# jopohl/urh

Hardware: NVIDIA H100
Metric: MSamples/s IQ demod+digitize (complex64) (higher is better)
Workload: dtype f32

## Files before the change

urh_b200/csrc/center.cu:

```cuda
#include "dense.cuh"
#include "tilescan.cuh"

#include <math.h>
#include <stdlib.h>

int urh_window_var_bitwise(urh_ctx* ctx, const float* d_x, int64_t n, const int64_t* d_prefix, int64_t t0, int64_t t1, int64_t r0,
                           int64_t r1, float* h_out2);

struct CenStats {
    double sum, sumsq;
    float mn, mx;
    long long cnt;
};

__global__ void __launch_bounds__(URH_WARPS_PER_BLOCK * 32)
k_tile_stats_f32(const float* __restrict__ x, int64_t n, int64_t ntiles, UrhTileStats* __restrict__ ts) {
    const int lane = threadIdx.x & 31;
    const int64_t tile = (int64_t)blockIdx.x * URH_WARPS_PER_BLOCK + (threadIdx.x >> 5);
    if (tile >= ntiles) return;
    const int64_t base = tile * URH_TILE;
    UrhStatAcc acc;
    acc.init();
    acc.all_noise = false;
    if (base + URH_TILE <= n && (((uintptr_t)x) & 15) == 0) {
        const float4* p = (const float4*)(x + base) + lane;
        constexpr int ITERS = URH_TILE / 128;
        float4 cur[4], nxt[4];
#pragma unroll
        for (int j = 0; j < 4; j++) cur[j] = __ldg(p + j * 32);
        for (int it = 0; it < ITERS; it += 4) {
            if (it + 4 < ITERS) {
#pragma unroll
                for (int j = 0; j < 4; j++) nxt[j] = __ldg(p + (it + 4 + j) * 32);
            }
#pragma unroll
            for (int j = 0; j < 4; j++) {
                acc.add(cur[j].x); acc.add(cur[j].y); acc.add(cur[j].z); acc.add(cur[j].w);
            }
#pragma unroll
            for (int j = 0; j < 4; j++) cur[j] = nxt[j];
        }
    } else {
        for (int j = lane; j < URH_TILE; j += 32)
            if (base + j < n) acc.add(x[base + j]);
    }
    acc.store(ts + tile, lane);
}

struct ScanKept {
    const UrhTileStats* ts;
    int64_t* prefix;
    __device__ __forceinline__ int64_t load(int64_t t) const { return ts[t].cnt; }
    __device__ __forceinline__ void post(int64_t t, const int64_t& excl, const int64_t&) const { prefix[t] = excl; }
};
struct CenAddI64 {
    __device__ __forceinline__ int64_t operator()(int64_t a, int64_t b) const { return a + b; }
};

static int kept_prefix(urh_ctx* ctx, const UrhTileStats* ts, int64_t ntiles, int64_t* prefix) {
    ScanKept fk;
    fk.ts = ts; fk.prefix = prefix;
    return urhts::scan<int64_t, CenAddI64, ScanKept>(ctx, ntiles, (int64_t)0, CenAddI64(), fk, prefix + ntiles);
}

#define CEN_PER (URH_TILE / 256)
__device__ __forceinline__ int64_t cen_tile_ranks(const float* __restrict__ x, int64_t n, int64_t t, int64_t tile_rank0, float (&v)[CEN_PER],
                                                  int* s_pre) {
    const int64_t base = t * URH_TILE + (int64_t)threadIdx.x * CEN_PER;
    int mine = 0;
#pragma unroll
    for (int j = 0; j < CEN_PER; j++) {
        v[j] = (base + j < n) ? x[base + j] : -5.0f;
        mine += (v[j] > -4.0f) ? 1 : 0;
    }
    s_pre[threadIdx.x] = mine;
    __syncthreads();
    for (int off = 1; off < 256; off <<= 1) {
        int add = 0;
        if (threadIdx.x >= off) add = s_pre[threadIdx.x - off];
        __syncthreads();
        s_pre[threadIdx.x] += add;
        __syncthreads();
    }
    return tile_rank0 + s_pre[threadIdx.x] - mine;
}

__device__ __forceinline__ void cen_block_fold(double sum, double sq, float mn, float mx, long long cnt, CenStats* out) {
    __shared__ double s_sum[256], s_sq[256];
    __shared__ float s_mn[256], s_mx[256];
    __shared__ long long s_cnt[256];
    __syncthreads();
    s_sum[threadIdx.x] = sum; s_sq[threadIdx.x] = sq; s_mn[threadIdx.x] = mn; s_mx[threadIdx.x] = mx; s_cnt[threadIdx.x] = cnt;
    __syncthreads();
    for (int off = 128; off > 0; off >>= 1) {
        if (threadIdx.x < off) {
            s_sum[threadIdx.x] += s_sum[threadIdx.x + off];
            s_sq[threadIdx.x] += s_sq[threadIdx.x + off];
            s_mn[threadIdx.x] = fminf(s_mn[threadIdx.x], s_mn[threadIdx.x + off]);
            s_mx[threadIdx.x] = fmaxf(s_mx[threadIdx.x], s_mx[threadIdx.x + off]);
            s_cnt[threadIdx.x] += s_cnt[threadIdx.x + off];
        }
        __syncthreads();
    }
    if (threadIdx.x == 0) {
        CenStats r;
        r.sum = s_sum[0]; r.sumsq = s_sq[0]; r.mn = s_mn[0]; r.mx = s_mx[0]; r.cnt = s_cnt[0];
        *out = r;
    }
}

int urh_center_tiles_begin(urh_ctx* ctx, const float* d_x, const UrhTileStats* ts, int64_t n, int64_t* h_total) {
    const int64_t ntiles = urh_div_up(n, URH_TILE);
    int64_t* prefix;
    URH_CHECK(urh_arena(ctx, (size_t)ntiles + 1, &prefix));
    URH_CHECK(kept_prefix(ctx, ts, ntiles, prefix));
    URH_CHECK(urh_read_i64(ctx, prefix + ntiles, 1, h_total));
    ctx->center_prefix = prefix;
    ctx->center_ts = ts;
    ctx->center_n = n;
    ctx->center_x = d_x;
    return URH_OK;
}

static int tiles_from_array(urh_ctx* ctx, const float* d_x, int64_t n, int64_t* h_total) {
    urh_arena_reset(ctx);
    ctx->center_prefix = nullptr;
    const int64_t ntiles = urh_div_up(n, URH_TILE);
    UrhTileStats* ts;
    URH_CHECK(urh_arena(ctx, (size_t)ntiles, &ts));
    URH_LAUNCH(ctx, k_tile_stats_f32, (unsigned)urh_div_up(ntiles, URH_WARPS_PER_BLOCK), URH_WARPS_PER_BLOCK * 32, 0, d_x, n, ntiles, ts);
    return urh_center_tiles_begin(ctx, d_x, ts, n, h_total);
}

static bool tiles_match(const urh_ctx* ctx, const float* d_x, int64_t n) {
    return ctx->center_prefix && ctx->center_n == n && ctx->center_x == (const void*)d_x;
}

extern "C" int urh_center_window_var(urh_ctx* ctx, const float* d_qad, int64_t n, int64_t r0, int64_t r1, double* h_out2) {
    h_out2[0] = h_out2[1] = 0.0;
    if (!tiles_match(ctx, d_qad, n)) URH_FAIL(ctx, URH_ERR_INVALID, "the tile table of this array must precede urh_center_window_var");
    if (r1 <= r0) return URH_OK;
    float mv[2];
    URH_CHECK(urh_window_var_bitwise(ctx, d_qad, n, (const int64_t*)ctx->center_prefix, 0, urh_div_up(n, URH_TILE) - 1, r0, r1, mv));
    h_out2[0] = (double)mv[0];
    h_out2[1] = (double)mv[1];
    return URH_OK;
}

extern "C" int urh_center_stats(urh_ctx* ctx, const float* d_x, int64_t n, int64_t max_size, double* h_out) {
    for (int i = 0; i < 7; i++) h_out[i] = 0.0;
    if (n <= 0) return URH_OK;
    int64_t total = 0;
    URH_CHECK(tiles_from_array(ctx, d_x, n, &total));
    int64_t r0 = (int64_t)(0.05 * (double)total), r1 = (int64_t)(0.95 * (double)total);
    if (max_size >= 0 && r1 - r0 > max_size) r1 = r0 + max_size;
    h_out[0] = (double)total; h_out[1] = (double)r0; h_out[2] = (double)r1;
    if (r1 <= r0) return URH_OK;
    double w[5];
    URH_CHECK(urh_center_window_stats(ctx, d_x, n, r0, r1, w));
    if (w[0] <= 0.0) return URH_OK;
    h_out[3] = w[1]; h_out[4] = w[2];
    float mv[2];
    URH_CHECK(urh_window_var_bitwise(ctx, d_x, n, (const int64_t*)ctx->center_prefix, 0, urh_div_up(n, URH_TILE) - 1, r0, r1, mv));
    h_out[5] = (double)mv[0];
    h_out[6] = (double)mv[1];
    return URH_OK;
}


template <typename K>
__device__ __forceinline__ double cen_edge(K k, const double& hmin, const double& edge1, const double& delta) {
    return (k == 0) ? hmin : (k == 1 ? edge1 : __dadd_rn(hmin, __dmul_rn((double)k, delta)));
}

__device__ __forceinline__ void cen_edge_table(long long k0, long long stride, long long nbins, const double& hmin, const double& edge1,
                                               const double& delta, float* __restrict__ fe, unsigned long long* __restrict__ hist,
                                               unsigned long long* __restrict__ xhist) {
    for (long long k = k0; k <= nbins; k += stride) {
        const double e = cen_edge(k, hmin, edge1, delta);
        fe[k] = __double2float_ru(e);
        if (k == nbins) {
            fe[nbins + 1] = __double2float_rd(e);
            fe[nbins + 2] = fmaxf(__double2float_ru(hmin), nextafterf(-4.0f, 0.0f));
        }
        if (k < nbins) {
            hist[k] = 0ull;
            if (xhist) xhist[k] = 0ull;
        }
    }
}

struct HistBins {
    const float* fe;
    float f_min, f_hi, scale, off;
    int nbins;
    __device__ __forceinline__ void load(const float* fe_, float scale_, int nbins_) {
        fe = fe_; nbins = nbins_; scale = scale_;
        f_hi = fe[nbins + 1];
        f_min = fe[nbins + 2];
        off = -fe[0] * scale;
    }
    template <bool FAST>
    __device__ __forceinline__ int bin_of(float f) const {
        const bool valid = f >= f_min && f <= f_hi;
        if (FAST) {
            const float t = fmaf(f, scale, off);
            int r = __float_as_int(t + 12582912.0f) - 0x4B400000;
            r = max(0, min(r, nbins));
            int k = r - ((f < fe[r]) ? 1 : 0);
            k = min(k, nbins - 1);
            return valid ? k : -1;
        }
        if (!valid) return -1;
        int k = (int)((f - fe[0]) * scale);
        k = max(0, min(k, nbins - 1));
        while (k > 0 && f < fe[k]) k--;
        while (k < nbins - 1 && f >= fe[k + 1]) k++;
        return k;
    }
};

struct HistCache {
    float lo0, hi0, lo1, hi1, lo2, hi2, lo3, hi3;
    int h0, h1, h2, h3;
    unsigned c0, c1, c2, c3;
    __device__ __forceinline__ void init() {
        lo0 = lo1 = lo2 = lo3 = INFINITY;
        hi0 = hi1 = hi2 = hi3 = -INFINITY;
        h0 = h1 = h2 = h3 = 0;
        c0 = c1 = c2 = c3 = 0u;
    }
};

template <bool SMEM>
__device__ __forceinline__ void hist_bump(unsigned int* s_hist, unsigned long long* hist, int k, unsigned c) {
    if (SMEM) atomicAdd(&s_hist[k], c);
    else atomicAdd(&hist[k], (unsigned long long)c);
}

template <bool SMEM, bool FAST>
__device__ __forceinline__ void hist_miss(HistCache& hc, const HistBins& hb, unsigned int* s_hist, unsigned long long* hist, float f) {
    const int k = hb.bin_of<FAST>(f);
    if (k < 0) return;
    const float lo = fmaxf(hb.fe[k], hb.f_min);
    const float hi = (k == hb.nbins - 1) ? nextafterf(hb.f_hi, INFINITY) : hb.fe[k + 1];
    unsigned cm = hc.c0; int which = 0;
    if (hc.c1 < cm) { cm = hc.c1; which = 1; }
    if (hc.c2 < cm) { cm = hc.c2; which = 2; }
    if (hc.c3 < cm) { cm = hc.c3; which = 3; }
    const int old = which == 0 ? hc.h0 : which == 1 ? hc.h1 : which == 2 ? hc.h2 : hc.h3;
    if (cm) hist_bump<SMEM>(s_hist, hist, old, cm);
    if (which == 0) { hc.h0 = k; hc.c0 = 1u; hc.lo0 = lo; hc.hi0 = hi; }
    else if (which == 1) { hc.h1 = k; hc.c1 = 1u; hc.lo1 = lo; hc.hi1 = hi; }
    else if (which == 2) { hc.h2 = k; hc.c2 = 1u; hc.lo2 = lo; hc.hi2 = hi; }
    else { hc.h3 = k; hc.c3 = 1u; hc.lo3 = lo; hc.hi3 = hi; }
}

template <bool SMEM, bool FAST>
__device__ __forceinline__ void hist_put(HistCache& hc, const HistBins& hb, unsigned int* s_hist, unsigned long long* hist, float f,
                                         unsigned one) {
    unsigned miss;
    asm("{\n\t.reg .pred p0, p1, p2, p3, pv;\n\t"
        "setp.ge.f32 p0, %5, %6;\n\tsetp.lt.and.f32 p0, %5, %7, p0;\n\t@p0 mad.lo.u32 %0, %0, %15, %15;\n\t"
        "setp.ge.f32 p1, %5, %8;\n\tsetp.lt.and.f32 p1, %5, %9, p1;\n\t@p1 mad.lo.u32 %1, %1, %15, %15;\n\t"
        "setp.ge.f32 p2, %5, %10;\n\tsetp.lt.and.f32 p2, %5, %11, p2;\n\t@p2 mad.lo.u32 %2, %2, %15, %15;\n\t"
        "setp.ge.f32 p3, %5, %12;\n\tsetp.lt.and.f32 p3, %5, %13, p3;\n\t@p3 mad.lo.u32 %3, %3, %15, %15;\n\t"
        "or.pred p0, p0, p1;\n\tor.pred p2, p2, p3;\n\tor.pred p0, p0, p2;\n\t"
        "setp.ge.f32 pv, %5, %14;\n\t"
        "and.pred pv, pv, !p0;\n\t"
        "selp.u32 %4, 1, 0, pv;\n\t}"
        : "+r"(hc.c0), "+r"(hc.c1), "+r"(hc.c2), "+r"(hc.c3), "=r"(miss)
        : "f"(f), "f"(hc.lo0), "f"(hc.hi0), "f"(hc.lo1), "f"(hc.hi1), "f"(hc.lo2), "f"(hc.hi2), "f"(hc.lo3), "f"(hc.hi3),
          "f"(hb.f_min), "r"(one));
    if (miss) hist_miss<SMEM, FAST>(hc, hb, s_hist, hist, f);
}

template <bool SMEM>
__device__ __forceinline__ void hist_flush(HistCache& hc, unsigned int* s_hist, unsigned long long* hist) {
    if (hc.c0) hist_bump<SMEM>(s_hist, hist, hc.h0, hc.c0);
    if (hc.c1) hist_bump<SMEM>(s_hist, hist, hc.h1, hc.c1);
    if (hc.c2) hist_bump<SMEM>(s_hist, hist, hc.h2, hc.c2);
    if (hc.c3) hist_bump<SMEM>(s_hist, hist, hc.h3, hc.c3);
}

template <bool SMEM, bool FAST>
__device__ __forceinline__ void hist_interior_body(const float* __restrict__ x, int64_t n, int64_t t_first, int64_t t_end, int blk, int nblk,
                                                   const float* __restrict__ g_fe, float scale, int nbins,
                                                   unsigned long long* __restrict__ hist, int edges_in_smem,
                                                   const int64_t* __restrict__ prefix) {
    extern __shared__ unsigned int s_dyn[];
    unsigned int* s_hist = s_dyn;
    float* s_fe = (float*)(s_dyn + (SMEM ? nbins : 0));
    const int lane = threadIdx.x & 31;
    if (SMEM)
        for (int b = threadIdx.x; b < nbins; b += 256) s_hist[b] = 0u;
    if (edges_in_smem)
        for (int b = threadIdx.x; b < nbins + 3; b += 256) s_fe[b] = g_fe[b];
    __syncthreads();
    HistBins hb;
    if (FAST) hb.load(s_fe, scale, nbins);
    else hb.load(edges_in_smem ? s_fe : g_fe, scale, nbins);
    HistCache hc;
    hc.init();
    const int64_t gw = (int64_t)blk * 8 + (threadIdx.x >> 5), nw = (int64_t)nblk * 8;
    const bool vec = (((uintptr_t)x) & 15) == 0;
    const unsigned one = blockDim.x >> 8;
    {
        for (int64_t t = t_first + gw; t < t_end; t += nw) {
            if (prefix[t + 1] == prefix[t]) continue;
            const int64_t base = t * URH_TILE;
            if (vec) {
                const float4* p = (const float4*)(x + base) + lane;
                constexpr int ITERS = URH_TILE / 128, DEPTH = 4;
                float4 buf[DEPTH];
#pragma unroll
                for (int j = 0; j < DEPTH; j++) buf[j] = __ldg(p + j * 32);
#pragma unroll 1
                for (int it = 0; it < ITERS; it += DEPTH) {
                    const bool more = it + DEPTH < ITERS;
#pragma unroll
                    for (int j = 0; j < DEPTH; j++) {
                        const float4 v = buf[j];
                        if (more) buf[j] = __ldg(p + (it + DEPTH + j) * 32);
                        hist_put<SMEM, FAST>(hc, hb, s_hist, hist, v.x, one);
                        hist_put<SMEM, FAST>(hc, hb, s_hist, hist, v.y, one);
                        hist_put<SMEM, FAST>(hc, hb, s_hist, hist, v.z, one);
                        hist_put<SMEM, FAST>(hc, hb, s_hist, hist, v.w, one);
                    }
                }
            } else {
                for (int j = lane; j < URH_TILE; j += 32) hist_put<SMEM, FAST>(hc, hb, s_hist, hist, x[base + j], one);
            }
        }
    }
    hist_flush<SMEM>(hc, s_hist, hist);
    if (SMEM) {
        __syncthreads();
        for (int b = threadIdx.x; b < nbins; b += 256)
            if (s_hist[b]) atomicAdd(&hist[b], (unsigned long long)s_hist[b]);
    }
}

__device__ __forceinline__ void hist_window_ends_body(const float* __restrict__ x, int64_t n, const int64_t* __restrict__ prefix,
                                                      const int64_t* __restrict__ win, int64_t r0, int64_t r1,
                                                      const float* __restrict__ g_fe, float scale, int nbins,
                                                      unsigned long long* __restrict__ hist, unsigned long long* __restrict__ hist2 = nullptr) {
    __shared__ int s_pre[256];
    const int64_t t = win[blockIdx.x];
    if (t < 0 || (blockIdx.x == 1 && t == win[0])) return;
    HistBins hb;
    hb.load(g_fe, scale, nbins);
    float v[CEN_PER];
    int64_t rank = cen_tile_ranks(x, n, t, prefix[t], v, s_pre);
#pragma unroll
    for (int j = 0; j < CEN_PER; j++) {
        const bool kept = v[j] > -4.0f;
        const int k = hb.bin_of<false>(v[j]);
        if (k >= 0 && rank >= r0 && rank < r1) {
            atomicAdd(&hist[k], 1ull);
            if (hist2) atomicAdd(&hist2[k], 1ull);
        }
        rank += kept ? 1 : 0;
    }
}

extern "C" int urh_center_histogram(urh_ctx* ctx, const float* d_x, int64_t n, int64_t r0, int64_t r1, double hmin,
                                    double hstep, int64_t nbins, int64_t* h_hist) {
    if (nbins <= 0 || n <= 0) return URH_OK;
    if (!tiles_match(ctx, d_x, n)) {
        int64_t total = 0;
        URH_CHECK(tiles_from_array(ctx, d_x, n, &total));
    }
    return urh_center_histogram_tiles(ctx, d_x, n, r0, r1, hmin, hstep, nbins, h_hist);
}

#define CEN_MAX_BINS 6000
#define CEN_VAR_MIN_RATIO 0x1p-14

struct __align__(16) CenterPlan {
    long long total, offset;
    long long r0, r1;
    long long lr0, lr1;
    long long win[4];
    CenStats local;
    double hmin, edge1, delta;
    long long nbins;
    double center;
    float centerf;
    float scale;
    int fast;
    int state;
    unsigned int ticket;
    int certified;
    long long straddle;
    long long pad;
};

__global__ void k_center_ranks(const int64_t* __restrict__ counts, int rank, int world, int64_t max_size, CenterPlan* __restrict__ plan) {
    long long total = 0, offset = 0;
    for (int q = 0; q < world; q++) {
        if (q < rank) offset += counts[q];
        total += counts[q];
    }
    const long long kept = counts[rank];
    long long r0 = (long long)(0.05 * (double)total), r1 = (long long)(0.95 * (double)total);
    if (max_size >= 0 && r1 - r0 > max_size) r1 = r0 + max_size;
    plan->total = total; plan->offset = offset; plan->r0 = r0; plan->r1 = r1;
    long long a = r0 - offset, b = r1 - offset;
    a = a < 0 ? 0 : (a > kept ? kept : a);
    b = b < 0 ? 0 : (b > kept ? kept : b);
    plan->lr0 = a; plan->lr1 = b;
    plan->ticket = 0u;
    plan->state = 1;
    plan->certified = 0;
    plan->straddle = 0;
}

__device__ __forceinline__ int64_t cen_tile_of_rank(const int64_t* __restrict__ prefix, int64_t ntiles, int64_t r) {
    int64_t lo = 0, hi = ntiles;
    while (hi - lo > 1) {
        const int64_t mid = (lo + hi) >> 1;
        if (prefix[mid] <= r) lo = mid; else hi = mid;
    }
    return lo;
}

__device__ __forceinline__ void cen_window_tiles(const int64_t* __restrict__ prefix, int64_t ntiles, long long r0, long long r1,
                                                 long long (&w)[4]) {
    long long w0 = -1, w1 = -1, w2 = -1, w3 = -1;
    if (r1 > r0) {
        w0 = cen_tile_of_rank(prefix, ntiles, r0);
        w1 = cen_tile_of_rank(prefix, ntiles, r1 - 1);
        const bool cov0 = prefix[w0] >= r0 && prefix[w0 + 1] <= r1;
        const bool cov1 = prefix[w1] >= r0 && prefix[w1 + 1] <= r1;
        w2 = cov0 ? -1 : w0;
        w3 = (cov1 || w1 == w0) ? -1 : w1;
    }
    w[0] = w0; w[1] = w1; w[2] = w2; w[3] = w3;
}

__global__ void __launch_bounds__(256) k_center_window(const float* __restrict__ x, int64_t n, const UrhTileStats* __restrict__ ts,
                                                      const int64_t* __restrict__ prefix, int64_t ntiles, CenterPlan* __restrict__ plan,
                                                      CenStats* __restrict__ partial) {
    __shared__ long long s_win[4];
    __shared__ int s_pre[256];
    __shared__ bool s_last;
    const long long r0 = plan->lr0, r1 = plan->lr1;
    if (threadIdx.x == 0) {
        long long w[4];
        cen_window_tiles(prefix, ntiles, r0, r1, w);
        s_win[0] = w[0]; s_win[1] = w[1]; s_win[2] = w[2]; s_win[3] = w[3];
        if (blockIdx.x == 0) { plan->win[0] = w[0]; plan->win[1] = w[1]; plan->win[2] = w[2]; plan->win[3] = w[3]; }
    }
    __syncthreads();
    double sum = 0.0, sq = 0.0;
    float mn = INFINITY, mx = -INFINITY;
    long long cnt = 0;
    if (s_win[0] >= 0) {
        for (int64_t t = s_win[0] + (int64_t)blockIdx.x * 256 + threadIdx.x; t <= s_win[1]; t += (int64_t)gridDim.x * 256) {
            const int64_t a = prefix[t], b = prefix[t + 1];
            if (b > a && a >= r0 && b <= r1) {
                const UrhTileStats v = ts[t];
                sum += v.sum; sq += v.sumsq; mn = fminf(mn, v.mn); mx = fmaxf(mx, v.mx); cnt += v.cnt;
            }
        }
    }
    cen_block_fold(sum, sq, mn, mx, cnt, partial + blockIdx.x);
    if (blockIdx.x < 2) {
        const int64_t t = s_win[2 + blockIdx.x];
        sum = 0.0; sq = 0.0; mn = INFINITY; mx = -INFINITY; cnt = 0;
        if (t >= 0) {
            float v[CEN_PER];
            int64_t rank = cen_tile_ranks(x, n, t, prefix[t], v, s_pre);
#pragma unroll
            for (int j = 0; j < CEN_PER; j++) {
                if (v[j] > -4.0f) {
                    if (rank >= r0 && rank < r1) {
                        sum += (double)v[j];
                        sq += (double)v[j] * (double)v[j];
                        mn = fminf(mn, v[j]);
                        mx = fmaxf(mx, v[j]);
                        cnt++;
                    }
                    rank++;
                }
            }
        }
        cen_block_fold(sum, sq, mn, mx, cnt, partial + gridDim.x + blockIdx.x);
    }
    __threadfence();
    __syncthreads();
    if (threadIdx.x == 0) s_last = atomicAdd(&plan->ticket, 1u) == gridDim.x - 1;
    __syncthreads();
    if (!s_last) return;
    __threadfence();
    sum = 0.0; sq = 0.0; mn = INFINITY; mx = -INFINITY; cnt = 0;
    for (int64_t t = threadIdx.x; t < (int64_t)gridDim.x + 2; t += 256) {
        CenStats p;
        {
            const int4* src = (const int4*)(partial + t);
            int4 w0 = __ldcg(src), w1 = __ldcg(src + 1);
            memcpy(&p, &w0, 16);
            memcpy((char*)&p + 16, &w1, 16);
        }
        sum += p.sum; sq += p.sumsq; mn = fminf(mn, p.mn); mx = fmaxf(mx, p.mx); cnt += p.cnt;
    }
    cen_block_fold(sum, sq, mn, mx, cnt, &plan->local);
}

__global__ void __launch_bounds__(256) k_center_plan(const CenStats* __restrict__ parts, int world, CenterPlan* __restrict__ plan,
                                                    float* __restrict__ fe, unsigned long long* __restrict__ hist,
                                                    unsigned long long* __restrict__ xhist) {
    __shared__ int s_state;
    __shared__ long long s_nbins;
    __shared__ double s_hmin, s_edge1, s_delta;
    if (threadIdx.x == 0) {
        double cnt = 0.0, sum = 0.0, sq = 0.0;
        float mn = INFINITY, mx = -INFINITY;
        for (int q = 0; q < world; q++) {
            cnt += (double)parts[q].cnt;
            mn = fminf(mn, parts[q].mn);
            mx = fmaxf(mx, parts[q].mx);
            sum = __dadd_rn(sum, parts[q].sum);
            sq = __dadd_rn(sq, parts[q].sumsq);
        }
        int state = 0;
        long long nbins = 0;
        double hmin = 0.0, edge1 = 0.0, delta = 0.0;
        if (plan->r1 > plan->r0 && cnt > 0.0) {
            const double mean = __ddiv_rn(sum, cnt);
            double ss = __dsub_rn(sq, __dmul_rn(__dmul_rn(cnt, mean), mean));
            if (ss < 0.0) ss = 0.0;
            const double var = __ddiv_rn(ss, cnt);
            const double hstep = (double)__double2float_rn(var);
            hmin = (double)mn;
            const double stop = __dadd_rn((double)mx, hstep);
            if (!(var >= __dmul_rn(__dmul_rn(mean, mean), CEN_VAR_MIN_RATIO))) state = 2;
            else if (hstep != 0.0) {
                const double val = __ddiv_rn(__dsub_rn(stop, hmin), hstep);
                if (val == val && fabs(val) < 9.0e18) {
                    const long long len = (long long)ceil(val);
                    if (len >= 2) {
                        nbins = len - 1;
                        edge1 = __dadd_rn(hmin, hstep);
                        delta = __dsub_rn(edge1, hmin);
                        state = (nbins <= CEN_MAX_BINS && delta > 0.0) ? 1 : 2;
                    }
                }
            }
        }
        plan->hmin = hmin; plan->edge1 = edge1; plan->delta = delta; plan->nbins = nbins;
        plan->state = state;
        plan->center = 0.0; plan->centerf = 0.0f;
        if (state == 1) {
            plan->scale = (float)(1.0 / delta);
            const double edge_abs = fmax(fabs(hmin), fabs(hmin + (double)nbins * delta));
            plan->fast = (edge_abs / delta < 1048576.0) ? 1 : 0;
        }
        s_state = state; s_nbins = nbins; s_hmin = hmin; s_edge1 = edge1; s_delta = delta;
    }
    __syncthreads();
    if (s_state != 1) return;
    cen_edge_table(threadIdx.x, 256, s_nbins, s_hmin, s_edge1, s_delta, fe, hist, xhist);
}

template <bool SMEM, bool FAST, int MIN_BLOCKS>
__global__ void __launch_bounds__(256, MIN_BLOCKS) k_hist_interior(const float* __restrict__ x, int64_t n, const CenterPlan* __restrict__ plan,
                                                                  const float* __restrict__ g_fe, unsigned long long* __restrict__ hist,
                                                                  const int64_t* __restrict__ prefix, int edges_in_smem) {
    if (plan->state != 1 || plan->certified || (plan->fast != 0) != FAST) return;
    hist_interior_body<SMEM, FAST>(x, n, plan->win[0] + 1, plan->win[1], blockIdx.x, gridDim.x, g_fe, plan->scale, (int)plan->nbins, hist,
                                   edges_in_smem, prefix);
}

__device__ __forceinline__ void cen_full_slabs(int64_t win0, int64_t win1, int64_t slab_tiles, int64_t* sf, int64_t* se) {
    *sf = (win0 + slab_tiles) / slab_tiles;
    *se = win1 / slab_tiles;
}

__global__ void __launch_bounds__(256) k_hist_window_ends(const float* __restrict__ x, int64_t n, const int64_t* __restrict__ prefix,
                                                         const CenterPlan* __restrict__ plan, const float* __restrict__ g_fe,
                                                         unsigned long long* __restrict__ hist, unsigned long long* __restrict__ xhist,
                                                         int64_t slab_tiles) {
    if (plan->state != 1) return;
    if (blockIdx.x < 2) {
        hist_window_ends_body(x, n, prefix, (const int64_t*)plan->win, plan->lr0, plan->lr1, g_fe, plan->scale, (int)plan->nbins, hist, xhist);
        return;
    }
    const int64_t w0 = plan->win[0], w1 = plan->win[1];
    int64_t sf, se;
    cen_full_slabs(w0, w1, slab_tiles, &sf, &se);
    int64_t a_end = w1, b_begin = w1;
    if (sf < se) { a_end = sf * slab_tiles; b_begin = se * slab_tiles; }
    const int blk = blockIdx.x - 2, nblk = gridDim.x - 2, nbins = (int)plan->nbins;
    const float scale = plan->scale;
    if (plan->fast) {
        hist_interior_body<true, true>(x, n, w0 + 1, a_end, blk, nblk, g_fe, scale, nbins, xhist, 1, prefix);
        hist_interior_body<true, true>(x, n, b_begin, w1, blk, nblk, g_fe, scale, nbins, xhist, 1, prefix);
    } else {
        hist_interior_body<true, false>(x, n, w0 + 1, a_end, blk, nblk, g_fe, scale, nbins, xhist, 1, prefix);
        hist_interior_body<true, false>(x, n, b_begin, w1, blk, nblk, g_fe, scale, nbins, xhist, 1, prefix);
    }
}

__device__ __forceinline__ double cen_left_edge(const CenterPlan* plan, int k) {
    return cen_edge(k, plan->hmin, plan->edge1, plan->delta);
}

#define CERT_THREADS 512
__global__ void __launch_bounds__(CERT_THREADS) k_center_certify(const UrhFine fine, CenterPlan* __restrict__ plan, const float* __restrict__ fe,
                                                                 const unsigned long long* __restrict__ xhist, unsigned long long* __restrict__ lo,
                                                                 unsigned long long* __restrict__ hi) {
    __shared__ unsigned long long s_ge[URH_FINE_NB + 1];
    __shared__ unsigned long long s_part[CERT_THREADS];
    __shared__ unsigned char s_flag[CEN_MAX_BINS];
    __shared__ unsigned long long s_key[3];
    __shared__ unsigned int s_certain;
    if (plan->state != 1) return;
    const int tid = threadIdx.x;
    constexpr int PER = URH_FINE_NB / CERT_THREADS;
    int64_t sf, se;
    cen_full_slabs(plan->win[0], plan->win[1], fine.slab_tiles, &sf, &se);
    unsigned long long b[PER], tot = 0;
#pragma unroll
    for (int j = 0; j < PER; j++) {
        unsigned long long v = 0;
        for (int64_t sl = sf; sl < se; sl++) v += fine.gh[sl * URH_FINE_NB + tid * PER + j];
        b[j] = v;
        tot += v;
    }
    s_part[tid] = tot;
    if (tid < 3) s_key[tid] = 0ull;
    if (tid == 0) s_certain = 0u;
    __syncthreads();
    for (int off = 1; off < CERT_THREADS; off <<= 1) {
        const unsigned long long add = (tid + off < CERT_THREADS) ? s_part[tid + off] : 0ull;
        __syncthreads();
        s_part[tid] += add;
        __syncthreads();
    }
    unsigned long long run = (tid + 1 < CERT_THREADS) ? s_part[tid + 1] : 0ull;
#pragma unroll
    for (int j = PER - 1; j >= 0; j--) {
        run += b[j];
        s_ge[tid * PER + j] = run;
    }
    if (tid == 0) s_ge[URH_FINE_NB] = 0ull;
    __syncthreads();
    const int nbins = (int)plan->nbins;
    const float f_hi = fe[nbins + 1], f_min = fe[nbins + 2], top = nextafterf(f_hi, INFINITY);
    auto ge = [&](float t, unsigned long long& glo, unsigned long long& ghi) {
        const int bt = urh_fine_bucket(t, fine.scale, fine.off);
        const bool straddles = urh_fine_bucket(nextafterf(t, -INFINITY), fine.scale, fine.off) == bt;
        ghi = s_ge[bt];
        glo = straddles ? s_ge[bt + 1] : s_ge[bt];
    };
    for (int k = tid; k < nbins; k += CERT_THREADS) {
        const float a = fmaxf(fe[k], f_min), e = (k == nbins - 1) ? top : fminf(fe[k + 1], top);
        unsigned long long l = 0, u = 0;
        if (a < e) {
            unsigned long long alo, ahi, elo, ehi;
            ge(a, alo, ahi);
            ge(e, elo, ehi);
            l = alo > ehi ? alo - ehi : 0ull;
            u = ahi - elo;
        }
        lo[k] = xhist[k] + l;
        hi[k] = xhist[k] + u;
    }
    __syncthreads();
    int window = (int)(0.05 * (double)nbins) + 1;
    if (window < 2) window = 2;
    for (int k = tid; k < nbins; k += CERT_THREADS) {
        const unsigned long long l = lo[k], u = hi[k];
        bool certain = l > 0ull, possible = u > 0ull;
        for (int d = -(window - 1); d < window && (certain || possible); d++) {
            const int j = k + d;
            if (d == 0 || j < 0 || j >= nbins) continue;
            certain = certain && l > hi[j];
            possible = possible && u > lo[j];
        }
        s_flag[k] = certain ? 1 : (possible ? 2 : 0);
        if (certain) atomicAdd(&s_certain, 1u);
    }
    __syncthreads();
    for (int pass = 0; pass < 3; pass++) {
        const long long p0 = pass > 0 ? (long long)(8191 - (s_key[0] & 8191)) : -1, p1 = pass > 1 ? (long long)(8191 - (s_key[1] & 8191)) : -1;
        for (int k = tid; k < nbins; k += CERT_THREADS) {
            if (k == p0 || k == p1) continue;
            if (pass < 2 && s_flag[k] == 1) atomicMax(&s_key[pass], (lo[k] << 13) | (unsigned long long)(8191 - k));
            if (pass == 2 && s_flag[k] != 0) atomicMax(&s_key[2], hi[k]);
        }
        __syncthreads();
    }
    if (tid != 0 || s_certain < 2u) return;
    const int k1 = 8191 - (int)(s_key[0] & 8191), k2 = 8191 - (int)(s_key[1] & 8191);
    plan->straddle = (long long)((hi[k1] - lo[k1]) + (hi[k2] - lo[k2]));
    if (!(lo[k2] > s_key[2])) return;
    const double c = __ddiv_rn(__dadd_rn(cen_left_edge(plan, k1), cen_left_edge(plan, k2)), 2.0);
    plan->center = c;
    plan->centerf = __double2float_rn(c);
    plan->certified = 1;
}

__global__ void __launch_bounds__(256) k_center_pick(const unsigned long long* __restrict__ y, CenterPlan* __restrict__ plan) {
    __shared__ unsigned long long s_best[256];
    __shared__ int s_idx[256];
    __shared__ int s_cnt[256];
    if (plan->state != 1 || plan->certified) return;
    const int nbins = (int)plan->nbins;
    int window = (int)(0.05 * (double)nbins) + 1;
    if (window < 2) window = 2;
    unsigned long long top_val[2] = {0ull, 0ull};
    int top_idx[2] = {-1, -1};
    int found = 0;
    bool undecided = false;
    for (int pass = 0; pass < 2 && !undecided; pass++) {
        unsigned long long best = 0ull;
        int bi = -1, ties = 0;
        for (int i = threadIdx.x; i < nbins; i += 256) {
            if (pass == 1 && i == top_idx[0]) continue;
            const unsigned long long v = y[i];
            if (v == 0ull || v < best) continue;
            bool peak = true;
            for (int d = 1; d < window && peak; d++) {
                const unsigned long long a = (i + d < nbins) ? y[i + d] : 0ull;
                const unsigned long long b = (i - d >= 0) ? y[i - d] : 0ull;
                peak = v > a && v > b;
            }
            if (!peak) continue;
            if (v > best) { best = v; bi = i; ties = 1; }
            else ties++;
        }
        s_best[threadIdx.x] = best; s_idx[threadIdx.x] = bi; s_cnt[threadIdx.x] = ties;
        __syncthreads();
        if (threadIdx.x == 0) {
            unsigned long long b = 0ull;
            int idx = -1, t = 0;
            for (int j = 0; j < 256; j++) {
                if (s_idx[j] < 0) continue;
                if (s_best[j] > b) { b = s_best[j]; idx = s_idx[j]; t = s_cnt[j]; }
                else if (s_best[j] == b) t += s_cnt[j];
            }
            s_best[0] = b; s_idx[0] = idx; s_cnt[0] = t;
        }
        __syncthreads();
        const unsigned long long b = s_best[0];
        const int idx = s_idx[0], t = s_cnt[0];
        __syncthreads();
        if (idx < 0) break;
        if (pass == 0) {
            top_val[0] = b; top_idx[0] = idx; found = 1;
            if (t == 2) {
                int other = -1;
                for (int i = threadIdx.x; i < nbins; i += 256) {
                    if (i == idx || y[i] != b) continue;
                    bool peak = true;
                    for (int d = 1; d < window && peak; d++) {
                        const unsigned long long a = (i + d < nbins) ? y[i + d] : 0ull;
                        const unsigned long long c = (i - d >= 0) ? y[i - d] : 0ull;
                        peak = b > a && b > c;
                    }
                    if (peak) other = i;
                }
                s_idx[threadIdx.x] = other;
                __syncthreads();
                if (threadIdx.x == 0) {
                    int o = -1;
                    for (int j = 0; j < 256; j++) if (s_idx[j] >= 0) o = s_idx[j];
                    s_idx[0] = o;
                }
                __syncthreads();
                top_idx[1] = s_idx[0]; top_val[1] = b; found = 2;
                __syncthreads();
                break;
            }
            if (t > 2) undecided = true;
        } else {
            if (t > 1) undecided = true;
            else { top_val[1] = b; top_idx[1] = idx; found = 2; }
        }
    }
    if (threadIdx.x != 0) return;
    if (undecided) { plan->state = 2; return; }
    if (found == 0) { plan->state = 0; return; }
    double c;
    if (found == 1) c = cen_left_edge(plan, top_idx[0]);
    else c = __ddiv_rn(__dadd_rn(cen_left_edge(plan, top_idx[0]), cen_left_edge(plan, top_idx[1])), 2.0);
    plan->center = c;
    plan->centerf = __double2float_rn(c);
    plan->state = 1;
    (void)top_val;
}

__global__ void __launch_bounds__(256) k_center_set(const int64_t* __restrict__ prefix, int64_t ntiles, long long r0, long long r1, double hmin,
                                                   double hstep, long long nbins, float scale, int fast, CenterPlan* __restrict__ plan,
                                                   float* __restrict__ fe, unsigned long long* __restrict__ hist) {
    const double edge1 = __dadd_rn(hmin, hstep);
    if (blockIdx.x == 0 && threadIdx.x == 0) {
        plan->lr0 = r0; plan->lr1 = r1;
        plan->ticket = 0u;
        plan->state = 1;
        plan->certified = 0;
        if (nbins > 0) {
            long long w[4];
            cen_window_tiles(prefix, ntiles, r0, r1, w);
            for (int i = 0; i < 4; i++) plan->win[i] = w[i];
            plan->hmin = hmin; plan->edge1 = edge1; plan->delta = hstep; plan->nbins = nbins;
            plan->scale = scale;
            plan->fast = fast;
        }
    }
    if (nbins > 0)
        cen_edge_table((long long)blockIdx.x * blockDim.x + threadIdx.x, (long long)gridDim.x * blockDim.x, nbins, hmin, edge1, hstep, fe, hist,
                       nullptr);
}

extern "C" int urh_center_window_stats(urh_ctx* ctx, const float* d_qad, int64_t n, int64_t r0, int64_t r1, double* h_out5) {
    h_out5[0] = 0.0; h_out5[1] = INFINITY; h_out5[2] = -INFINITY; h_out5[3] = 0.0; h_out5[4] = 0.0;
    if (!tiles_match(ctx, d_qad, n)) URH_FAIL(ctx, URH_ERR_INVALID, "urh_afp_demod_tiles (same qad, same n) must precede urh_center_window_stats");
    if (r1 <= r0) return URH_OK;
    const int64_t ntiles = urh_div_up(n, URH_TILE);
    const int64_t* prefix = (const int64_t*)ctx->center_prefix;
    CenterPlan* plan;
    CenStats* partial;
    const int nb = ctx->sm_count * 2;
    URH_CHECK(urh_arena(ctx, 1, &plan));
    URH_CHECK(urh_arena(ctx, (size_t)nb + 2, &partial));
    URH_LAUNCH(ctx, k_center_set, 1, 1, 0, prefix, ntiles, (long long)r0, (long long)r1, 0.0, 0.0, 0LL, 0.0f, 0, plan, nullptr, nullptr);
    URH_LAUNCH(ctx, k_center_window, nb, 256, 0, d_qad, n, (const UrhTileStats*)ctx->center_ts, prefix, ntiles, plan, partial);
    CenStats st;
    URH_CUDA(ctx, cudaMemcpyAsync(ctx->h_mail, &plan->local, sizeof(CenStats), cudaMemcpyDeviceToHost, ctx->stream));
    URH_CUDA(ctx, cudaStreamSynchronize(ctx->stream));
    memcpy(&st, ctx->h_mail, sizeof(st));
    h_out5[0] = (double)st.cnt; h_out5[1] = (double)st.mn; h_out5[2] = (double)st.mx; h_out5[3] = st.sum; h_out5[4] = st.sumsq;
    return URH_OK;
}

extern "C" int urh_center_histogram_tiles(urh_ctx* ctx, const float* d_qad, int64_t n, int64_t r0, int64_t r1, double hmin,
                                          double hstep, int64_t nbins, int64_t* h_hist) {
    if (nbins <= 0) return URH_OK;
    if (!tiles_match(ctx, d_qad, n)) URH_FAIL(ctx, URH_ERR_INVALID, "urh_afp_demod_tiles (same qad, same n) must precede urh_center_histogram_tiles");
    if (nbins > (int64_t)1 << 30) URH_FAIL(ctx, URH_ERR_INVALID, "too many histogram bins");
    if (r1 <= r0) {
        memset(h_hist, 0, (size_t)nbins * sizeof(int64_t));
        return URH_OK;
    }
    const int64_t ntiles = urh_div_up(n, URH_TILE);
    const int64_t* prefix = (const int64_t*)ctx->center_prefix;
    CenterPlan* plan;
    float* fe;
    unsigned long long* hist;
    URH_CHECK(urh_arena(ctx, 1, &plan));
    URH_CHECK(urh_arena(ctx, (size_t)nbins + 3, &fe));
    URH_CHECK(urh_arena(ctx, (size_t)nbins, &hist));
    const bool in_smem = nbins <= 12000;
    const int edges_smem = (in_smem && nbins <= 6000) ? 1 : 0;
    const size_t dyn = (in_smem ? (size_t)nbins * 4 : 0) + (edges_smem ? (size_t)(nbins + 3) * 4 : 0);
    const float scale = (float)(1.0 / hstep);
    const double edge_abs = fmax(fabs(hmin), fabs(hmin + (double)nbins * hstep));
    const int fast = (edges_smem && hstep > 0.0 && edge_abs / hstep < 1048576.0) ? 1 : 0;
    const unsigned gs = (unsigned)min(urh_div_up(ntiles, 8), (int64_t)ctx->sm_count * 8);
    URH_LAUNCH(ctx, k_center_set, (unsigned)urh_div_up(nbins + 1, 256), 256, 0, prefix, ntiles, (long long)r0, (long long)r1, hmin, hstep,
               (long long)nbins, scale, fast, plan, fe, hist);
    const CenterPlan* cplan = plan;
    const float* cfe = fe;
    if (fast) URH_LAUNCH(ctx, (k_hist_interior<true, true, 3>), gs, 256, dyn, d_qad, n, cplan, cfe, hist, prefix, edges_smem);
    else if (edges_smem) URH_LAUNCH(ctx, (k_hist_interior<true, false, 3>), gs, 256, dyn, d_qad, n, cplan, cfe, hist, prefix, edges_smem);
    else if (in_smem) URH_LAUNCH(ctx, (k_hist_interior<true, false, 4>), gs, 256, dyn, d_qad, n, cplan, cfe, hist, prefix, edges_smem);
    else URH_LAUNCH(ctx, (k_hist_interior<false, false, 4>), gs, 256, dyn, d_qad, n, cplan, cfe, hist, prefix, edges_smem);
    URH_LAUNCH(ctx, k_hist_window_ends, 2, 256, 0, d_qad, n, prefix, cplan, cfe, hist, (unsigned long long*)nullptr, (int64_t)1);
    URH_CUDA(ctx, cudaMemcpyAsync(h_hist, hist, (size_t)nbins * sizeof(int64_t), cudaMemcpyDeviceToHost, ctx->stream));
    URH_CUDA(ctx, cudaStreamSynchronize(ctx->stream));
    return URH_OK;
}

int urh_center_chain(urh_ctx* ctx, const float* d_qad, int64_t n, const UrhTileStats* ts, int64_t max_size, int rank, int world,
                     const UrhFine* fine, CenterPlan** d_plan_out) {
    const int64_t ntiles = urh_div_up(n, URH_TILE);
    int64_t* prefix;
    CenterPlan* plan;
    CenStats* partial;
    float* fe;
    unsigned long long* hist;
    int64_t* d_counts;
    CenStats* d_parts;
    unsigned long long *xhist = nullptr, *cert_lo = nullptr, *cert_hi = nullptr;
    const int nb = ctx->sm_count * 2;
    URH_CHECK(urh_arena(ctx, (size_t)ntiles + 1, &prefix));
    URH_CHECK(urh_arena(ctx, 1, &plan));
    URH_CHECK(urh_arena(ctx, (size_t)nb + 2, &partial));
    URH_CHECK(urh_arena(ctx, (size_t)CEN_MAX_BINS + 3, &fe));
    URH_CHECK(urh_arena(ctx, (size_t)CEN_MAX_BINS, &hist));
    URH_CHECK(urh_arena(ctx, (size_t)world, &d_counts));
    URH_CHECK(urh_arena(ctx, (size_t)world, &d_parts));
    if (fine) {
        URH_CHECK(urh_arena(ctx, (size_t)CEN_MAX_BINS, &xhist));
        URH_CHECK(urh_arena(ctx, (size_t)CEN_MAX_BINS, &cert_lo));
        URH_CHECK(urh_arena(ctx, (size_t)CEN_MAX_BINS, &cert_hi));
    }
    URH_CHECK(kept_prefix(ctx, ts, ntiles, prefix));
    const int64_t* counts = prefix + ntiles;
    if (world > 1) {
        URH_TL_MARK(ctx, "x1 kept counts: enter");
        URH_CHECK(urh_nccl_allgather(ctx, prefix + ntiles, d_counts, sizeof(int64_t)));
        URH_TL_MARK(ctx, "x1 kept counts: done");
        counts = d_counts;
    }
    URH_LAUNCH(ctx, k_center_ranks, 1, 1, 0, counts, rank, world, max_size, plan);
    URH_LAUNCH(ctx, k_center_window, nb, 256, 0, d_qad, n, ts, (const int64_t*)prefix, ntiles, plan, partial);
    const CenStats* parts = &plan->local;
    if (world > 1) {
        URH_TL_MARK(ctx, "x2 window partials: enter");
        URH_CHECK(urh_nccl_allgather(ctx, &plan->local, d_parts, sizeof(CenStats)));
        URH_TL_MARK(ctx, "x2 window partials: done");
        parts = d_parts;
    }
    URH_LAUNCH(ctx, k_center_plan, 1, 256, 0, parts, world, plan, fe, hist, xhist);
    const size_t dyn = (size_t)CEN_MAX_BINS * 4 + (size_t)(CEN_MAX_BINS + 3) * 4;
    const unsigned gs = (unsigned)min(urh_div_up(ntiles, 8), (int64_t)ctx->sm_count * 8);
    URH_LAUNCH(ctx, k_hist_window_ends, fine ? 2 + ctx->sm_count * 4 : 2, 256, fine ? dyn : 0, d_qad, n, (const int64_t*)prefix,
               (const CenterPlan*)plan, (const float*)fe, hist, xhist, fine ? fine->slab_tiles : (int64_t)1);
    if (fine) URH_LAUNCH(ctx, k_center_certify, 1, CERT_THREADS, 0, *fine, plan, (const float*)fe, (const unsigned long long*)xhist, cert_lo, cert_hi);
    URH_LAUNCH(ctx, (k_hist_interior<true, true, 3>), gs, 256, dyn, d_qad, n, (const CenterPlan*)plan, (const float*)fe, hist, (const int64_t*)prefix, 1);
    URH_LAUNCH(ctx, (k_hist_interior<true, false, 3>), gs, 256, dyn, d_qad, n, (const CenterPlan*)plan, (const float*)fe, hist, (const int64_t*)prefix, 1);
    if (world > 1) {
        URH_TL_MARK(ctx, "x3 histogram sum: enter");
        URH_CHECK(urh_nccl_allreduce_i64(ctx, (int64_t*)hist, CEN_MAX_BINS, 0));
        URH_TL_MARK(ctx, "x3 histogram sum: done");
    }
    URH_LAUNCH(ctx, k_center_pick, 1, 256, 0, (const unsigned long long*)hist, plan);
    ctx->center_prefix = prefix;
    ctx->center_ts = ts;
    ctx->center_n = n;
    ctx->center_x = d_qad;
    *d_plan_out = plan;
    return URH_OK;
}

int urh_center_plan_certify_stats(urh_ctx* ctx, const CenterPlan* plan, int64_t* h_dst3) {
    h_dst3[0] = h_dst3[1] = h_dst3[2] = 0;
    URH_CUDA(ctx, cudaMemcpyAsync(h_dst3, &plan->certified, sizeof(int), cudaMemcpyDeviceToHost, ctx->stream));
    URH_CUDA(ctx, cudaMemcpyAsync(h_dst3 + 2, &plan->straddle, sizeof(long long), cudaMemcpyDeviceToHost, ctx->stream));
    return URH_OK;
}

extern "C" int urh_center_certify_stats(urh_ctx* ctx, int64_t* h_out3) {
    for (int i = 0; i < 3; i++) h_out3[i] = ctx->center_cert[i];
    return URH_OK;
}

int urh_center_plan_result(urh_ctx* ctx, const CenterPlan* plan, const float** d_centerf, const double** d_center, const int** d_state) {
    if (d_centerf) *d_centerf = &plan->centerf;
    if (d_center) *d_center = &plan->center;
    if (d_state) *d_state = &plan->state;
    return URH_OK;
}
```

urh_b200/csrc/digitize.cu:

```cuda
#include "dense.cuh"
#include "tilescan.cuh"
#include "sparse.cuh"
#include "fsk_fast.cuh"
#include "dense_f32.cuh"
#include "stream_ring.cuh"

#include <math.h>
#include <stdlib.h>


template <int DT, int MOD, bool DIGITIZE>
__device__ __forceinline__ void dense_iq_tile(const void* __restrict__ iq, int64_t n, const UrhDemodParams& dp, float* __restrict__ qad_out,
                                              int vec_in, int vec_out, const UrhClassify& cls, int tol, UrhTileSummary* __restrict__ tiles,
                                              uint32_t* __restrict__ staging, int stage_cap, int16_t* __restrict__ init_cls, int cls_of_zero,
                                              int64_t tile, int has_halo, UrhTileStats* __restrict__ tile_stats, const UrhFine& fine,
                                              unsigned int* s_fine, unsigned int* g_fine) {
    const int lane = threadIdx.x & 31;
    const int64_t tile_start = tile * URH_TILE;
    const int tile_len = (int)((n - tile_start) < URH_TILE ? (n - tile_start) : URH_TILE);
    const int iters = (tile_len + 63) >> 6;

    UrhRunTracker rt;
    if (DIGITIZE) rt.init(tol, staging + tile * (int64_t)stage_cap);
    UrhStatAcc acc;
    acc.init();

    float cA = 0.0f, cB = 0.0f;
    if (MOD == URH_MOD_FSK && (tile_start > 0 || has_halo) && lane == 0) {
        typedef typename UrhElem<DT>::type E;
        const E* pp = (const E*)iq + 2 * (tile_start - 1);
        const UrhFskTerms t = urh_fsk_terms((float)pp[0], (float)pp[1]);
        cA = t.A; cB = t.B;
    }

    UrhPair cur = urh_load_pair<DT>(iq, tile_start + 2 * lane, n, vec_in != 0);
    for (int it = 0; it < iters; it++) {
        const int64_t pos0 = tile_start + (int64_t)it * 64 + 2 * lane;
        UrhPair nxt;
        if (it + 1 < iters) nxt = urh_load_pair<DT>(iq, pos0 + 64, n, vec_in != 0);

        const float m0 = __fadd_rn(__fmul_rn(cur.r0, cur.r0), __fmul_rn(cur.i0, cur.i0));
        const float m1 = __fadd_rn(__fmul_rn(cur.r1, cur.r1), __fmul_rn(cur.i1, cur.i1));
        float s0 = dp.noise_value, s1 = dp.noise_value;
        if (MOD == URH_MOD_FSK) {
            const UrhFskTerms t0 = urh_fsk_terms(cur.r0, cur.i0);
            const UrhFskTerms t1 = urh_fsk_terms(cur.r1, cur.i1);
            float pA = __shfl_up_sync(URH_FULL_MASK, t1.A, 1);
            float pB = __shfl_up_sync(URH_FULL_MASK, t1.B, 1);
            if (lane == 0) { pA = cA; pB = cB; }
            cA = __shfl_sync(URH_FULL_MASK, t1.A, 31);
            cB = __shfl_sync(URH_FULL_MASK, t1.B, 31);
            if (!(m0 <= dp.noise_sqrd)) s0 = urh_fsk_angle(pA, pB, t0.C, t0.D);
            if (!(m1 <= dp.noise_sqrd)) s1 = urh_fsk_angle(t0.A, t0.B, t1.C, t1.D);
        } else if (MOD == URH_MOD_ASK) {
            if (!(m0 <= dp.noise_sqrd)) s0 = __fdiv_rn(__fsqrt_rn(m0), dp.max_mag);
            if (!(m1 <= dp.noise_sqrd)) s1 = __fdiv_rn(__fsqrt_rn(m1), dp.max_mag);
        }
        if (pos0 == 0 && !has_halo) s0 = dp.noise_value;

        const bool v0 = pos0 < n, v1 = pos0 + 1 < n;
        if (tile_stats) {
            if (v0) { acc.add(s0); acc.all_noise = acc.all_noise && (s0 == dp.noise_value); }
            if (v1) { acc.add(s1); acc.all_noise = acc.all_noise && (s1 == dp.noise_value); }
            if (s_fine) {
                if (v0) urh_fine_add(s0, fine, s_fine, g_fine);
                if (v1) urh_fine_add(s1, fine, s_fine, g_fine);
            }
        }
        if (qad_out) {
            if (v1 && vec_out) urh_stg_f2(qad_out + pos0, s0, s1);
            else {
                if (v0) qad_out[pos0] = s0;
                if (v1) qad_out[pos0 + 1] = s1;
            }
        }
        if (DIGITIZE) {
            const int c0 = urh_classify(s0, cls), c1 = urh_classify(s1, cls);
            if (pos0 == 0) *init_cls = (int16_t)((s0 == cls.noise_value) ? -1 : cls_of_zero);
            rt.feed(it, c0, c1, v0, v1, lane);
        }
        cur = nxt;
    }
    if (tile_stats) acc.store(tile_stats + tile, lane);
    if (DIGITIZE) rt.finish(tile_len, tiles + tile, lane);
}

template <int DT, int MOD, bool DIGITIZE>
__global__ void __launch_bounds__(URH_WARPS_PER_BLOCK * 32)
k_dense_iq(const void* __restrict__ iq, int64_t n, UrhDemodParams dp, float* __restrict__ qad_out, int vec_in,
           int vec_out, const __grid_constant__ UrhClassify cls, int tol, UrhTileSummary* __restrict__ tiles,
           uint32_t* __restrict__ staging, int stage_cap, int16_t* __restrict__ init_cls, int cls_of_zero,
           int64_t tile_begin, int64_t tile_count, int has_halo, UrhTileStats* __restrict__ tile_stats, const UrhFine fine) {
    extern __shared__ unsigned int s_fine[];
    const int64_t tile_rel = (int64_t)blockIdx.x * URH_WARPS_PER_BLOCK + (threadIdx.x >> 5);
    const int64_t block_tile0 = tile_begin + (int64_t)blockIdx.x * URH_WARPS_PER_BLOCK;
    if (fine.gh) urh_fine_zero(s_fine);
    if (tile_rel < tile_count && (tile_begin + tile_rel) * URH_TILE < n)
        dense_iq_tile<DT, MOD, DIGITIZE>(iq, n, dp, qad_out, vec_in, vec_out, cls, tol, tiles, staging, stage_cap, init_cls, cls_of_zero,
                                    tile_begin + tile_rel, has_halo, tile_stats, fine,
                                    fine.gh ? s_fine : nullptr, fine.gh ? urh_fine_row(fine, tile_begin + tile_rel, block_tile0) : nullptr);
    if (fine.gh) urh_fine_flush(fine, s_fine, block_tile0);
}

template <int DT, bool DIGITIZE, bool WRITE, bool STATS>
__global__ void __launch_bounds__(URH_WARPS_PER_BLOCK * 32, (DT == URH_DT_F32) ? 5 : 4)
k_fsk_fifo(const void* __restrict__ iq, int64_t n, UrhDemodParams dp, float* __restrict__ qad_out, float thr0,
           float cls_noise, int tol, UrhTileSummary* __restrict__ tiles, uint32_t* __restrict__ staging, int stage_cap,
           int64_t tile_begin, int64_t tile_count, UrhTileStats* __restrict__ tile_stats, const UrhFine fine,
           const float* __restrict__ d_thr0 = nullptr, float* __restrict__ margin = nullptr) {
    __shared__ __align__(16) unsigned char s_fifo[URH_WARPS_PER_BLOCK][URH_FSK_FIFO + 1][64 * 2 * sizeof(typename UrhElem<DT>::type)];
    extern __shared__ unsigned int s_fine[];
    const bool fine_on = STATS && fine.gh;
    if (DIGITIZE && STATS) thr0 = *d_thr0;
    const int lane = threadIdx.x & 31;
    const int64_t tile_rel = (int64_t)blockIdx.x * URH_WARPS_PER_BLOCK + (threadIdx.x >> 5);
    const int64_t block_tile0 = tile_begin + (int64_t)blockIdx.x * URH_WARPS_PER_BLOCK;
    if (fine_on) urh_fine_zero(s_fine);
    if (tile_rel < tile_count) {
        const int64_t tile = tile_begin + tile_rel;
        UrhRunTracker rt;
        if (DIGITIZE) rt.init(tol, staging + tile * (int64_t)stage_cap);
        UrhOne one;
        one.p = dp.one;
        one.m = dp.mone;
        const uint32_t fifo = (uint32_t)__cvta_generic_to_shared(&s_fifo[threadIdx.x >> 5][0][0]);
        urh_fsk_full_tile<DT, DIGITIZE, WRITE, STATS>(iq, n, tile * URH_TILE, dp, qad_out, thr0, cls_noise, rt, lane, one,
                                                      STATS ? tile_stats + tile : nullptr, fifo, DIGITIZE ? tiles + tile : nullptr, fine,
                                                      fine_on ? s_fine : nullptr, fine_on ? urh_fine_row(fine, tile, block_tile0) : nullptr,
                                                      (DIGITIZE && STATS) ? margin + tile : nullptr);
    }
    if (fine_on) urh_fine_flush(fine, s_fine, block_tile0);
}

#define URH_GUESS_SAMPLES 16384
#define URH_GUESS_BINS 128
#define URH_GUESS_THREADS 1024
__global__ void __launch_bounds__(URH_GUESS_THREADS) k_speculate_guess(const float2* __restrict__ iq, int64_t n, float noise_sqrd, int forced,
                                                                      float forced_tg, float* __restrict__ d_tg, unsigned int* __restrict__ redone) {
    constexpr int PER = URH_GUESS_SAMPLES / URH_GUESS_THREADS;
    __shared__ unsigned int s_hist[URH_GUESS_BINS];
    __shared__ float s_mn[32], s_mx[32];
    if (forced) {
        if (threadIdx.x == 0) { *d_tg = forced_tg; *redone = 0u; }
        return;
    }
    for (int b = threadIdx.x; b < URH_GUESS_BINS; b += blockDim.x) s_hist[b] = 0u;
    float v[PER];
    float mn = INFINITY, mx = -INFINITY;
#pragma unroll
    for (int k = 0; k < PER; k++) {
        const int64_t i = 1 + (int64_t)(k * URH_GUESS_THREADS + threadIdx.x) * (n - 1) / URH_GUESS_SAMPLES;
        const float2 p = iq[i - 1], c = iq[i];
        v[k] = NAN;
        if (!(c.x * c.x + c.y * c.y <= noise_sqrd)) {
            v[k] = atan2f(p.x * c.y - p.y * c.x, p.x * c.x + p.y * c.y);
            mn = fminf(mn, v[k]);
            mx = fmaxf(mx, v[k]);
        }
    }
    for (int off = 16; off > 0; off >>= 1) {
        mn = fminf(mn, __shfl_xor_sync(URH_FULL_MASK, mn, off));
        mx = fmaxf(mx, __shfl_xor_sync(URH_FULL_MASK, mx, off));
    }
    if ((threadIdx.x & 31) == 0) { s_mn[threadIdx.x >> 5] = mn; s_mx[threadIdx.x >> 5] = mx; }
    __syncthreads();
    mn = INFINITY; mx = -INFINITY;
    for (int w = 0; w < URH_GUESS_THREADS / 32; w++) { mn = fminf(mn, s_mn[w]); mx = fmaxf(mx, s_mx[w]); }
    const float width = (mx - mn) / URH_GUESS_BINS;
    if (width > 0.0f) {
#pragma unroll
        for (int k = 0; k < PER; k++)
            if (!isnan(v[k])) atomicAdd(&s_hist[min((int)((v[k] - mn) / width), URH_GUESS_BINS - 1)], 1u);
    }
    __syncthreads();
    if (threadIdx.x != 0) return;
    *redone = 0u;
    if (!(mn <= mx)) { *d_tg = 0.0f; return; }
    if (!(width > 0.0f)) { *d_tg = mn; return; }
    constexpr int WINDOW = (int)(0.05 * URH_GUESS_BINS) + 1;
    int top[2] = {-1, -1};
    for (int b = 0; b < URH_GUESS_BINS; b++) {
        const unsigned int y = s_hist[b];
        bool peak = y > 0u;
        for (int d = 1; d < WINDOW && peak; d++)
            peak = y > (b + d < URH_GUESS_BINS ? s_hist[b + d] : 0u) && y > (b - d >= 0 ? s_hist[b - d] : 0u);
        if (!peak) continue;
        if (top[0] < 0 || y > s_hist[top[0]]) { top[1] = top[0]; top[0] = b; }
        else if (top[1] < 0 || y > s_hist[top[1]]) top[1] = b;
    }
    if (top[0] < 0) *d_tg = 0.5f * (mn + mx);
    else if (top[1] < 0) *d_tg = mn + ((float)top[0] + 0.5f) * width;
    else *d_tg = mn + (0.5f * (float)(top[0] + top[1]) + 0.5f) * width;
}


extern "C" int urh_get_center_thresholds(float center, float spacing, int modulation_order, float* h_out) {
    const int n = modulation_order / 2;
    for (int i = 0; i < n; i++) {
        volatile float t = (float)(n - (i + 1)) * spacing;
        h_out[i] = center - t;
    }
    for (int i = n; i < modulation_order - 1; i++) {
        volatile float t = (float)(i + 1 - n) * spacing;
        h_out[i] = center + t;
    }
    return URH_OK;
}

static int fill_classify(urh_ctx* ctx, UrhClassify* C, int mod_type, float center, uint8_t bits_per_symbol,
                         float spacing) {
    if (bits_per_symbol > 8) URH_FAIL(ctx, URH_ERR_INVALID, "bits_per_symbol %d > 8 not supported", (int)bits_per_symbol);
    memset(C, 0, sizeof(*C));
    C->noise_value = urh_noise_value(mod_type);
    C->order = 1 << bits_per_symbol;
    if (C->order > 1) urh_get_center_thresholds(center, spacing, C->order, C->thr);
    return URH_OK;
}

static int host_classify(float s, const UrhClassify& C) {
    int c = C.order - 1;
    for (int k = 0; k < C.order - 1; k++)
        if (s <= C.thr[k]) { c = k; break; }
    return c;
}

static float max_magnitude_for(int dtype) {
    switch (dtype) {
        case URH_DT_I8: return (float)sqrt(127.0 * 127.0 + 128.0 * 128.0);
        case URH_DT_U8: return (float)sqrt(255.0 * 255.0);
        case URH_DT_I16: return (float)sqrt(32768.0 * 32768.0 + 32767.0 * 32767.0);
        case URH_DT_U16: return (float)sqrt(65535.0 * 65535.0);
        default: return (float)sqrt(2.0);
    }
}

static bool iq_vec_aligned(const void* p, int dtype) { return ((uintptr_t)p % (2 * (size_t)urh_iq_bytes(dtype))) == 0; }

struct DensePass {
    float* qad = nullptr;
    const UrhDigitizer* dz = nullptr;
    int has_halo = 0;
    UrhTileStats* tile_stats = nullptr;
    int64_t tile_lo = 0, tile_hi = -1;
    UrhFine fine = {};
    UrhSpec* spec = nullptr;
};

template <int DT, int MOD, bool DIG>
static int launch_dense_iq_t(urh_ctx* ctx, const void* d_iq, int64_t n, const UrhDemodParams& dp, const UrhClassify& cls,
                             const DensePass& o) {
    static const UrhDigitizer none = {};
    const UrhDigitizer& dz = o.dz ? *o.dz : none;
    int16_t* init_cls = DIG ? dz.d_init : nullptr;
    const int cls_of_zero = DIG ? host_classify(0.0f, cls) : 0;
    const int64_t ntiles = urh_div_up(n, URH_TILE);
    const size_t fine_smem = o.fine.gh ? (size_t)URH_FINE_NB * sizeof(unsigned int) : 0;
    const int64_t tile_lo = o.tile_lo, tile_hi = (o.tile_hi < 0 || o.tile_hi > ntiles) ? ntiles : o.tile_hi;
    const int vec_in = iq_vec_aligned(d_iq, DT) ? 1 : 0;
    const int vec_out = (o.qad && ((uintptr_t)o.qad % 8) == 0) ? 1 : 0;
    const int threads = URH_WARPS_PER_BLOCK * 32;
    auto generic = [&](int64_t begin, int64_t end) -> int {
        begin = begin < tile_lo ? tile_lo : begin;
        end = end > tile_hi ? tile_hi : end;
        const int64_t count = end - begin;
        if (count <= 0) return URH_OK;
        URH_LAUNCH(ctx, (k_dense_iq<DT, MOD, DIG>), (unsigned)urh_div_up(count, URH_WARPS_PER_BLOCK), threads, fine_smem, d_iq, n, dp,
                   o.qad, vec_in, vec_out, cls, dz.tol, dz.tiles, dz.staging, dz.cap, init_cls, cls_of_zero, begin, count, o.has_halo,
                   o.tile_stats, o.fine);
        return URH_OK;
    };
    const int64_t nfull = n / URH_TILE;
    const bool fast = MOD == URH_MOD_FSK && vec_in && (!o.qad || vec_out) && (!DIG || cls.order == 2) && nfull > 1;
    URH_PROF_BEGIN(ctx);
    if (fast) {
        const int64_t fb = tile_lo > 1 ? tile_lo : 1, fe = tile_hi < nfull ? tile_hi : nfull;
        if (fe > fb) {
            const unsigned grid = (unsigned)urh_div_up(fe - fb, URH_WARPS_PER_BLOCK);
            bool speculated = false;
            if constexpr (DT == URH_DT_F32 && MOD == URH_MOD_FSK && !DIG) {
                if (o.spec && o.tile_stats && o.qad) {
                    URH_LAUNCH(ctx, (k_fsk_fifo<DT, true, true, true>), grid, threads, fine_smem, d_iq, n, dp, o.qad, 0.0f, dp.noise_value,
                               dz.tol, dz.tiles, dz.staging, dz.cap, fb, fe - fb, o.tile_stats, o.fine, (const float*)o.spec->tg, o.spec->margin);
                    o.spec->lo = fb;
                    o.spec->hi = fe;
                    speculated = true;
                }
            }
            if (speculated) {
            } else if (o.tile_stats && o.qad && !DIG) {
                URH_LAUNCH(ctx, (k_fsk_fifo<DT, false, true, true>), grid, threads, fine_smem, d_iq, n, dp, o.qad, cls.thr[0], cls.noise_value,
                           dz.tol, dz.tiles, dz.staging, dz.cap, fb, fe - fb, o.tile_stats, o.fine);
            } else if (o.qad) {
                URH_LAUNCH(ctx, (k_fsk_fifo<DT, DIG, true, false>), grid, threads, 0, d_iq, n, dp, o.qad, cls.thr[0], cls.noise_value, dz.tol,
                           dz.tiles, dz.staging, dz.cap, fb, fe - fb, nullptr, UrhFine{});
            } else {
                URH_LAUNCH(ctx, (k_fsk_fifo<DT, DIG, false, false>), grid, threads, 0, d_iq, n, dp, o.qad, cls.thr[0], cls.noise_value, dz.tol,
                           dz.tiles, dz.staging, dz.cap, fb, fe - fb, nullptr, UrhFine{});
            }
        }
        URH_CHECK(generic(0, 1));
        URH_CHECK(generic(nfull, ntiles));
    } else {
        URH_CHECK(generic(0, ntiles));
    }
    URH_PROF_END(ctx);
    return URH_OK;
}

template <int DT>
static int launch_dense_iq_dt(urh_ctx* ctx, int mod_type, const void* d_iq, int64_t n, const UrhDemodParams& dp, const UrhClassify& cls,
                              const DensePass& o) {
    const bool dig = o.dz && !o.spec;
    if (mod_type == URH_MOD_ASK)
        return dig ? launch_dense_iq_t<DT, URH_MOD_ASK, true>(ctx, d_iq, n, dp, cls, o) : launch_dense_iq_t<DT, URH_MOD_ASK, false>(ctx, d_iq, n, dp, cls, o);
    return dig ? launch_dense_iq_t<DT, URH_MOD_FSK, true>(ctx, d_iq, n, dp, cls, o) : launch_dense_iq_t<DT, URH_MOD_FSK, false>(ctx, d_iq, n, dp, cls, o);
}

static int launch_dense_iq(urh_ctx* ctx, int dtype, int mod_type, const void* d_iq, int64_t n, const UrhDemodParams& dp,
                           const UrhClassify& cls, const DensePass& o) {
    switch (dtype) {
        case URH_DT_I8: return launch_dense_iq_dt<URH_DT_I8>(ctx, mod_type, d_iq, n, dp, cls, o);
        case URH_DT_U8: return launch_dense_iq_dt<URH_DT_U8>(ctx, mod_type, d_iq, n, dp, cls, o);
        case URH_DT_I16: return launch_dense_iq_dt<URH_DT_I16>(ctx, mod_type, d_iq, n, dp, cls, o);
        case URH_DT_U16: return launch_dense_iq_dt<URH_DT_U16>(ctx, mod_type, d_iq, n, dp, cls, o);
        case URH_DT_F32: return launch_dense_iq_dt<URH_DT_F32>(ctx, mod_type, d_iq, n, dp, cls, o);
        default: URH_FAIL(ctx, URH_ERR_DTYPE, "Unsupported dtype");
    }
}

int urh_costas_demod(urh_ctx* ctx, const void* d_iq, int dtype, int64_t n, float noise_sqrd, int loop_order,
                     float bandwidth, float* d_out);

static UrhDemodParams make_demod_params(float noise_mag, int mod_type, int dtype) {
    UrhDemodParams dp;
    volatile float nm = noise_mag;
    volatile float sq = nm * nm;
    dp.noise_sqrd = sq;
    dp.noise_value = urh_noise_value(mod_type);
    dp.max_mag = max_magnitude_for(dtype);
    dp.one = 1.0f;
    dp.mone = -1.0f;
    return dp;
}

extern "C" int urh_afp_demod(urh_ctx* ctx, const void* d_iq, int dtype, int64_t n, float noise_mag, int mod_type,
                             int mod_order, float costas_loop_bandwidth, float* d_out) {
    if (n < 0) URH_FAIL(ctx, URH_ERR_INVALID, "negative length");
    if (urh_iq_bytes(dtype) == 0) URH_FAIL(ctx, URH_ERR_DTYPE, "Unsupported dtype");
    if (n == 0) return URH_OK;
    if (n <= 2 || (mod_type != URH_MOD_ASK && mod_type != URH_MOD_FSK && mod_type != URH_MOD_PSK)) {
        URH_CUDA(ctx, cudaMemsetAsync(d_out, 0, (size_t)n * sizeof(float), ctx->stream));
        if (n > 2) {
            const float nv = urh_noise_value(mod_type);
            URH_CUDA(ctx, cudaMemcpyAsync(d_out, &nv, sizeof(float), cudaMemcpyHostToDevice, ctx->stream));
            URH_CUDA(ctx, cudaStreamSynchronize(ctx->stream));
        }
        return URH_OK;
    }
    const UrhDemodParams dp = make_demod_params(noise_mag, mod_type, dtype);
    if (mod_type == URH_MOD_PSK) return urh_costas_demod(ctx, d_iq, dtype, n, dp.noise_sqrd, mod_order, costas_loop_bandwidth, d_out);
    UrhClassify cls;
    memset(&cls, 0, sizeof(cls));
    return launch_dense_iq(ctx, dtype, mod_type, d_iq, n, dp, cls, DensePass{d_out});
}

int urh_center_tiles_begin(urh_ctx* ctx, const float* d_x, const UrhTileStats* ts, int64_t n, int64_t* h_total);

extern "C" int urh_afp_demod_tiles(urh_ctx* ctx, const void* d_iq, int dtype, int64_t n, float noise_mag, int mod_type,
                                   float* d_qad_out, int halo, int64_t* h_kept) {
    if (n <= 2 || (mod_type != URH_MOD_ASK && mod_type != URH_MOD_FSK) || !d_qad_out)
        URH_FAIL(ctx, URH_ERR_INVALID, "urh_afp_demod_tiles: ASK/FSK, n > 2 and a qad buffer are required");
    if (urh_iq_bytes(dtype) == 0) URH_FAIL(ctx, URH_ERR_DTYPE, "Unsupported dtype");
    urh_arena_reset(ctx);
    const UrhDemodParams dp = make_demod_params(noise_mag, mod_type, dtype);
    UrhClassify cls;
    memset(&cls, 0, sizeof(cls));
    const int64_t ntiles = urh_div_up(n, URH_TILE);
    UrhTileStats* ts;
    URH_CHECK(urh_arena(ctx, (size_t)ntiles, &ts));
    URH_CHECK(launch_dense_iq(ctx, dtype, mod_type, d_iq, n, dp, cls, DensePass{d_qad_out, nullptr, halo, ts}));
    return urh_center_tiles_begin(ctx, d_qad_out, ts, n, h_kept);
}

static int pulses_begin(urh_ctx* ctx, int64_t* k, bool args_ok = true) {
    if (!k || !args_ok) return URH_ERR_INVALID;
    *k = 0;
    ctx->pulses_k = 0;
    return URH_OK;
}

static int launch_dense_qad(urh_ctx* ctx, const UrhDigitizer& dz, const float* x, int64_t s0, int64_t s1, const UrhClassify& cls,
                            const float* d_thr0 = nullptr, const UrhTileStats* ts = nullptr) {
    const int64_t n = s1 - s0;
    const unsigned grid = (unsigned)urh_div_up(urh_div_up(n, URH_TILE), URH_WARPS_PER_BLOCK);
    const int vec_in = (((uintptr_t)x % 8) == 0) ? 1 : 0;
    int16_t* init = s0 == 0 ? dz.d_init : nullptr;
    const int c0 = d_thr0 ? 0 : host_classify(0.0f, cls);
    if (ts) ts += s0 / URH_TILE;
    if (cls.order == 2)
        URH_LAUNCH(ctx, (k_dense_f32<SrcQad2, float>), grid, URH_WARPS_PER_BLOCK * 32, 0, x, n, vec_in, cls, dz.tol, dz.tiles, dz.staging,
                   dz.cap, init, c0, d_thr0, ts);
    else
        URH_LAUNCH(ctx, (k_dense_f32<SrcQad, float>), grid, URH_WARPS_PER_BLOCK * 32, 0, x, n, vec_in, cls, dz.tol, dz.tiles, dz.staging,
                   dz.cap, init, c0, d_thr0, ts);
    return URH_OK;
}

extern "C" int urh_grab_pulse_lens(urh_ctx* ctx, const float* d_qad, int64_t n, float center, uint16_t tolerance,
                                   int mod_type, uint32_t samples_per_symbol, uint8_t bits_per_symbol,
                                   float center_spacing, int64_t* k) {
    URH_CHECK(pulses_begin(ctx, k));
    if (n < 0) URH_FAIL(ctx, URH_ERR_INVALID, "negative length");
    if (n == 0) return URH_OK;
    urh_arena_reset(ctx);
    UrhClassify cls;
    URH_CHECK(fill_classify(ctx, &cls, mod_type, center, bits_per_symbol, center_spacing));
    UrhDigitizer dz;
    URH_CHECK(dz.init(ctx, n, tolerance, mod_type == URH_MOD_ASK, samples_per_symbol, urh_div_up(n, URH_TILE), false));
    URH_PROF_BEGIN(ctx);
    URH_CHECK(launch_dense_qad(ctx, dz, d_qad, 0, n, cls));
    URH_PROF_END(ctx);
    return finish_tiles(ctx, dz, FinishShard::local(dz), k);
}

extern "C" int urh_demod_digitize(urh_ctx* ctx, const void* d_iq, int dtype, int64_t n, float noise_mag,
                                  int mod_type, float center, uint16_t tolerance, uint32_t samples_per_symbol,
                                  uint8_t bits_per_symbol, float center_spacing, float* d_qad_out, int64_t* k) {
    URH_CHECK(pulses_begin(ctx, k));
    if (n < 0) URH_FAIL(ctx, URH_ERR_INVALID, "negative length");
    if (urh_iq_bytes(dtype) == 0) URH_FAIL(ctx, URH_ERR_DTYPE, "Unsupported dtype");
    if (n == 0) return URH_OK;
    if (n <= 2 || (mod_type != URH_MOD_ASK && mod_type != URH_MOD_FSK)) {
        float* q = d_qad_out;
        if (!q) URH_CUDA(ctx, cudaMalloc((void**)&q, (size_t)n * sizeof(float)));
        int rc = urh_afp_demod(ctx, d_iq, dtype, n, noise_mag, mod_type, 1 << bits_per_symbol, 0.1f, q);
        if (rc == URH_OK)
            rc = urh_grab_pulse_lens(ctx, q, n, center, tolerance, mod_type, samples_per_symbol, bits_per_symbol,
                                     center_spacing, k);
        if (!d_qad_out) {
            cudaStreamSynchronize(ctx->stream);
            cudaFree(q);
        }
        return rc;
    }
    urh_arena_reset(ctx);
    UrhClassify cls;
    URH_CHECK(fill_classify(ctx, &cls, mod_type, center, bits_per_symbol, center_spacing));
    const UrhDemodParams dp = make_demod_params(noise_mag, mod_type, dtype);
    UrhDigitizer dz;
    URH_CHECK(dz.init(ctx, n, tolerance, mod_type == URH_MOD_ASK, samples_per_symbol, urh_div_up(n, URH_TILE), false));
    URH_CHECK(launch_dense_iq(ctx, dtype, mod_type, d_iq, n, dp, cls, DensePass{d_qad_out, &dz}));
    return finish_tiles(ctx, dz, FinishShard::local(dz), k);
}

static int64_t rows_bound(int64_t n, int tol) { return n / (tol + 1) + 3; }

struct StreamSizes {
    int64_t cs;
    int64_t src_slot;
    int64_t qad_slot;
    int64_t ring_bytes;
    int64_t arena;
    int64_t scan_items;
    int64_t rows_chunk;
};
static int64_t scan_workspace_bytes(int64_t items) {
    const int64_t nb = 2 * (items / 256 + 1);
    return 256 + (nb > 8192 ? nb : 8192) * (4 + 2 * (int64_t)urhts::SLOT);
}
static int64_t finish_arena_bytes(int64_t tiles, int64_t rows_cap, bool ask) {
    return r256(tiles * (int64_t)sizeof(RunCarry)) + 2 * r256(tiles * 4) + 2 * r256(tiles * 8) + r256((32 + 8) * 8) +
           (ask ? r256(rows_cap * 16) : 0);
}
static int psk_order_of(int entry) { return (entry & URH_STREAM_PSK) ? ((entry & URH_STREAM_PSK4) ? 4 : 2) : 0; }
static int psk_entry_flags(int mod_order) { return URH_STREAM_PSK | (mod_order >= 4 ? URH_STREAM_PSK4 : 0); }

static StreamSizes stream_sizes(int64_t n, int dtype, int tol, int64_t chunk_samples, int ring, int entry) {
    StreamSizes z;
    const int kind = entry & 0xf;
    const int psk = psk_order_of(entry);
    const bool resident = entry & URH_STREAM_RESIDENT;
    const int64_t ntiles = urh_div_up(n, URH_TILE);
    z.cs = resident ? ntiles * URH_TILE : stream_chunk_samples(n, chunk_samples);
    const int64_t ct = z.cs / URH_TILE;
    const int64_t cap = stage_cap_for(tol);
    const bool iq = kind != URH_STREAM_ENTRY_GRAB_PULSE_LENS;
    const bool digitize = kind != URH_STREAM_ENTRY_AFP_DEMOD;
    z.rows_chunk = rows_bound(z.cs, tol);
    if (resident) {
        z.src_slot = iq ? n * urh_iq_bytes(dtype) : n * 4;
        z.qad_slot = (kind == URH_STREAM_ENTRY_GRAB_PULSE_LENS) ? 0 : n * 4;
        z.ring_bytes = r256(z.src_slot) + r256(z.qad_slot);
    } else {
        z.src_slot = (kind == URH_STREAM_ENTRY_GRAB_PULSE_LENS && (entry & URH_STREAM_QAD_ON_DEVICE)) ? 0
                     : URH_STREAM_PAD + z.cs * (iq ? urh_iq_bytes(dtype) : 4);
        const bool qad_ring = kind == URH_STREAM_ENTRY_AFP_DEMOD ||
                              (kind == URH_STREAM_ENTRY_DEMOD_DIGITIZE && ((entry & URH_STREAM_QAD_OUT) || psk));
        z.qad_slot = qad_ring ? z.cs * 4 : 0;
        z.ring_bytes = ring * (r256(z.src_slot) + r256(z.qad_slot));
        if (kind == URH_STREAM_ENTRY_DEMOD_CENTER_DIGITIZE) z.ring_bytes += r256(n * 4);
    }
    z.arena = 0;
    z.scan_items = ct > z.rows_chunk ? ct : z.rows_chunk;
    if (digitize) z.arena += r256(ct * (int64_t)sizeof(UrhTileSummary)) + r256(ct * cap * 4) + r256(16) + r256(sizeof(UrhChain)) +
                             finish_arena_bytes(ct, z.rows_chunk, true);
    if (psk && !resident) z.arena += urh_costas_arena_bytes(z.cs, psk) + r256(16) + r256(6 * 8);
    if (kind == URH_STREAM_ENTRY_DEMOD_CENTER_DIGITIZE) {
        z.arena += r256(ntiles * (int64_t)sizeof(UrhTileStats)) + r256((int64_t)URH_FINE_SLABS * URH_FINE_NB * 4) + r256((ntiles + 1) * 8) +
                   ((int64_t)2 << 20);
        if (ntiles > z.scan_items) z.scan_items = ntiles;
    }
    return z;
}

static int64_t segment_arena_bytes(int64_t tiles) {
    const int64_t cap = URH_TILE / 10 + 2, cand = tiles * URH_TILE / 10 + 3;
    return r256(tiles * (int64_t)sizeof(UrhTileSummary)) + r256(tiles * cap * 4) + 2 * r256(2 * (int64_t)sizeof(RunCarry)) +
           r256(tiles * 4) + r256(tiles * 8) + r256(32) + r256(cand * 8) + r256(cand * 2);
}
SegmentStreamSizes urh_segment_stream_sizes(int64_t n, int dtype, int64_t chunk_samples) {
    SegmentStreamSizes z;
    z.cs = stream_chunk_samples(n, chunk_samples);
    z.src_slot = r256(URH_STREAM_PAD + z.cs * urh_iq_bytes(dtype));
    z.mag_bytes = r256(z.cs * 8);
    z.arena = segment_arena_bytes(z.cs / URH_TILE);
    return z;
}

extern "C" int urh_stream_footprint(int64_t n, int dtype, int tolerance, int64_t chunk_samples, int ring, int entry, int64_t rows,
                                    int64_t* bytes) {
    if (!bytes || n < 0 || tolerance < 0 || tolerance > 0xffff || (entry & 0xf) > URH_STREAM_ENTRY_ESTIMATE) return URH_ERR_INVALID;
    if ((entry & 0xf) == URH_STREAM_ENTRY_SEGMENT_MESSAGES) {
        if (urh_iq_bytes(dtype) == 0) return URH_ERR_DTYPE;
        if (entry & URH_STREAM_RESIDENT) {
            const int64_t ntiles = urh_div_up(n, URH_TILE);
            *bytes = r256(n * urh_iq_bytes(dtype)) + r256(n * 8) + segment_arena_bytes(ntiles) + URH_ARENA_BLOCK + scan_workspace_bytes(ntiles);
            return URH_OK;
        }
        if (ring < 2 || ring > URH_STREAM_MAX_RING) return URH_ERR_INVALID;
        const SegmentStreamSizes z = urh_segment_stream_sizes(n, dtype, chunk_samples);
        *bytes = ring * z.src_slot + z.mag_bytes + stream_arena_bytes(z.arena) + scan_workspace_bytes(z.cs / URH_TILE);
        return URH_OK;
    }
    if ((entry & 0xf) == URH_STREAM_ENTRY_ESTIMATE) {
        if (!(entry & URH_STREAM_RESIDENT)) return URH_ERR_INVALID;
        if (urh_iq_bytes(dtype) == 0) return URH_ERR_DTYPE;
        int64_t demod = 0;
        URH_CHECK(urh_stream_footprint(n, dtype, 0, chunk_samples, ring, URH_STREAM_ENTRY_AFP_DEMOD | URH_STREAM_PSK | URH_STREAM_RESIDENT,
                                       -1, &demod));
        *bytes = r256(n * 8) + demod;
        return URH_OK;
    }
    if (!(entry & URH_STREAM_RESIDENT) && (ring < 2 || ring > URH_STREAM_MAX_RING)) return URH_ERR_INVALID;
    if ((entry & 0xf) != URH_STREAM_ENTRY_GRAB_PULSE_LENS && urh_iq_bytes(dtype) == 0) return URH_ERR_DTYPE;
    if ((entry & URH_STREAM_PSK) && (entry & 0xf) != URH_STREAM_ENTRY_AFP_DEMOD && (entry & 0xf) != URH_STREAM_ENTRY_DEMOD_DIGITIZE)
        return URH_ERR_INVALID;
    const StreamSizes z = stream_sizes(n, dtype, tolerance, chunk_samples, ring, entry);
    const bool digitize = (entry & 0xf) != URH_STREAM_ENTRY_AFP_DEMOD;
    const int64_t r = rows == -2 ? n / 64 + 1024 : (rows < 0 ? rows_bound(n, tolerance) : rows);
    if (entry & URH_STREAM_RESIDENT) {
        const int64_t ntiles = urh_div_up(n, URH_TILE);
        int64_t b = z.ring_bytes + URH_ARENA_BLOCK;
        if (digitize)
            b += r256(ntiles * (int64_t)sizeof(UrhTileSummary)) + r256(ntiles * (int64_t)stage_cap_for(tolerance) * 4) +
                 finish_arena_bytes(ntiles, r + r / 4, true) + 16 * (r + r / 4);
        if ((entry & 0xf) == URH_STREAM_ENTRY_DEMOD_CENTER_DIGITIZE)
            b += r256(ntiles * (int64_t)sizeof(UrhTileStats)) + r256((int64_t)URH_FINE_SLABS * URH_FINE_NB * 4) + r256((ntiles + 1) * 8);
        if (psk_order_of(entry)) b += urh_costas_arena_bytes(n, psk_order_of(entry));
        *bytes = b;
        return URH_OK;
    }
    int64_t b = z.ring_bytes + stream_arena_bytes(z.arena);
    b += scan_workspace_bytes(z.scan_items);
    if (digitize) b += 3 * 16 * (r + z.rows_chunk);
    *bytes = b;
    return URH_OK;
}

extern "C" int urh_stream_stats(urh_ctx* ctx, int64_t* h_out3) {
    h_out3[0] = ctx->stream_free_low;
    h_out3[1] = ctx->stream_chunks;
    h_out3[2] = (int64_t)ctx->arena_peak;
    return URH_OK;
}

struct StreamDigitizer {
    UrhDigitizer dz;
    UrhChain* chain;
    int64_t rows, rows_all;
    UrhArenaMark mark;
    int init(urh_ctx* ctx, int64_t n, int64_t cs, int tol, bool ask, uint32_t sps) {
        rows = 0;
        rows_all = rows_bound(n, tol);
        URH_CHECK(dz.init(ctx, n, tol, ask, sps, cs / URH_TILE, true));
        URH_CHECK(urh_arena(ctx, 1, &chain));
        mark = urh_arena_mark(ctx);
        return URH_OK;
    }
    int finish(urh_ctx* ctx, int64_t s0, int64_t s1) {
        const int64_t rc = rows_bound(s1 - s0, dz.tol);
        const int64_t need = rows + rc;
        if (need > (int64_t)ctx->pulses_cap_rows) {
            int64_t grow = 2 * (int64_t)ctx->pulses_cap_rows;
            if (grow > rows_all + rc) grow = rows_all + rc;
            URH_CHECK(urh_ensure_pulses_keep(ctx, (size_t)(grow > need ? grow : need), (size_t)rows));
        }
        urh_arena_release(ctx, mark);
        int64_t kc = 0;
        URH_CHECK(finish_tiles(ctx, dz, FinishShard::chunk(chain, s0, s1, dz.n, rows, rc), &kc));
        urh_stream_sample_free(ctx);
        rows += kc;
        return URH_OK;
    }
};

static int stream_check(urh_ctx* ctx, int64_t n, int ring, int mod_type, int dtype, bool iq);
static int psk_stream_check(urh_ctx* ctx, int64_t n, int ring, int dtype) {
    URH_CHECK(stream_check(ctx, n, ring, URH_MOD_PSK, dtype, false));
    if (n <= 2) URH_FAIL(ctx, URH_ERR_INVALID, "streamed PSK demodulation: n > 2");
    if (urh_iq_bytes(dtype) == 0) URH_FAIL(ctx, URH_ERR_DTYPE, "Unsupported dtype");
    return URH_OK;
}

static int stream_check(urh_ctx* ctx, int64_t n, int ring, int mod_type, int dtype, bool iq) {
    if (n <= 0) URH_FAIL(ctx, URH_ERR_INVALID, "streamed call: empty capture");
    if (ring < 2 || ring > URH_STREAM_MAX_RING) URH_FAIL(ctx, URH_ERR_INVALID, "streamed call: ring of %d slots (2..%d)", ring, URH_STREAM_MAX_RING);
    if (iq && (n <= 2 || (mod_type != URH_MOD_ASK && mod_type != URH_MOD_FSK)))
        URH_FAIL(ctx, URH_ERR_INVALID, "streamed demodulation: ASK/FSK and n > 2 (PSK is a serial recurrence)");
    if (iq && urh_iq_bytes(dtype) == 0) URH_FAIL(ctx, URH_ERR_DTYPE, "Unsupported dtype");
    return URH_OK;
}

static int stream_dense_iq(urh_ctx* ctx, int dtype, int mod_type, const char* slot, int64_t n, const UrhDemodParams& dp,
                           const UrhClassify& cls, const UrhWindow& w, DensePass o) {
    const void* iq = slot + URH_STREAM_PAD - w.k0 * urh_iq_bytes(dtype);
    o.tile_lo = w.k0 / URH_TILE;
    o.tile_hi = urh_div_up(w.k1, URH_TILE);
    UrhDigitizer view;
    if (o.dz) {
        view = *o.dz;
        view.tiles -= o.tile_lo;
        view.staging -= o.tile_lo * view.cap;
        o.dz = &view;
    }
    return launch_dense_iq(ctx, dtype, mod_type, iq, n, dp, cls, o);
}

struct CenterPlan;
int urh_center_chain(urh_ctx* ctx, const float* d_qad, int64_t n, const UrhTileStats* ts, int64_t max_size, int rank, int world,
                     const UrhFine* fine, CenterPlan** d_plan_out);
int urh_center_plan_result(urh_ctx* ctx, const CenterPlan* plan, const float** d_centerf, const double** d_center, const int** d_state);
int urh_center_plan_certify_stats(urh_ctx* ctx, const CenterPlan* plan, int64_t* h_dst3);

extern "C" int urh_shard_digitize(urh_ctx* ctx, const void* d_iq, int dtype, const float* d_qad_in, int64_t n, int has_halo,
                                  float noise_mag, int mod_type, float center, uint16_t tolerance, uint32_t samples_per_symbol,
                                  uint8_t bits_per_symbol, float center_spacing, float* d_qad_out, int64_t global_offset,
                                  int64_t n_total, int64_t* k) {
    URH_CHECK(pulses_begin(ctx, k));
    if (n <= 0) URH_FAIL(ctx, URH_ERR_INVALID, "empty shard");
    if (mod_type != URH_MOD_ASK && mod_type != URH_MOD_FSK) URH_FAIL(ctx, URH_ERR_INVALID, "sharded path: ASK / FSK only");
    if (!d_qad_in && urh_iq_bytes(dtype) == 0) URH_FAIL(ctx, URH_ERR_DTYPE, "Unsupported dtype");
    if (!ctx->nccl_comm) URH_FAIL(ctx, URH_ERR_INVALID, "NCCL communicator not initialised (urh_nccl_init)");
    urh_arena_reset(ctx);
    UrhClassify cls;
    URH_CHECK(fill_classify(ctx, &cls, mod_type, center, bits_per_symbol, center_spacing));
    UrhDigitizer dz;
    URH_CHECK(dz.init(ctx, n, tolerance, mod_type == URH_MOD_ASK, samples_per_symbol, urh_div_up(n, URH_TILE), true));
    if (d_qad_in) {
        URH_PROF_BEGIN(ctx);
        URH_CHECK(launch_dense_qad(ctx, dz, d_qad_in, 0, n, cls));
        URH_PROF_END(ctx);
    } else {
        const UrhDemodParams dp = make_demod_params(noise_mag, mod_type, dtype);
        URH_CHECK(launch_dense_iq(ctx, dtype, mod_type, d_iq, n, dp, cls, DensePass{d_qad_out, &dz, has_halo}));
    }
    return finish_tiles(ctx, dz, FinishShard::shard(ctx, dz, global_offset, n_total), k);
}

struct CenterMail {
    double center;
    int state, pad;
    int64_t cert[3];
    int64_t kept;
    unsigned int redone;
};
static_assert(40 * sizeof(int64_t) + sizeof(CenterMail) <= 64 * sizeof(int64_t), "CenterMail outgrows the mailbox");

struct StreamCenter {
    int ring;
    int64_t chunk_samples;
    const void* h_iq;
    float* h_qad;
    int64_t* kept;
};

struct CenterStep {
    const void* d_iq;
    int dtype, mod_type, has_halo;
    int64_t n, ntiles;
    float* d_qad;
    UrhDemodParams dp;
    UrhClassify cls;
    UrhTileStats* ts;
    UrhFine fine;
    bool speculate;
    UrhSpec spec;
    UrhDigitizer dz;
};

static int center_setup(urh_ctx* ctx, CenterStep& S, bool certify, bool tables, const char* forced_guess, int tol, uint32_t sps) {
    URH_CHECK(urh_arena(ctx, (size_t)S.ntiles, &S.ts));
    if (certify) {
        S.fine.slab_tiles = urh_div_up(S.ntiles, URH_FINE_SLABS);
        if (S.fine.slab_tiles < URH_WARPS_PER_BLOCK) S.fine.slab_tiles = URH_WARPS_PER_BLOCK;
        const int64_t nslabs = urh_div_up(S.ntiles, S.fine.slab_tiles);
        URH_CHECK(urh_arena(ctx, (size_t)(nslabs * URH_FINE_NB), &S.fine.gh));
        URH_CUDA(ctx, cudaMemsetAsync(S.fine.gh, 0, (size_t)(nslabs * URH_FINE_NB) * sizeof(unsigned int), ctx->stream));
        S.fine.scale = (S.mod_type == URH_MOD_FSK) ? 512.0f : 4096.0f;
        S.fine.off = (S.mod_type == URH_MOD_FSK) ? 2048.0f : 0.0f;
    }
    S.cls.noise_value = urh_noise_value(S.mod_type);
    S.cls.order = 2;
    if (tables) URH_CHECK(S.dz.init(ctx, S.n, tol, S.mod_type == URH_MOD_ASK, sps, S.ntiles, false));
    if (S.speculate) {
        float* tg;
        URH_CHECK(urh_arena(ctx, 1, &tg));
        URH_CHECK(urh_arena(ctx, 1, &S.spec.redone));
        URH_CHECK(urh_arena(ctx, (size_t)S.ntiles, &S.spec.margin));
        S.spec.tg = tg;
        URH_LAUNCH(ctx, k_speculate_guess, 1, URH_GUESS_THREADS, 0, (const float2*)S.d_iq, S.n, S.dp.noise_sqrd, forced_guess ? 1 : 0,
                   forced_guess ? strtof(forced_guess, nullptr) : 0.0f, tg, S.spec.redone);
    }
    return URH_OK;
}

static int center_demod(urh_ctx* ctx, CenterStep& S, int64_t t0, int64_t t1) {
    DensePass o{S.d_qad, nullptr, S.has_halo, S.ts, t0, t1, S.fine};
    if (S.speculate) {
        o.dz = &S.dz;
        o.spec = &S.spec;
    }
    return launch_dense_iq(ctx, S.dtype, S.mod_type, S.d_iq, S.n, S.dp, S.cls, o);
}

static int center_demod_host(urh_ctx* ctx, CenterStep& S, const void* h_iq, int64_t chunk_samples) {
    const int64_t chunk_tiles = chunk_samples >= URH_TILE ? chunk_samples / URH_TILE : 1;
    const size_t sample_bytes = (size_t)urh_iq_bytes(S.dtype);
    int chunk_no = 0;
    for (int64_t t0 = 0; t0 < S.ntiles; t0 += chunk_tiles, chunk_no++) {
        const int64_t t1 = (t0 + chunk_tiles < S.ntiles) ? t0 + chunk_tiles : S.ntiles;
        const int64_t s0 = t0 * URH_TILE, s1 = (t1 * URH_TILE < S.n) ? t1 * URH_TILE : S.n;
        cudaEvent_t ev = ctx->ev_copy[chunk_no & 1];
        URH_CUDA(ctx, cudaMemcpyAsync((char*)S.d_iq + (size_t)s0 * sample_bytes, (const char*)h_iq + (size_t)s0 * sample_bytes,
                                      (size_t)(s1 - s0) * sample_bytes, cudaMemcpyHostToDevice, ctx->copy_stream[0]));
        URH_CUDA(ctx, cudaEventRecord(ev, ctx->copy_stream[0]));
        URH_CUDA(ctx, cudaStreamWaitEvent(ctx->stream, ev, 0));
        URH_CHECK(center_demod(ctx, S, t0, t1));
    }
    return URH_OK;
}

static int center_demod_ring(urh_ctx* ctx, CenterStep& S, const StreamCenter& sc, int tol, StreamRing& R, int64_t* cs) {
    const StreamSizes z = stream_sizes(S.n, S.dtype, tol, sc.chunk_samples, sc.ring, URH_STREAM_ENTRY_DEMOD_CENTER_DIGITIZE);
    *cs = z.cs;
    const int64_t slot = r256(z.src_slot);
    URH_CHECK(R.init(ctx, sc.ring, sc.ring * slot));
    std::vector<UrhWindow> win;
    URH_CHECK(urh_filter_windows(URH_FILTER_TILES, S.n, S.n, 1, 0, sc.chunk_samples, nullptr, nullptr, 0, win));
    return stream_run(ctx, win, R, (const char*)sc.h_iq, urh_iq_bytes(S.dtype), R.mem, slot, sc.h_qad != nullptr,
                      [&](int64_t, const UrhWindow& w, int s) {
                          return stream_dense_iq(ctx, S.dtype, S.mod_type, R.mem + s * slot, S.n, S.dp, S.cls, w,
                                                 DensePass{S.d_qad, nullptr, 0, S.ts, 0, -1, S.fine});
                      },
                      [&](int64_t, const UrhWindow& w, int, cudaStream_t cp) {
                          URH_CUDA(ctx, cudaMemcpyAsync(sc.h_qad + w.k0, S.d_qad + w.k0, (size_t)(w.k1 - w.k0) * sizeof(float),
                                                        cudaMemcpyDeviceToHost, cp));
                          return URH_OK;
                      },
                      place_after_pad, true);
}

static int center_copy_results(urh_ctx* ctx, const CenterPlan* plan, CenterMail* mail) {
    const double* d_center;
    const int* d_state;
    urh_center_plan_result(ctx, plan, nullptr, &d_center, &d_state);
    URH_CUDA(ctx, cudaMemcpyAsync(&mail->center, d_center, sizeof(double), cudaMemcpyDeviceToHost, ctx->stream));
    URH_CUDA(ctx, cudaMemcpyAsync(&mail->state, d_state, sizeof(int), cudaMemcpyDeviceToHost, ctx->stream));
    return urh_center_plan_certify_stats(ctx, plan, mail->cert);
}

static int center_digitize_resident(urh_ctx* ctx, CenterStep& S, const CenterPlan* plan, const FinishShard& sh, CenterMail* mail,
                                    int64_t* rows) {
    const float* d_centerf;
    urh_center_plan_result(ctx, plan, &d_centerf, nullptr, nullptr);
    URH_CUDA(ctx, cudaMemsetAsync(S.dz.d_init, 0, 16, ctx->stream));
    const int vec_in = (((uintptr_t)S.d_qad % 8) == 0) ? 1 : 0;
    int64_t grid = urh_div_up(S.ntiles, URH_WARPS_PER_BLOCK);
    if (S.speculate) {
        int per_sm = 0;
        URH_CUDA(ctx, cudaOccupancyMaxActiveBlocksPerMultiprocessor(&per_sm, k_dense_f32<SrcQad2, float>, URH_WARPS_PER_BLOCK * 32, 0));
        const int64_t resident = (int64_t)ctx->sm_count * (per_sm > 0 ? per_sm : 1);
        if (grid > resident) grid = resident;
    }
    URH_LAUNCH(ctx, (k_dense_f32<SrcQad2, float>), (unsigned)grid, URH_WARPS_PER_BLOCK * 32, 0, (const float*)S.d_qad, S.n, vec_in, S.cls,
               S.dz.tol, S.dz.tiles, S.dz.staging, S.dz.cap, S.dz.d_init, 0, d_centerf, (const UrhTileStats*)S.ts, S.spec);
    URH_CHECK(center_copy_results(ctx, plan, mail));
    mail->redone = 0u;
    if (S.speculate) URH_CUDA(ctx, cudaMemcpyAsync(&mail->redone, S.spec.redone, sizeof(unsigned int), cudaMemcpyDeviceToHost, ctx->stream));
    return finish_tiles(ctx, S.dz, sh, rows);
}

static int center_digitize_chunked(urh_ctx* ctx, CenterStep& S, const CenterPlan* plan, int64_t cs, int tol, uint32_t sps,
                                   CenterMail* mail, int64_t* rows) {
    URH_CHECK(center_copy_results(ctx, plan, mail));
    URH_CUDA(ctx, cudaMemcpyAsync(&mail->kept, (const int64_t*)ctx->center_prefix + S.ntiles, sizeof(int64_t), cudaMemcpyDeviceToHost,
                                  ctx->stream));
    URH_CUDA(ctx, cudaStreamSynchronize(ctx->stream));
    if (mail->state != 1) return URH_OK;
    const float* d_centerf;
    urh_center_plan_result(ctx, plan, &d_centerf, nullptr, nullptr);
    StreamDigitizer sd;
    URH_CHECK(sd.init(ctx, S.n, cs, tol, S.mod_type == URH_MOD_ASK, sps));
    for (int64_t s0 = 0; s0 < S.n; s0 += cs) {
        const int64_t s1 = s0 + cs < S.n ? s0 + cs : S.n;
        URH_CHECK(launch_dense_qad(ctx, sd.dz, S.d_qad + s0, s0, s1, S.cls, d_centerf, S.ts));
        URH_CHECK(sd.finish(ctx, s0, s1));
    }
    *rows = sd.rows;
    return URH_OK;
}

static int demod_center_digitize_impl(urh_ctx* ctx, const void* d_iq, int dtype, int64_t n, int has_halo, float noise_mag, int mod_type,
                                      uint16_t tolerance, uint32_t samples_per_symbol, int64_t max_size, float* d_qad_out, bool sharded,
                                      int64_t global_offset, int64_t n_total, double* center, int* center_state, int64_t* k,
                                      const void* h_iq = nullptr, int64_t chunk_samples = 0, const StreamCenter* sc = nullptr) {
    URH_CHECK(pulses_begin(ctx, k, center && center_state));
    *center = 0.0;
    *center_state = 0;
    if (n <= 2 || (mod_type != URH_MOD_ASK && mod_type != URH_MOD_FSK) || !d_qad_out)
        URH_FAIL(ctx, URH_ERR_INVALID, "demod_center_digitize: ASK/FSK, n > 2 and a qad buffer are required");
    if (urh_iq_bytes(dtype) == 0) URH_FAIL(ctx, URH_ERR_DTYPE, "Unsupported dtype");
    if (sharded && !ctx->nccl_comm) URH_FAIL(ctx, URH_ERR_INVALID, "NCCL communicator not initialised (urh_nccl_init)");
    const bool no_certify = getenv("URH_B200_CENTER_NO_CERTIFY") != nullptr, no_speculate = getenv("URH_B200_NO_SPECULATE") != nullptr;
    const char* forced_guess = getenv("URH_B200_SPECULATE_GUESS");
    urh_arena_reset(ctx);
    URH_TL_RESET(ctx);
    URH_TL_MARK(ctx, "step start");
    CenterStep S = {};
    S.d_iq = d_iq; S.dtype = dtype; S.mod_type = mod_type; S.has_halo = has_halo;
    S.n = n; S.ntiles = urh_div_up(n, URH_TILE);
    S.d_qad = d_qad_out;
    S.dp = make_demod_params(noise_mag, mod_type, dtype);
    S.speculate = !sharded && !h_iq && !sc && mod_type == URH_MOD_FSK && dtype == URH_DT_F32 && !no_speculate;
    URH_CHECK(center_setup(ctx, S, !sharded && !no_certify, !sc, forced_guess, tolerance, samples_per_symbol));

    StreamRing ring;
    int64_t cs = 0;
    if (sc) URH_CHECK(center_demod_ring(ctx, S, *sc, tolerance, ring, &cs));
    else if (h_iq) URH_CHECK(center_demod_host(ctx, S, h_iq, chunk_samples));
    else URH_CHECK(center_demod(ctx, S, 0, S.ntiles));

    CenterPlan* plan = nullptr;
    URH_CHECK(urh_center_chain(ctx, d_qad_out, n, S.ts, max_size, sharded ? ctx->nccl_rank : 0, sharded ? ctx->nccl_world : 1,
                               S.fine.gh ? &S.fine : nullptr, &plan));

    CenterMail* mail = (CenterMail*)(ctx->h_mail + 40);
    int64_t rows = 0;
    if (sc)
        URH_CHECK(center_digitize_chunked(ctx, S, plan, cs, tolerance, samples_per_symbol, mail, &rows));
    else
        URH_CHECK(center_digitize_resident(ctx, S, plan, sharded ? FinishShard::shard(ctx, S.dz, global_offset, n_total) : FinishShard::local(S.dz),
                                           mail, &rows));

    *center = mail->center;
    *center_state = mail->state;
    if (sc) *sc->kept = mail->kept;
    ctx->center_cert[0] = mail->cert[0];
    ctx->center_cert[1] = S.fine.gh ? URH_FINE_NB : 0;
    ctx->center_cert[2] = mail->cert[2];
    const int64_t redone = (S.spec.hi > S.spec.lo) ? mail->redone : 0;
    ctx->spec_stats[0] = S.spec.hi - S.spec.lo;
    ctx->spec_stats[1] = S.spec.hi - S.spec.lo - redone;
    ctx->spec_stats[2] = redone;
    if (mail->state != 1) {
        ctx->pulses_k = 0;
        rows = 0;
    }
    *k = rows;
    return URH_OK;
}

extern "C" int urh_speculate_stats(urh_ctx* ctx, int64_t* h_out3) {
    for (int i = 0; i < 3; i++) h_out3[i] = ctx->spec_stats[i];
    return URH_OK;
}

extern "C" int urh_demod_center_digitize(urh_ctx* ctx, const void* d_iq, int dtype, int64_t n, float noise_mag, int mod_type,
                                         uint16_t tolerance, uint32_t samples_per_symbol, int64_t max_size, float* d_qad_out,
                                         double* center, int* center_state, int64_t* k) {
    return demod_center_digitize_impl(ctx, d_iq, dtype, n, 0, noise_mag, mod_type, tolerance, samples_per_symbol, max_size, d_qad_out, false,
                                      0, n, center, center_state, k);
}

extern "C" int urh_demod_center_digitize_host(urh_ctx* ctx, const void* h_iq, int dtype, int64_t n, float noise_mag, int mod_type,
                                              uint16_t tolerance, uint32_t samples_per_symbol, int64_t max_size, int64_t chunk_samples,
                                              void* d_iq_scratch, float* d_qad_out, double* center, int* center_state, int64_t* k) {
    if (!h_iq || !d_iq_scratch) return URH_ERR_INVALID;
    URH_CUDA(ctx, cudaEventRecord(ctx->ev_comp[0], ctx->stream));
    URH_CUDA(ctx, cudaStreamWaitEvent(ctx->copy_stream[0], ctx->ev_comp[0], 0));
    return demod_center_digitize_impl(ctx, d_iq_scratch, dtype, n, 0, noise_mag, mod_type, tolerance, samples_per_symbol, max_size, d_qad_out,
                                      false, 0, n, center, center_state, k, h_iq, chunk_samples > 0 ? chunk_samples : ((int64_t)1 << 24));
}

extern "C" int urh_shard_demod_center_digitize_host(urh_ctx* ctx, const void* h_iq, int dtype, int64_t n, int has_halo, float noise_mag,
                                                    int mod_type, uint16_t tolerance, uint32_t samples_per_symbol, int64_t max_size,
                                                    int64_t chunk_samples, void* d_iq_scratch, float* d_qad_out, int64_t global_offset,
                                                    int64_t n_total, double* center, int* center_state, int64_t* k) {
    if (!h_iq || !d_iq_scratch) return URH_ERR_INVALID;
    URH_CUDA(ctx, cudaEventRecord(ctx->ev_comp[0], ctx->stream));
    URH_CUDA(ctx, cudaStreamWaitEvent(ctx->copy_stream[0], ctx->ev_comp[0], 0));
    return demod_center_digitize_impl(ctx, d_iq_scratch, dtype, n, has_halo, noise_mag, mod_type, tolerance, samples_per_symbol, max_size,
                                      d_qad_out, true, global_offset, n_total, center, center_state, k, h_iq,
                                      chunk_samples > 0 ? chunk_samples : ((int64_t)1 << 24));
}

extern "C" int urh_shard_demod_center_digitize(urh_ctx* ctx, const void* d_iq, int dtype, int64_t n, int has_halo, float noise_mag,
                                               int mod_type, uint16_t tolerance, uint32_t samples_per_symbol, int64_t max_size,
                                               float* d_qad_out, int64_t global_offset, int64_t n_total, double* center,
                                               int* center_state, int64_t* k) {
    return demod_center_digitize_impl(ctx, d_iq, dtype, n, has_halo, noise_mag, mod_type, tolerance, samples_per_symbol, max_size, d_qad_out,
                                      true, global_offset, n_total, center, center_state, k);
}

extern "C" int urh_afp_demod_stream(urh_ctx* ctx, const void* h_iq, int dtype, int64_t n, float noise_mag, int mod_type, int64_t chunk_samples,
                                    int ring, float* h_qad) {
    if (!h_iq || !h_qad) return URH_ERR_INVALID;
    URH_CHECK(stream_check(ctx, n, ring, mod_type, dtype, true));
    urh_arena_reset(ctx);
    const StreamSizes z = stream_sizes(n, dtype, 0, chunk_samples, ring, URH_STREAM_ENTRY_AFP_DEMOD);
    StreamRing R;
    URH_CHECK(R.init(ctx, ring, z.ring_bytes));
    char* d_src = R.mem;
    float* d_qad = (float*)(R.mem + ring * r256(z.src_slot));
    const UrhDemodParams dp = make_demod_params(noise_mag, mod_type, dtype);
    UrhClassify cls;
    memset(&cls, 0, sizeof(cls));
    std::vector<UrhWindow> win;
    URH_CHECK(urh_filter_windows(URH_FILTER_TILES, n, n, 1, 0, chunk_samples, nullptr, nullptr, 0, win));
    return stream_run(ctx, win, R, (const char*)h_iq, urh_iq_bytes(dtype), d_src, r256(z.src_slot), true,
                      [&](int64_t, const UrhWindow& w, int s) {
                          return stream_dense_iq(ctx, dtype, mod_type, d_src + s * r256(z.src_slot), n, dp, cls, w,
                                                 DensePass{d_qad + s * z.cs - w.k0});
                      },
                      contiguous_download(ctx, (const char*)d_qad, z.cs * 4, (char*)h_qad, 4), place_after_pad);
}

extern "C" int urh_grab_pulse_lens_stream(urh_ctx* ctx, const float* qad, int qad_on_device, int64_t n, float center, uint16_t tolerance,
                                          int mod_type, uint32_t samples_per_symbol, uint8_t bits_per_symbol, float center_spacing,
                                          int64_t chunk_samples, int ring, int64_t* k) {
    URH_CHECK(pulses_begin(ctx, k, qad != nullptr));
    URH_CHECK(stream_check(ctx, n, ring, mod_type, 0, false));
    urh_arena_reset(ctx);
    UrhClassify cls;
    URH_CHECK(fill_classify(ctx, &cls, mod_type, center, bits_per_symbol, center_spacing));
    const StreamSizes z = stream_sizes(n, 0, tolerance, chunk_samples, ring,
                                       URH_STREAM_ENTRY_GRAB_PULSE_LENS | (qad_on_device ? URH_STREAM_QAD_ON_DEVICE : 0));
    StreamRing R;
    URH_CHECK(R.init(ctx, ring, z.ring_bytes));
    StreamDigitizer sd;
    URH_CHECK(sd.init(ctx, n, z.cs, tolerance, mod_type == URH_MOD_ASK, samples_per_symbol));
    char* d_src = R.mem;
    std::vector<UrhWindow> win;
    URH_CHECK(urh_filter_windows(URH_FILTER_TILES, n, n, 0, 0, chunk_samples, nullptr, nullptr, 0, win));
    URH_CHECK(stream_run(ctx, win, R, qad_on_device ? nullptr : (const char*)qad, 4, d_src, r256(z.src_slot), false,
                         [&](int64_t, const UrhWindow& w, int s) {
                             const float* x = qad_on_device ? qad + w.k0 : (const float*)(d_src + s * r256(z.src_slot) + URH_STREAM_PAD);
                             URH_CHECK(launch_dense_qad(ctx, sd.dz, x, w.k0, w.k1, cls));
                             return sd.finish(ctx, w.k0, w.k1);
                         },
                         no_download, place_after_pad));
    *k = sd.rows;
    return URH_OK;
}

extern "C" int urh_demod_digitize_stream(urh_ctx* ctx, const void* h_iq, int dtype, int64_t n, float noise_mag, int mod_type, float center,
                                         uint16_t tolerance, uint32_t samples_per_symbol, uint8_t bits_per_symbol, float center_spacing,
                                         int64_t chunk_samples, int ring, float* h_qad_out, int64_t* k) {
    URH_CHECK(pulses_begin(ctx, k, h_iq != nullptr));
    URH_CHECK(stream_check(ctx, n, ring, mod_type, dtype, true));
    urh_arena_reset(ctx);
    UrhClassify cls;
    URH_CHECK(fill_classify(ctx, &cls, mod_type, center, bits_per_symbol, center_spacing));
    const UrhDemodParams dp = make_demod_params(noise_mag, mod_type, dtype);
    const StreamSizes z = stream_sizes(n, dtype, tolerance, chunk_samples, ring,
                                       URH_STREAM_ENTRY_DEMOD_DIGITIZE | (h_qad_out ? URH_STREAM_QAD_OUT : 0));
    StreamRing R;
    URH_CHECK(R.init(ctx, ring, z.ring_bytes));
    StreamDigitizer sd;
    URH_CHECK(sd.init(ctx, n, z.cs, tolerance, mod_type == URH_MOD_ASK, samples_per_symbol));
    char* d_src = R.mem;
    float* d_qad = h_qad_out ? (float*)(R.mem + ring * r256(z.src_slot)) : nullptr;
    std::vector<UrhWindow> win;
    URH_CHECK(urh_filter_windows(URH_FILTER_TILES, n, n, 1, 0, chunk_samples, nullptr, nullptr, 0, win));
    URH_CHECK(stream_run(ctx, win, R, (const char*)h_iq, urh_iq_bytes(dtype), d_src, r256(z.src_slot), h_qad_out != nullptr,
                         [&](int64_t, const UrhWindow& w, int s) {
                             URH_CHECK(stream_dense_iq(ctx, dtype, mod_type, d_src + s * r256(z.src_slot), n, dp, cls, w,
                                                       DensePass{d_qad ? d_qad + s * z.cs - w.k0 : nullptr, &sd.dz}));
                             return sd.finish(ctx, w.k0, w.k1);
                         },
                         contiguous_download(ctx, (const char*)d_qad, z.cs * 4, (char*)h_qad_out, 4), place_after_pad));
    *k = sd.rows;
    return URH_OK;
}

extern "C" int urh_demod_center_digitize_stream(urh_ctx* ctx, const void* h_iq, int dtype, int64_t n, float noise_mag, int mod_type,
                                                uint16_t tolerance, uint32_t samples_per_symbol, int64_t max_size, int64_t chunk_samples,
                                                int ring, float* d_qad_out, float* h_qad_out, double* center, int* center_state,
                                                int64_t* kept, int64_t* k) {
    if (!h_iq || !d_qad_out || !kept) return URH_ERR_INVALID;
    URH_CHECK(stream_check(ctx, n, ring, mod_type, dtype, true));
    StreamCenter sc;
    sc.ring = ring; sc.chunk_samples = chunk_samples; sc.h_iq = h_iq; sc.h_qad = h_qad_out; sc.kept = kept;
    return demod_center_digitize_impl(ctx, nullptr, dtype, n, 0, noise_mag, mod_type, tolerance, samples_per_symbol, max_size, d_qad_out,
                                      false, 0, n, center, center_state, k, nullptr, 0, &sc);
}

extern "C" int urh_afp_demod_psk_stream(urh_ctx* ctx, const void* h_iq, int dtype, int64_t n, float noise_mag, int mod_order,
                                        float costas_loop_bandwidth, int64_t chunk_samples, int ring, float* h_qad) {
    if (!h_iq || !h_qad) return URH_ERR_INVALID;
    URH_CHECK(psk_stream_check(ctx, n, ring, dtype));
    urh_arena_reset(ctx);
    const StreamSizes z = stream_sizes(n, dtype, 0, chunk_samples, ring, URH_STREAM_ENTRY_AFP_DEMOD | psk_entry_flags(mod_order));
    StreamRing R;
    URH_CHECK(R.init(ctx, ring, z.ring_bytes));
    const int64_t slot = r256(z.src_slot);
    char* d_src = R.mem;
    float* d_qad = (float*)(R.mem + ring * slot);
    const UrhDemodParams dp = make_demod_params(noise_mag, URH_MOD_PSK, dtype);
    UrhCostasStream cs;
    URH_CHECK(urh_costas_stream_begin(ctx, &cs));
    const UrhArenaMark mark = urh_arena_mark(ctx);
    std::vector<UrhWindow> win;
    URH_CHECK(urh_filter_windows(URH_FILTER_TILES, n, n, 0, 0, chunk_samples, nullptr, nullptr, 0, win));
    URH_CHECK(stream_run(ctx, win, R, (const char*)h_iq, urh_iq_bytes(dtype), d_src, slot, true,
                         [&](int64_t c, const UrhWindow& w, int s) {
                             urh_arena_release(ctx, mark);
                             return urh_costas_stream_chunk(ctx, &cs, c, d_src + s * slot + URH_STREAM_PAD, dtype, w.k1 - w.k0, dp.noise_sqrd,
                                                            mod_order, costas_loop_bandwidth, d_qad + s * z.cs);
                         },
                         contiguous_download(ctx, (const char*)d_qad, z.cs * 4, (char*)h_qad, 4), place_after_pad));
    return urh_costas_stream_end(ctx, &cs);
}

extern "C" int urh_demod_digitize_psk_stream(urh_ctx* ctx, const void* h_iq, int dtype, int64_t n, float noise_mag, float center,
                                             uint16_t tolerance, uint32_t samples_per_symbol, uint8_t bits_per_symbol, float center_spacing,
                                             int64_t chunk_samples, int ring, float* h_qad_out, int64_t* k) {
    URH_CHECK(pulses_begin(ctx, k, h_iq != nullptr));
    URH_CHECK(psk_stream_check(ctx, n, ring, dtype));
    urh_arena_reset(ctx);
    UrhClassify cls;
    URH_CHECK(fill_classify(ctx, &cls, URH_MOD_PSK, center, bits_per_symbol, center_spacing));
    const int mod_order = 1 << bits_per_symbol;
    const UrhDemodParams dp = make_demod_params(noise_mag, URH_MOD_PSK, dtype);
    const StreamSizes z = stream_sizes(n, dtype, tolerance, chunk_samples, ring,
                                       URH_STREAM_ENTRY_DEMOD_DIGITIZE | (h_qad_out ? URH_STREAM_QAD_OUT : 0) | psk_entry_flags(mod_order));
    StreamRing R;
    URH_CHECK(R.init(ctx, ring, z.ring_bytes));
    const int64_t slot = r256(z.src_slot);
    char* d_src = R.mem;
    float* d_qad = (float*)(R.mem + ring * slot);
    UrhCostasStream cs;
    URH_CHECK(urh_costas_stream_begin(ctx, &cs));
    StreamDigitizer sd;
    URH_CHECK(sd.init(ctx, n, z.cs, tolerance, false, samples_per_symbol));
    std::vector<UrhWindow> win;
    URH_CHECK(urh_filter_windows(URH_FILTER_TILES, n, n, 0, 0, chunk_samples, nullptr, nullptr, 0, win));
    URH_CHECK(stream_run(ctx, win, R, (const char*)h_iq, urh_iq_bytes(dtype), d_src, slot, h_qad_out != nullptr,
                         [&](int64_t c, const UrhWindow& w, int s) {
                             urh_arena_release(ctx, sd.mark);
                             float* q = d_qad + s * z.cs;
                             URH_CHECK(urh_costas_stream_chunk(ctx, &cs, c, d_src + s * slot + URH_STREAM_PAD, dtype, w.k1 - w.k0, dp.noise_sqrd,
                                                               mod_order, 0.1f, q));
                             URH_CHECK(launch_dense_qad(ctx, sd.dz, q, w.k0, w.k1, cls));
                             return sd.finish(ctx, w.k0, w.k1);
                         },
                         contiguous_download(ctx, (const char*)d_qad, z.cs * 4, (char*)h_qad_out, 4), place_after_pad));
    *k = sd.rows;
    return urh_costas_stream_end(ctx, &cs);
}

struct UrhShardState {
    UrhCandidates cand;
};
static UrhShardState* shard_state(urh_ctx* ctx) {
    if (!ctx->shard_state) ctx->shard_state = calloc(1, sizeof(UrhShardState));
    return (UrhShardState*)ctx->shard_state;
}

extern "C" int urh_shard_candidates(urh_ctx* ctx, int carry_valid, int carry_cls, int64_t carry_len, int64_t global_offset,
                                    int64_t* count, const int64_t** d_pos, const int16_t** d_cls, int* last_cand_cls) {
    if (!ctx->shard_tiles) URH_FAIL(ctx, URH_ERR_INVALID, "urh_segment_shard_pass must precede urh_shard_candidates");
    UrhShardCarry in;
    in.valid = carry_valid; in.cls = carry_cls; in.len = carry_len;
    UrhShardState* S = shard_state(ctx);
    URH_CHECK(urh_collect_candidates_shard(ctx, ctx->shard_n, ctx->shard_tol, (const UrhTileSummary*)ctx->shard_tiles,
                                           (const uint32_t*)ctx->shard_staging, ctx->shard_cap, in, global_offset, &S->cand));
    *count = S->cand.count;
    if (d_pos) *d_pos = S->cand.pos;
    if (d_cls) *d_cls = S->cand.cls;
    if (last_cand_cls) {
        *last_cand_cls = 0;
        if (S->cand.count > 0) {
            int16_t v = 0;
            URH_CUDA(ctx, cudaMemcpyAsync(&v, S->cand.cls + S->cand.count - 1, sizeof(v), cudaMemcpyDeviceToHost, ctx->stream));
            URH_CUDA(ctx, cudaStreamSynchronize(ctx->stream));
            *last_cand_cls = v;
        }
    }
    ctx->shard_tiles = nullptr;
    return URH_OK;
}

extern "C" int urh_fetch_candidates(urh_ctx* ctx, int64_t* h_pos, int16_t* h_cls, int64_t count) {
    UrhShardState* S = shard_state(ctx);
    if (count < 0 || count > S->cand.count) URH_FAIL(ctx, URH_ERR_INVALID, "fetch_candidates: count exceeds the table");
    if (count == 0) return URH_OK;
    URH_CUDA(ctx, cudaMemcpyAsync(h_pos, S->cand.pos, (size_t)count * sizeof(int64_t), cudaMemcpyDeviceToHost, ctx->stream));
    URH_CUDA(ctx, cudaMemcpyAsync(h_cls, S->cand.cls, (size_t)count * sizeof(int16_t), cudaMemcpyDeviceToHost, ctx->stream));
    URH_CUDA(ctx, cudaStreamSynchronize(ctx->stream));
    return URH_OK;
}

extern "C" int urh_fetch_pulses(urh_ctx* ctx, int64_t* h_rows, int64_t k) {
    if (k < 0 || k > ctx->pulses_k) URH_FAIL(ctx, URH_ERR_INVALID, "fetch_pulses: k=%lld exceeds last result %lld", (long long)k, (long long)ctx->pulses_k);
    if (k == 0) return URH_OK;
    URH_CUDA(ctx, cudaMemcpyAsync(h_rows, ctx->pulses, (size_t)k * 2 * sizeof(int64_t), cudaMemcpyDeviceToHost, ctx->stream));
    URH_CUDA(ctx, cudaStreamSynchronize(ctx->stream));
    return URH_OK;
}

extern "C" int urh_pulses_device_ptr(urh_ctx* ctx, const int64_t** d_rows, int64_t* k) {
    if (d_rows) *d_rows = ctx->pulses;
    if (k) *k = ctx->pulses_k;
    return URH_OK;
}


__global__ void k_selftest_div(uint64_t seed, int64_t count, unsigned long long* mismatches, unsigned long long* tested) {
    const int64_t stride = (int64_t)gridDim.x * blockDim.x;
    unsigned long long bad = 0, ok = 0;
    for (int64_t i = (int64_t)blockIdx.x * blockDim.x + threadIdx.x; i < count; i += stride) {
        uint64_t h = seed + (uint64_t)i * 0x9E3779B97F4A7C15ull;
        h = (h ^ (h >> 30)) * 0xBF58476D1CE4E5B9ull;
        h = (h ^ (h >> 27)) * 0x94D049BB133111EBull;
        h ^= h >> 31;
        uint64_t g = h * 0xD6E8FEB86659FD93ull + 0x632BE59BD9B4E019ull;
        g ^= g >> 29;
        const uint32_t span = URH_DIVWIN_HI - URH_DIVWIN_LO;
        uint32_t ea = URH_DIVWIN_LO + (uint32_t)((h >> 40) % span), eb = URH_DIVWIN_LO + (uint32_t)((g >> 40) % span);
        uint32_t ma = (uint32_t)h & 0x7fffff, mb = (uint32_t)g & 0x7fffff;
        if ((i & 15) == 1) ma = 0;
        if ((i & 15) == 2) mb = 0;
        if ((i & 15) == 3) { ma = 0x7fffff; }
        if ((i & 15) == 4) { mb = 0x7fffff; }
        if ((i & 15) == 5) { eb = ea; }
        float a0 = __uint_as_float((ea << 23) | ma), b0 = __uint_as_float((eb << 23) | mb);
        float a1 = __uint_as_float(((URH_DIVWIN_LO + (uint32_t)((g >> 12) % span)) << 23) | ((uint32_t)(h >> 9) & 0x7fffff));
        float b1 = __uint_as_float(((URH_DIVWIN_LO + (uint32_t)((h >> 12) % span)) << 23) | ((uint32_t)(g >> 9) & 0x7fffff));
        if ((i & 15) == 6) { a1 = __uint_as_float((URH_DIVWIN_LO << 23)); b1 = __uint_as_float(((URH_DIVWIN_HI - 1) << 23) | 0x7fffff); }
        if ((i & 15) == 8) { b1 = __uint_as_float((URH_DIVWIN_LO << 23)); a1 = __uint_as_float(((URH_DIVWIN_HI - 1) << 23) | 0x7fffff); }
        if ((i & 63) == 7) a1 = 0.0f;
        const float2 q = urh_div2_window(make_float2(a0, a1), make_float2(b0, b1));
        const float r0 = __fdiv_rn(a0, b0), r1 = __fdiv_rn(a1, b1);
        bad += (__float_as_uint(q.x) != __float_as_uint(r0)) + (__float_as_uint(q.y) != __float_as_uint(r1));
        ok += 2;
    }
    atomicAdd(mismatches, bad);
    atomicAdd(tested, ok);
}

extern "C" int urh_selftest_packed_div(urh_ctx* ctx, uint64_t seed, int64_t count, int64_t* mismatches, int64_t* tested) {
    urh_arena_reset(ctx);
    unsigned long long* d;
    URH_CHECK(urh_arena(ctx, 2, &d));
    URH_CUDA(ctx, cudaMemsetAsync(d, 0, 16, ctx->stream));
    URH_LAUNCH(ctx, k_selftest_div, (unsigned)(ctx->sm_count * 8), 256, 0, seed, count, d, d + 1);
    int64_t h[2];
    URH_CHECK(urh_read_i64(ctx, (const int64_t*)d, 2, h));
    *mismatches = h[0];
    *tested = h[1];
    return URH_OK;
}
```

urh_b200/csrc/finish.cu:

```cuda
#include "sparse.cuh"
#include "tilescan.cuh"

#include <limits.h>

#define CLS_NONE INT_MIN

struct __align__(16) CandAgg {
    int64_t cnt;
    int32_t last_cls;
    int32_t pad;
};
struct CandOp {
    __device__ __forceinline__ CandAgg operator()(const CandAgg& a, const CandAgg& b) const {
        CandAgg r;
        r.cnt = a.cnt + b.cnt;
        r.last_cls = (b.last_cls != CLS_NONE) ? b.last_cls : a.last_cls;
        r.pad = 0;
        return r;
    }
};
struct __align__(16) FireAgg {
    int64_t fired;
    int64_t last_pos;
};
struct FireOp {
    __device__ __forceinline__ FireAgg operator()(const FireAgg& a, const FireAgg& b) const {
        FireAgg r;
        r.fired = a.fired + b.fired;
        r.last_pos = (b.last_pos >= 0) ? b.last_pos : a.last_pos;
        return r;
    }
};

struct ScanRunCarry : TileRuns {
    RunCarry* carry;
    __device__ __forceinline__ void post(int64_t t, const RunCarry& excl, const RunCarry&) const { carry[t] = excl; }
};

struct __align__(16) TileFire {
    int32_t first_cls;
    int32_t first_rel;
    int32_t fired;
    int32_t last_rel;
};
struct ScanCandidates {
    const UrhTileSummary* tiles;
    const uint32_t* staging;
    int stage_cap;
    const RunCarry* carry;
    const RunCarry* xcarry;
    int tol;
    int32_t* head_rel;
    int32_t* prev_cls;
    TileFire* fire;
    __device__ __forceinline__ CandAgg load(int64_t t) const {
        const UrhTileSummary s = tiles[t];
        RunCarry c = carry[t];
        if (xcarry) c = RunCarryOp()(*xcarry, c);
        int64_t start_len = 0;
        if (!(c.flags & 2) && c.cls == s.first_cls) start_len = c.len;
        int32_t rel = -1;
        if (start_len <= tol && (int64_t)tol < start_len + s.head_len) rel = (int32_t)(tol - start_len);
        head_rel[t] = rel;
        TileFire f;
        f.first_cls = CLS_NONE; f.first_rel = -1; f.fired = 0; f.last_rel = -1;
        int prev = CLS_NONE;
        if (rel >= 0) {
            prev = s.first_cls;
            f.first_cls = prev;
            f.first_rel = rel;
        }
        const uint32_t* st = staging + t * (int64_t)stage_cap;
        for (int j = 0; j < s.ncand; j += 4) {
            uint32_t w[4];
#pragma unroll
            for (int u = 0; u < 4; u++) w[u] = (j + u < s.ncand) ? st[j + u] : 0u;
#pragma unroll
            for (int u = 0; u < 4; u++) {
                if (j + u < s.ncand) {
                    const int cl = (int)(w[u] & 0xffffu) - 1;
                    const int p = (int)(w[u] >> 16);
                    if (prev == CLS_NONE) {
                        f.first_cls = cl;
                        f.first_rel = p;
                    } else if (cl != prev) {
                        f.fired++;
                        f.last_rel = p;
                    }
                    prev = cl;
                }
            }
        }
        fire[t] = f;
        CandAgg r;
        r.cnt = (int64_t)s.ncand + (rel >= 0 ? 1 : 0);
        r.last_cls = prev;
        r.pad = 0;
        return r;
    }
    __device__ __forceinline__ void post(int64_t t, const CandAgg& excl, const CandAgg&) const { prev_cls[t] = excl.last_cls; }
};

struct ScanFirings {
    const TileFire* fire;
    const int32_t* prev_cls;
    const int16_t* d_prev0;
    int64_t global_offset;
    int64_t* row_off;
    int64_t* prev_fired;
    __device__ __forceinline__ FireAgg load(int64_t t) const {
        const TileFire f = fire[t];
        int prev = prev_cls[t];
        if (prev == CLS_NONE) prev = *d_prev0;
        FireAgg r;
        r.fired = f.fired;
        int32_t last = f.last_rel;
        if (f.first_cls != CLS_NONE && f.first_cls != prev) {
            r.fired++;
            if (last < 0) last = f.first_rel;
        }
        r.last_pos = (last >= 0) ? t * URH_TILE + global_offset + last : -1;
        return r;
    }
    __device__ __forceinline__ void post(int64_t t, const FireAgg& excl, const FireAgg&) const {
        row_off[t] = excl.fired;
        prev_fired[t] = excl.last_pos;
    }
};

constexpr int FIN_TILES = 32;
constexpr int FIN_BATCH = 8;

struct FinRows {
    int64_t* out;
    int64_t cap_rows;
    int tol;
    int is_ask;
    int64_t sps;
};

struct FinWalk {
    int prev;
    int64_t pp;
    int64_t idx;
};

__device__ __forceinline__ void fin_row(const FinRows& R, int64_t idx, int64_t p, int64_t pp, int prev) {
    const int64_t rec = (pp >= 0) ? (p - pp) : (p + 1 - R.tol);
    int64_t st = prev;
    if (R.is_ask && st == -1 && rec < R.sps) st = 0;
    if (idx < R.cap_rows) *((longlong2*)R.out + idx) = make_longlong2(st, rec);
}

__device__ __forceinline__ void fin_chunk(FinWalk& W, uint32_t w, int cnt, int lane, int64_t base, const FinRows& R) {
    const int c = (int)(w & 0xffffu) - 1;
    const int rel = (int)(w >> 16);
    int pc = __shfl_up_sync(URH_FULL_MASK, c, 1);
    if (lane == 0) pc = W.prev;
    const bool fire = lane < cnt && c != pc;
    const unsigned fm = __ballot_sync(URH_FULL_MASK, fire);
    const unsigned lower = fm & ((1u << lane) - 1u);
    const int before = __shfl_sync(URH_FULL_MASK, rel, lower ? 31 - __clz(lower) : 0);
    if (fire) fin_row(R, W.idx + __popc(lower), base + rel, lower ? base + before : W.pp, pc);
    if (fm) W.pp = base + __shfl_sync(URH_FULL_MASK, rel, 31 - __clz(fm));
    W.idx += __popc(fm);
    if (cnt > 0) W.prev = __shfl_sync(URH_FULL_MASK, c, cnt - 1);
}

__global__ void __launch_bounds__(256) k_finish_rows(const UrhTileSummary* __restrict__ tiles, const uint32_t* __restrict__ staging,
                                                    int stage_cap, const int32_t* __restrict__ head_rel, const int32_t* __restrict__ prev_cls,
                                                    const int16_t* __restrict__ d_prev0, const int64_t* __restrict__ row_off,
                                                    const int64_t* __restrict__ prev_fired, const int64_t* __restrict__ d_xprev_fired,
                                                    int64_t ntiles, int64_t global_offset, int64_t n_total, int tol, int is_ask, int64_t sps,
                                                    int emit_tail, int64_t row_base, int64_t* __restrict__ out, int64_t cap_rows,
                                                    int64_t* __restrict__ d_out) {
    const int64_t t0 = ((int64_t)blockIdx.x * blockDim.x + threadIdx.x) / 32 * FIN_TILES;
    if (t0 >= ntiles) return;
    const int lane = threadIdx.x & 31;
    FinRows R;
    R.out = out; R.cap_rows = cap_rows; R.tol = tol; R.is_ask = is_ask; R.sps = sps;
    const int64_t tl = t0 + lane;
    int l_first = 0, l_ncand = 0, l_rel = -1, l_prev = 0;
    int64_t l_idx = 0, l_pp = -1;
    if (tl < ntiles) {
        const UrhTileSummary s = tiles[tl];
        l_first = s.first_cls;
        l_ncand = s.ncand;
        l_rel = head_rel[tl];
        l_prev = prev_cls[tl];
        if (l_prev == CLS_NONE) l_prev = *d_prev0;
        l_idx = row_off[tl];
        l_pp = prev_fired[tl];
        if (l_pp < 0) l_pp = *d_xprev_fired;
    }
    for (int j0 = 0; j0 < FIN_TILES && t0 + j0 < ntiles; j0 += FIN_BATCH) {
        uint32_t w0[FIN_BATCH];
#pragma unroll
        for (int u = 0; u < FIN_BATCH; u++) {
            const int nc = __shfl_sync(URH_FULL_MASK, l_ncand, j0 + u);
            w0[u] = (lane < nc) ? __ldg(staging + (t0 + j0 + u) * (int64_t)stage_cap + lane) : 0u;
        }
#pragma unroll
        for (int u = 0; u < FIN_BATCH; u++) {
            const int j = j0 + u;
            const int64_t t = t0 + j;
            if (t >= ntiles) break;
            const int64_t base = t * URH_TILE + global_offset;
            const int ncand = __shfl_sync(URH_FULL_MASK, l_ncand, j);
            const int rel = __shfl_sync(URH_FULL_MASK, l_rel, j);
            FinWalk W;
            W.prev = __shfl_sync(URH_FULL_MASK, l_prev, j);
            W.pp = __shfl_sync(URH_FULL_MASK, l_pp, j);
            W.idx = __shfl_sync(URH_FULL_MASK, l_idx, j);
            if (rel >= 0) {
                const int c = __shfl_sync(URH_FULL_MASK, l_first, j);
                if (c != W.prev) {
                    if (lane == 0) fin_row(R, W.idx, base + rel, W.pp, W.prev);
                    W.idx++;
                    W.pp = base + rel;
                }
                W.prev = c;
            }
            const uint32_t* st = staging + t * (int64_t)stage_cap;
            for (int k = 0; k < ncand; k += 32) {
                const uint32_t w = (k == 0) ? w0[u] : ((k + lane < ncand) ? __ldg(st + k + lane) : 0u);
                fin_chunk(W, w, min(32, ncand - k), lane, base, R);
            }
            if (t == ntiles - 1 && lane == 0) {
                int64_t idx = W.idx;
                const int64_t fired = idx;
                if (emit_tail && (is_ask || row_base + fired < n_total)) {
                    if (idx < cap_rows) *((longlong2*)out + idx) = make_longlong2(W.prev, (W.pp >= 0) ? (n_total - 1 - W.pp) : (n_total - tol));
                    idx++;
                }
                d_out[0] = idx;
                d_out[1] = fired;
            }
        }
    }
}

struct ScanMergeRows {
    const int64_t* raw;
    int64_t rows;
    int64_t n_total;
    int has_tail;
    int64_t* out;
    int64_t* d_k;
    const int64_t* prev_last;
    int64_t row_base;
    __device__ __forceinline__ int64_t load(int64_t r) const {
        if (r == 0) return (prev_last && raw[0] == *prev_last) ? 0 : 1;
        return raw[2 * r] != raw[2 * r - 2] ? 1 : 0;
    }
    __device__ __forceinline__ void post(int64_t r, const int64_t& excl, const int64_t& head) const {
        const bool is_tail = has_tail && r == rows - 1;
        if (is_tail && row_base + excl >= n_total) {
            *d_k = excl;
            return;
        }
        const int64_t o = excl + head - 1;
        if (head) out[2 * o] = raw[2 * r];
        atomicAdd((unsigned long long*)&out[2 * o + 1], (unsigned long long)raw[2 * r + 1]);
        if (r == rows - 1) *d_k = o + 1;
    }
};
struct AddI64 {
    __device__ __forceinline__ int64_t operator()(int64_t a, int64_t b) const { return a + b; }
};

__global__ void k_pack_stage1(const int16_t* __restrict__ d_init, const RunCarry* __restrict__ total, int64_t* __restrict__ msg) {
    memcpy(msg, total, sizeof(RunCarry));
    msg[2] = *d_init;
    msg[3] = 0;
}
__global__ void k_fold_carry(const int64_t* __restrict__ all, int rank, RunCarry* __restrict__ xcarry) {
    RunCarry acc;
    acc.len = 0; acc.cls = 0; acc.flags = 2 | 1;
    for (int q = 0; q < rank; q++) {
        RunCarry c;
        memcpy(&c, all + 4 * q, sizeof(c));
        acc = RunCarryOp()(acc, c);
    }
    if (rank == 0) acc.flags = 2;
    else acc.flags &= ~1;
    *xcarry = acc;
}
__global__ void k_fold_prev_cls(const int64_t* __restrict__ all, int rank, const int64_t* __restrict__ stage1, int16_t* __restrict__ prev0) {
    int v = (int)stage1[2];
    for (int q = 0; q < rank; q++) {
        CandAgg c;
        memcpy(&c, all + 2 * q, sizeof(c));
        if (c.last_cls != CLS_NONE) v = c.last_cls;
    }
    *prev0 = (int16_t)v;
}
__global__ void k_fold_prev_fired(const int64_t* __restrict__ all, int rank, int64_t* __restrict__ xprev) {
    int64_t v = -1;
    for (int q = 0; q < rank; q++) {
        FireAgg c;
        memcpy(&c, all + 2 * q, sizeof(c));
        if (c.last_pos >= 0) v = c.last_pos;
    }
    *xprev = v;
}

__global__ void k_chain_start(const int16_t* __restrict__ d_init, UrhChain* __restrict__ chain) {
    chain->run.len = 0; chain->run.cls = 0; chain->run.flags = 2 | 1;
    chain->prev_fired = -1;
    chain->last_state = INT64_MIN;
    chain->prev_cls = *d_init;
}
__global__ void k_chain_advance(UrhChain* __restrict__ chain, const RunCarry* __restrict__ tot_run, const CandAgg* __restrict__ tot_cand,
                                const FireAgg* __restrict__ tot_fire) {
    chain->run = RunCarryOp()(chain->run, *tot_run);
    if (tot_cand->last_cls != CLS_NONE) chain->prev_cls = (int16_t)tot_cand->last_cls;
    if (tot_fire->last_pos >= 0) chain->prev_fired = tot_fire->last_pos;
}
__global__ void k_chain_last_row(UrhChain* __restrict__ chain, const int64_t* __restrict__ table, int64_t rows) {
    if (rows > 0) chain->last_state = table[2 * (rows - 1)];
}

int finish_tiles(urh_ctx* ctx, const UrhDigitizer& dz, const FinishShard& sh, int64_t* k) {
    const int64_t n = sh.n;
    const int64_t ntiles = urh_div_up(n, URH_TILE);
    const bool sharded = sh.world > 1;
    UrhChain* chain = sh.chain;
    RunCarry* carry;
    int32_t *head_rel, *prev_cls;
    int64_t *row_off, *prev_fired, *d_small;
    URH_CHECK(urh_arena(ctx, (size_t)ntiles, &carry));
    URH_CHECK(urh_arena(ctx, (size_t)ntiles, &head_rel));
    URH_CHECK(urh_arena(ctx, (size_t)ntiles, &prev_cls));
    URH_CHECK(urh_arena(ctx, (size_t)ntiles, &row_off));
    URH_CHECK(urh_arena(ctx, (size_t)ntiles, &prev_fired));
    TileFire* fire;
    URH_CHECK(urh_arena(ctx, (size_t)ntiles, &fire));
    URH_CHECK(urh_arena(ctx, (size_t)(32 + 8 * (sharded ? sh.world : 0)), &d_small));
    URH_CUDA(ctx, cudaMemsetAsync(d_small, 0xff, 4 * sizeof(int64_t), ctx->stream));
    RunCarry* d_tot_run = (RunCarry*)(d_small + 4);
    CandAgg* d_tot_cand = (CandAgg*)(d_small + 6);
    FireAgg* d_tot_fire = (FireAgg*)(d_small + 8);
    RunCarry* d_xcarry = (RunCarry*)(d_small + 10);
    int16_t* d_prev0 = (int16_t*)(d_small + 12);
    int64_t* d_xprev = d_small + 13;
    int64_t* d_msg1 = d_small + 16;
    int64_t* d_all1 = d_small + 32;
    int64_t* d_all2 = d_all1 + 4 * (sharded ? sh.world : 0);
    int64_t* d_all3 = d_all2 + 2 * (sharded ? sh.world : 0);

    if (chain && sh.global_offset == 0) URH_LAUNCH(ctx, k_chain_start, 1, 1, 0, dz.d_init, chain);
    RunCarry rc_ident;
    rc_ident.len = 0; rc_ident.cls = 0; rc_ident.flags = 2 | 1;
    ScanRunCarry fa;
    fa.tiles = dz.tiles; fa.n = n; fa.carry = carry;
    URH_CHECK((urhts::scan<RunCarry, RunCarryOp, ScanRunCarry>(ctx, ntiles, rc_ident, RunCarryOp(), fa, d_tot_run)));
    if (sharded) {
        URH_LAUNCH(ctx, k_pack_stage1, 1, 1, 0, dz.d_init, (const RunCarry*)d_tot_run, d_msg1);
        URH_TL_MARK(ctx, "x4 run carry: enter");
        URH_CHECK(urh_nccl_allgather(ctx, d_msg1, d_all1, 4 * sizeof(int64_t)));
        URH_TL_MARK(ctx, "x4 run carry: done");
        URH_LAUNCH(ctx, k_fold_carry, 1, 1, 0, (const int64_t*)d_all1, sh.rank, d_xcarry);
    }
    ScanCandidates fb;
    fb.tiles = dz.tiles; fb.staging = dz.staging; fb.stage_cap = dz.cap; fb.carry = carry;
    fb.xcarry = sharded ? d_xcarry : (chain ? &chain->run : nullptr);
    fb.tol = dz.tol; fb.head_rel = head_rel; fb.prev_cls = prev_cls; fb.fire = fire;
    CandAgg ca_ident;
    ca_ident.cnt = 0; ca_ident.last_cls = CLS_NONE; ca_ident.pad = 0;
    URH_CHECK((urhts::scan<CandAgg, CandOp, ScanCandidates, 4>(ctx, ntiles, ca_ident, CandOp(), fb, d_tot_cand)));
    const int16_t* prev0 = chain ? &chain->prev_cls : dz.d_init;
    if (sharded) {
        URH_TL_MARK(ctx, "x5 candidates: enter");
        URH_CHECK(urh_nccl_allgather(ctx, d_tot_cand, d_all2, sizeof(CandAgg)));
        URH_TL_MARK(ctx, "x5 candidates: done");
        URH_LAUNCH(ctx, k_fold_prev_cls, 1, 1, 0, (const int64_t*)d_all2, sh.rank, (const int64_t*)d_all1, d_prev0);
        prev0 = d_prev0;
    }
    ScanFirings fc;
    fc.fire = fire; fc.prev_cls = prev_cls; fc.d_prev0 = prev0; fc.global_offset = sh.global_offset; fc.row_off = row_off;
    fc.prev_fired = prev_fired;
    FireAgg fi_ident;
    fi_ident.fired = 0; fi_ident.last_pos = -1;
    URH_CHECK((urhts::scan<FireAgg, FireOp, ScanFirings>(ctx, ntiles, fi_ident, FireOp(), fc, d_tot_fire)));
    const int64_t* xprev = chain ? &chain->prev_fired : d_small + 2;
    if (sharded) {
        URH_TL_MARK(ctx, "x6 firings: enter");
        URH_CHECK(urh_nccl_allgather(ctx, d_tot_fire, d_all3, sizeof(FireAgg)));
        URH_TL_MARK(ctx, "x6 firings: done");
        URH_LAUNCH(ctx, k_fold_prev_fired, 1, 1, 0, (const int64_t*)d_all3, sh.rank, d_xprev);
        xprev = d_xprev;
    }

    int64_t cap_rows = (int64_t)ctx->pulses_cap_rows;
    const int64_t guess = n / 64 + 1024;
    if (!chain && cap_rows < guess) {
        URH_CHECK(urh_ensure_pulses(ctx, (size_t)guess));
        cap_rows = (int64_t)ctx->pulses_cap_rows;
    }
    const int64_t row_base = chain ? sh.row_base : 0;
    int64_t* raw = ctx->pulses + 2 * row_base;
    int64_t raw_cap = chain ? sh.rows_cap : cap_rows;
    if (dz.is_ask) URH_CHECK(urh_arena(ctx, (size_t)raw_cap * 2, &raw));
    int64_t got[2] = {0, 0};
    for (int attempt = 0; attempt < 2; attempt++) {
        URH_LAUNCH(ctx, k_finish_rows, (unsigned)urh_div_up(ntiles, 8 * FIN_TILES), 256, 0, dz.tiles, dz.staging, dz.cap, (const int32_t*)head_rel,
                   (const int32_t*)prev_cls, prev0, (const int64_t*)row_off, (const int64_t*)prev_fired, xprev, ntiles, sh.global_offset,
                   sh.n_total, dz.tol, dz.is_ask ? 1 : 0, (int64_t)dz.sps, sh.emit_tail, row_base, raw, raw_cap, d_small);
        if (sharded && attempt == 0) URH_TL_MARK(ctx, "rows written");
        URH_CHECK(urh_read_i64(ctx, d_small, 2, got));
        if (got[0] <= raw_cap) break;
        if (attempt == 1 || chain) URH_FAIL(ctx, URH_ERR_CUDA, "finish_tiles: row buffer overflow after regrowth");
        if (dz.is_ask) {
            URH_CHECK(urh_arena(ctx, (size_t)got[0] * 2, &raw));
            raw_cap = got[0];
        } else {
            URH_CHECK(urh_ensure_pulses(ctx, (size_t)got[0]));
            raw = ctx->pulses;
            raw_cap = (int64_t)ctx->pulses_cap_rows;
        }
    }
    if (chain) URH_LAUNCH(ctx, k_chain_advance, 1, 1, 0, chain, (const RunCarry*)d_tot_run, (const CandAgg*)d_tot_cand, (const FireAgg*)d_tot_fire);
    int64_t K = got[0];
    if (dz.is_ask && K > 0) {
        if (!chain) URH_CHECK(urh_ensure_pulses(ctx, (size_t)K));
        int64_t* out = ctx->pulses + 2 * row_base;
        URH_CUDA(ctx, cudaMemsetAsync(out, 0, (size_t)K * 2 * sizeof(int64_t), ctx->stream));
        ScanMergeRows fm;
        fm.raw = raw; fm.rows = K; fm.n_total = sh.n_total; fm.has_tail = (sh.emit_tail && K > got[1]) ? 1 : 0; fm.out = out;
        fm.d_k = d_small;
        fm.prev_last = (chain && row_base > 0) ? &chain->last_state : nullptr;
        fm.row_base = row_base;
        URH_CHECK((urhts::scan<int64_t, AddI64, ScanMergeRows>(ctx, K, (int64_t)0, AddI64(), fm, (int64_t*)nullptr)));
        URH_CHECK(urh_read_i64(ctx, d_small, 1, &K));
        if (chain) URH_LAUNCH(ctx, k_chain_last_row, 1, 1, 0, chain, (const int64_t*)ctx->pulses, row_base + K);
    }
    ctx->pulses_k = row_base + K;
    *k = K;
    return URH_OK;
}
```

Measured before the change: 217,300.

## Parallelize small single-block kernels, fuse scans, and cut host round-trips

Several unrelated changes land together. Binary searches over the tile prefix become warp-cooperative 32-way searches, and the certify and guess kernels go from one block to many blocks with a last-block ticket reduction. The candidate and firing scans are fused into a single scan for the unsharded case, and the finish-rows kernel is restructured with shared-memory row staging. Memsets are folded into kernels, and result readback now goes through mapped host memory and one combined copy. The aim is to remove serial single-thread or single-block latency and launch or copy overhead, at the cost of more complex inter-block synchronization.

```diff
diff --git a/urh_b200/csrc/center.cu b/urh_b200/csrc/center.cu
--- a/urh_b200/csrc/center.cu
+++ b/urh_b200/csrc/center.cu
@@ -416,21 +416,26 @@
     plan->straddle = 0;
 }
 
-__device__ __forceinline__ int64_t cen_tile_of_rank(const int64_t* __restrict__ prefix, int64_t ntiles, int64_t r) {
+__device__ __forceinline__ int64_t cen_tile_of_rank(const int64_t* __restrict__ prefix, int64_t ntiles, int64_t r, int lane) {
     int64_t lo = 0, hi = ntiles;
     while (hi - lo > 1) {
-        const int64_t mid = (lo + hi) >> 1;
-        if (prefix[mid] <= r) lo = mid; else hi = mid;
+        const int64_t step = (hi - lo + 31) / 32;
+        const int64_t p = lo + (int64_t)(lane + 1) * step;
+        const bool le = p < hi && prefix[p] <= r;
+        const int k = __popc(__ballot_sync(URH_FULL_MASK, le));
+        const int64_t nhi = lo + (int64_t)(k + 1) * step;
+        lo += (int64_t)k * step;
+        if (nhi < hi) hi = nhi;
     }
     return lo;
 }
 
 __device__ __forceinline__ void cen_window_tiles(const int64_t* __restrict__ prefix, int64_t ntiles, long long r0, long long r1,
-                                                 long long (&w)[4]) {
+                                                 long long (&w)[4], int lane) {
     long long w0 = -1, w1 = -1, w2 = -1, w3 = -1;
     if (r1 > r0) {
-        w0 = cen_tile_of_rank(prefix, ntiles, r0);
-        w1 = cen_tile_of_rank(prefix, ntiles, r1 - 1);
+        w0 = cen_tile_of_rank(prefix, ntiles, r0, lane);
+        w1 = cen_tile_of_rank(prefix, ntiles, r1 - 1, lane);
         const bool cov0 = prefix[w0] >= r0 && prefix[w0 + 1] <= r1;
         const bool cov1 = prefix[w1] >= r0 && prefix[w1 + 1] <= r1;
         w2 = cov0 ? -1 : w0;
@@ -446,11 +451,13 @@
     __shared__ int s_pre[256];
     __shared__ bool s_last;
     const long long r0 = plan->lr0, r1 = plan->lr1;
-    if (threadIdx.x == 0) {
+    if (threadIdx.x < 32) {
         long long w[4];
-        cen_window_tiles(prefix, ntiles, r0, r1, w);
-        s_win[0] = w[0]; s_win[1] = w[1]; s_win[2] = w[2]; s_win[3] = w[3];
-        if (blockIdx.x == 0) { plan->win[0] = w[0]; plan->win[1] = w[1]; plan->win[2] = w[2]; plan->win[3] = w[3]; }
+        cen_window_tiles(prefix, ntiles, r0, r1, w, threadIdx.x);
+        if (threadIdx.x == 0) {
+            s_win[0] = w[0]; s_win[1] = w[1]; s_win[2] = w[2]; s_win[3] = w[3];
+            if (blockIdx.x == 0) { plan->win[0] = w[0]; plan->win[1] = w[1]; plan->win[2] = w[2]; plan->win[3] = w[3]; }
+        }
     }
     __syncthreads();
     double sum = 0.0, sq = 0.0;
@@ -608,26 +615,39 @@
 }
 
 #define CERT_THREADS 512
+#define CERT_BLOCKS (URH_FINE_NB / CERT_THREADS)
 __global__ void __launch_bounds__(CERT_THREADS) k_center_certify(const UrhFine fine, CenterPlan* __restrict__ plan, const float* __restrict__ fe,
                                                                  const unsigned long long* __restrict__ xhist, unsigned long long* __restrict__ lo,
-                                                                 unsigned long long* __restrict__ hi) {
+                                                                 unsigned long long* __restrict__ hi, unsigned long long* __restrict__ buckets,
+                                                                 unsigned long long* __restrict__ ticket, unsigned long long ticket_base) {
     __shared__ unsigned long long s_ge[URH_FINE_NB + 1];
     __shared__ unsigned long long s_part[CERT_THREADS];
     __shared__ unsigned char s_flag[CEN_MAX_BINS];
     __shared__ unsigned long long s_key[3];
     __shared__ unsigned int s_certain;
-    if (plan->state != 1) return;
+    __shared__ bool s_last;
     const int tid = threadIdx.x;
+    const bool live = plan->state == 1;
+    if (live) {
+        int64_t sf, se;
+        cen_full_slabs(plan->win[0], plan->win[1], fine.slab_tiles, &sf, &se);
+        const int64_t b = (int64_t)blockIdx.x * CERT_THREADS + tid;
+        unsigned long long v = 0;
+        for (int64_t sl = sf; sl < se; sl++) v += fine.gh[sl * URH_FINE_NB + b];
+        buckets[b] = v;
+    }
+    __threadfence();
+    __syncthreads();
+    if (tid == 0) s_last = atomicAdd(ticket, 1ull) - ticket_base == (unsigned long long)gridDim.x - 1;
+    __syncthreads();
+    if (!s_last || !live) return;
+    __threadfence();
     constexpr int PER = URH_FINE_NB / CERT_THREADS;
-    int64_t sf, se;
-    cen_full_slabs(plan->win[0], plan->win[1], fine.slab_tiles, &sf, &se);
     unsigned long long b[PER], tot = 0;
 #pragma unroll
     for (int j = 0; j < PER; j++) {
-        unsigned long long v = 0;
-        for (int64_t sl = sf; sl < se; sl++) v += fine.gh[sl * URH_FINE_NB + tid * PER + j];
-        b[j] = v;
-        tot += v;
+        b[j] = __ldcg(buckets + tid * PER + j);
+        tot += b[j];
     }
     s_part[tid] = tot;
     if (tid < 3) s_key[tid] = 0ull;
@@ -797,18 +817,20 @@
                                                    double hstep, long long nbins, float scale, int fast, CenterPlan* __restrict__ plan,
                                                    float* __restrict__ fe, unsigned long long* __restrict__ hist) {
     const double edge1 = __dadd_rn(hmin, hstep);
-    if (blockIdx.x == 0 && threadIdx.x == 0) {
-        plan->lr0 = r0; plan->lr1 = r1;
-        plan->ticket = 0u;
-        plan->state = 1;
-        plan->certified = 0;
-        if (nbins > 0) {
-            long long w[4];
-            cen_window_tiles(prefix, ntiles, r0, r1, w);
-            for (int i = 0; i < 4; i++) plan->win[i] = w[i];
-            plan->hmin = hmin; plan->edge1 = edge1; plan->delta = hstep; plan->nbins = nbins;
-            plan->scale = scale;
-            plan->fast = fast;
+    if (blockIdx.x == 0 && threadIdx.x < 32) {
+        long long w[4];
+        if (nbins > 0) cen_window_tiles(prefix, ntiles, r0, r1, w, threadIdx.x);
+        if (threadIdx.x == 0) {
+            plan->lr0 = r0; plan->lr1 = r1;
+            plan->ticket = 0u;
+            plan->state = 1;
+            plan->certified = 0;
+            if (nbins > 0) {
+                for (int i = 0; i < 4; i++) plan->win[i] = w[i];
+                plan->hmin = hmin; plan->edge1 = edge1; plan->delta = hstep; plan->nbins = nbins;
+                plan->scale = scale;
+                plan->fast = fast;
+            }
         }
     }
     if (nbins > 0)
@@ -885,7 +907,7 @@
     unsigned long long* hist;
     int64_t* d_counts;
     CenStats* d_parts;
-    unsigned long long *xhist = nullptr, *cert_lo = nullptr, *cert_hi = nullptr;
+    unsigned long long *xhist = nullptr, *cert_lo = nullptr, *cert_hi = nullptr, *cert_buckets = nullptr;
     const int nb = ctx->sm_count * 2;
     URH_CHECK(urh_arena(ctx, (size_t)ntiles + 1, &prefix));
     URH_CHECK(urh_arena(ctx, 1, &plan));
@@ -898,6 +920,7 @@
         URH_CHECK(urh_arena(ctx, (size_t)CEN_MAX_BINS, &xhist));
         URH_CHECK(urh_arena(ctx, (size_t)CEN_MAX_BINS, &cert_lo));
         URH_CHECK(urh_arena(ctx, (size_t)CEN_MAX_BINS, &cert_hi));
+        URH_CHECK(urh_arena(ctx, (size_t)URH_FINE_NB, &cert_buckets));
     }
     URH_CHECK(kept_prefix(ctx, ts, ntiles, prefix));
     const int64_t* counts = prefix + ntiles;
@@ -921,7 +944,12 @@
     const unsigned gs = (unsigned)min(urh_div_up(ntiles, 8), (int64_t)ctx->sm_count * 8);
     URH_LAUNCH(ctx, k_hist_window_ends, fine ? 2 + ctx->sm_count * 4 : 2, 256, fine ? dyn : 0, d_qad, n, (const int64_t*)prefix,
                (const CenterPlan*)plan, (const float*)fe, hist, xhist, fine ? fine->slab_tiles : (int64_t)1);
-    if (fine) URH_LAUNCH(ctx, k_center_certify, 1, CERT_THREADS, 0, *fine, plan, (const float*)fe, (const unsigned long long*)xhist, cert_lo, cert_hi);
+    if (fine) {
+        urhts::Ws ws;
+        URH_CHECK(urhts::prepare(ctx, CERT_BLOCKS, &ws));
+        URH_LAUNCH(ctx, k_center_certify, CERT_BLOCKS, CERT_THREADS, 0, *fine, plan, (const float*)fe, (const unsigned long long*)xhist, cert_lo,
+                   cert_hi, cert_buckets, ws.counter, ws.base);
+    }
     URH_LAUNCH(ctx, (k_hist_interior<true, true, 3>), gs, 256, dyn, d_qad, n, (const CenterPlan*)plan, (const float*)fe, hist, (const int64_t*)prefix, 1);
     URH_LAUNCH(ctx, (k_hist_interior<true, false, 3>), gs, 256, dyn, d_qad, n, (const CenterPlan*)plan, (const float*)fe, hist, (const int64_t*)prefix, 1);
     if (world > 1) {
@@ -938,11 +966,23 @@
     return URH_OK;
 }
 
-int urh_center_plan_certify_stats(urh_ctx* ctx, const CenterPlan* plan, int64_t* h_dst3) {
-    h_dst3[0] = h_dst3[1] = h_dst3[2] = 0;
-    URH_CUDA(ctx, cudaMemcpyAsync(h_dst3, &plan->certified, sizeof(int), cudaMemcpyDeviceToHost, ctx->stream));
-    URH_CUDA(ctx, cudaMemcpyAsync(h_dst3 + 2, &plan->straddle, sizeof(long long), cudaMemcpyDeviceToHost, ctx->stream));
+static constexpr size_t CENTER_RESULT_BYTES = offsetof(CenterPlan, pad) - offsetof(CenterPlan, center);
+static_assert(CENTER_RESULT_BYTES == 40, "CenterPlan: center .. straddle must stay together");
+int urh_center_plan_copy_results(urh_ctx* ctx, const CenterPlan* plan, void* h_dst, cudaStream_t st) {
+    URH_CUDA(ctx, cudaMemcpyAsync(h_dst, &plan->center, CENTER_RESULT_BYTES, cudaMemcpyDeviceToHost, st));
     return URH_OK;
+}
+void urh_center_results_unpack(const void* h_src, double* center, int* state, int64_t* cert3) {
+    const char* b = (const char*)h_src - offsetof(CenterPlan, center);
+    int certified;
+    long long straddle;
+    memcpy(center, b + offsetof(CenterPlan, center), sizeof(double));
+    memcpy(state, b + offsetof(CenterPlan, state), sizeof(int));
+    memcpy(&certified, b + offsetof(CenterPlan, certified), sizeof(int));
+    memcpy(&straddle, b + offsetof(CenterPlan, straddle), sizeof(long long));
+    cert3[0] = certified;
+    cert3[1] = 0;
+    cert3[2] = straddle;
 }
 
 extern "C" int urh_center_certify_stats(urh_ctx* ctx, int64_t* h_out3) {
diff --git a/urh_b200/csrc/digitize.cu b/urh_b200/csrc/digitize.cu
--- a/urh_b200/csrc/digitize.cu
+++ b/urh_b200/csrc/digitize.cu
@@ -134,43 +134,75 @@
 
 #define URH_GUESS_SAMPLES 16384
 #define URH_GUESS_BINS 128
-#define URH_GUESS_THREADS 1024
+#define URH_GUESS_THREADS 256
+#define URH_GUESS_BLOCKS (URH_GUESS_SAMPLES / URH_GUESS_THREADS)
 __global__ void __launch_bounds__(URH_GUESS_THREADS) k_speculate_guess(const float2* __restrict__ iq, int64_t n, float noise_sqrd, int forced,
-                                                                      float forced_tg, float* __restrict__ d_tg, unsigned int* __restrict__ redone) {
+                                                                      float forced_tg, float* __restrict__ d_tg, unsigned int* __restrict__ redone,
+                                                                      float* __restrict__ vals, float2* __restrict__ ranges,
+                                                                      unsigned long long* __restrict__ ticket, unsigned long long ticket_base,
+                                                                      uint4* __restrict__ zero, int64_t zero_words4) {
     constexpr int PER = URH_GUESS_SAMPLES / URH_GUESS_THREADS;
+    constexpr int WARPS = URH_GUESS_THREADS / 32;
     __shared__ unsigned int s_hist[URH_GUESS_BINS];
-    __shared__ float s_mn[32], s_mx[32];
+    __shared__ float s_mn[WARPS], s_mx[WARPS];
+    __shared__ bool s_last;
+    for (int64_t w = (int64_t)blockIdx.x * URH_GUESS_THREADS + threadIdx.x; w < zero_words4; w += (int64_t)gridDim.x * URH_GUESS_THREADS)
+        zero[w] = make_uint4(0u, 0u, 0u, 0u);
+    float mn = INFINITY, mx = -INFINITY;
+    if (!forced) {
+        const int m = blockIdx.x * URH_GUESS_THREADS + threadIdx.x;
+        const int64_t i = 1 + (int64_t)m * (n - 1) / URH_GUESS_SAMPLES;
+        const float2 p = iq[i - 1], c = iq[i];
+        float v = NAN;
+        if (!(c.x * c.x + c.y * c.y <= noise_sqrd)) {
+            v = atan2f(p.x * c.y - p.y * c.x, p.x * c.x + p.y * c.y);
+            mn = fminf(mn, v);
+            mx = fmaxf(mx, v);
+        }
+        vals[m] = v;
+    }
+    for (int off = 16; off > 0; off >>= 1) {
+        mn = fminf(mn, __shfl_xor_sync(URH_FULL_MASK, mn, off));
+        mx = fmaxf(mx, __shfl_xor_sync(URH_FULL_MASK, mx, off));
+    }
+    if ((threadIdx.x & 31) == 0) { s_mn[threadIdx.x >> 5] = mn; s_mx[threadIdx.x >> 5] = mx; }
+    __syncthreads();
+    if (threadIdx.x == 0) {
+        for (int w = 0; w < WARPS; w++) { mn = fminf(mn, s_mn[w]); mx = fmaxf(mx, s_mx[w]); }
+        ranges[blockIdx.x] = make_float2(mn, mx);
+        __threadfence();
+        s_last = atomicAdd(ticket, 1ull) - ticket_base == (unsigned long long)gridDim.x - 1;
+    }
+    __syncthreads();
+    if (!s_last) return;
+    __threadfence();
     if (forced) {
         if (threadIdx.x == 0) { *d_tg = forced_tg; *redone = 0u; }
         return;
     }
-    for (int b = threadIdx.x; b < URH_GUESS_BINS; b += blockDim.x) s_hist[b] = 0u;
-    float v[PER];
-    float mn = INFINITY, mx = -INFINITY;
-#pragma unroll
-    for (int k = 0; k < PER; k++) {
-        const int64_t i = 1 + (int64_t)(k * URH_GUESS_THREADS + threadIdx.x) * (n - 1) / URH_GUESS_SAMPLES;
-        const float2 p = iq[i - 1], c = iq[i];
-        v[k] = NAN;
-        if (!(c.x * c.x + c.y * c.y <= noise_sqrd)) {
-            v[k] = atan2f(p.x * c.y - p.y * c.x, p.x * c.x + p.y * c.y);
-            mn = fminf(mn, v[k]);
-            mx = fmaxf(mx, v[k]);
-        }
+    mn = INFINITY; mx = -INFINITY;
+    for (int b = threadIdx.x; b < URH_GUESS_BLOCKS; b += URH_GUESS_THREADS) {
+        const float2 r = __ldcg(ranges + b);
+        mn = fminf(mn, r.x);
+        mx = fmaxf(mx, r.y);
     }
     for (int off = 16; off > 0; off >>= 1) {
         mn = fminf(mn, __shfl_xor_sync(URH_FULL_MASK, mn, off));
         mx = fmaxf(mx, __shfl_xor_sync(URH_FULL_MASK, mx, off));
     }
+    for (int b = threadIdx.x; b < URH_GUESS_BINS; b += URH_GUESS_THREADS) s_hist[b] = 0u;
+    __syncthreads();
     if ((threadIdx.x & 31) == 0) { s_mn[threadIdx.x >> 5] = mn; s_mx[threadIdx.x >> 5] = mx; }
     __syncthreads();
     mn = INFINITY; mx = -INFINITY;
-    for (int w = 0; w < URH_GUESS_THREADS / 32; w++) { mn = fminf(mn, s_mn[w]); mx = fmaxf(mx, s_mx[w]); }
+    for (int w = 0; w < WARPS; w++) { mn = fminf(mn, s_mn[w]); mx = fmaxf(mx, s_mx[w]); }
     const float width = (mx - mn) / URH_GUESS_BINS;
     if (width > 0.0f) {
 #pragma unroll
-        for (int k = 0; k < PER; k++)
-            if (!isnan(v[k])) atomicAdd(&s_hist[min((int)((v[k] - mn) / width), URH_GUESS_BINS - 1)], 1u);
+        for (int k = 0; k < PER; k++) {
+            const float v = __ldcg(vals + k * URH_GUESS_THREADS + threadIdx.x);
+            if (!isnan(v)) atomicAdd(&s_hist[min((int)((v - mn) / width), URH_GUESS_BINS - 1)], 1u);
+        }
     }
     __syncthreads();
     if (threadIdx.x != 0) return;
@@ -650,7 +682,8 @@
 int urh_center_chain(urh_ctx* ctx, const float* d_qad, int64_t n, const UrhTileStats* ts, int64_t max_size, int rank, int world,
                      const UrhFine* fine, CenterPlan** d_plan_out);
 int urh_center_plan_result(urh_ctx* ctx, const CenterPlan* plan, const float** d_centerf, const double** d_center, const int** d_state);
-int urh_center_plan_certify_stats(urh_ctx* ctx, const CenterPlan* plan, int64_t* h_dst3);
+int urh_center_plan_copy_results(urh_ctx* ctx, const CenterPlan* plan, void* h_dst, cudaStream_t st);
+void urh_center_results_unpack(const void* h_src, double* center, int* state, int64_t* cert3);
 
 extern "C" int urh_shard_digitize(urh_ctx* ctx, const void* d_iq, int dtype, const float* d_qad_in, int64_t n, int has_halo,
                                   float noise_mag, int mod_type, float center, uint16_t tolerance, uint32_t samples_per_symbol,
@@ -678,9 +711,7 @@
 }
 
 struct CenterMail {
-    double center;
-    int state, pad;
-    int64_t cert[3];
+    int64_t plan[5];
     int64_t kept;
     unsigned int redone;
 };
@@ -710,27 +741,36 @@
 
 static int center_setup(urh_ctx* ctx, CenterStep& S, bool certify, bool tables, const char* forced_guess, int tol, uint32_t sps) {
     URH_CHECK(urh_arena(ctx, (size_t)S.ntiles, &S.ts));
+    int64_t fine_words = 0;
     if (certify) {
         S.fine.slab_tiles = urh_div_up(S.ntiles, URH_FINE_SLABS);
         if (S.fine.slab_tiles < URH_WARPS_PER_BLOCK) S.fine.slab_tiles = URH_WARPS_PER_BLOCK;
-        const int64_t nslabs = urh_div_up(S.ntiles, S.fine.slab_tiles);
-        URH_CHECK(urh_arena(ctx, (size_t)(nslabs * URH_FINE_NB), &S.fine.gh));
-        URH_CUDA(ctx, cudaMemsetAsync(S.fine.gh, 0, (size_t)(nslabs * URH_FINE_NB) * sizeof(unsigned int), ctx->stream));
+        fine_words = urh_div_up(S.ntiles, S.fine.slab_tiles) * URH_FINE_NB;
+        URH_CHECK(urh_arena(ctx, (size_t)fine_words, &S.fine.gh));
         S.fine.scale = (S.mod_type == URH_MOD_FSK) ? 512.0f : 4096.0f;
         S.fine.off = (S.mod_type == URH_MOD_FSK) ? 2048.0f : 0.0f;
     }
-    S.cls.noise_value = urh_noise_value(S.mod_type);
-    S.cls.order = 2;
-    if (tables) URH_CHECK(S.dz.init(ctx, S.n, tol, S.mod_type == URH_MOD_ASK, sps, S.ntiles, false));
     if (S.speculate) {
         float* tg;
         URH_CHECK(urh_arena(ctx, 1, &tg));
         URH_CHECK(urh_arena(ctx, 1, &S.spec.redone));
+        S.spec.tg = tg;
+        float* vals;
+        float2* ranges;
+        URH_CHECK(urh_arena(ctx, URH_GUESS_SAMPLES, &vals));
+        URH_CHECK(urh_arena(ctx, URH_GUESS_BLOCKS, &ranges));
+        urhts::Ws ws;
+        URH_CHECK(urhts::prepare(ctx, URH_GUESS_BLOCKS, &ws));
+        URH_LAUNCH(ctx, k_speculate_guess, URH_GUESS_BLOCKS, URH_GUESS_THREADS, 0, (const float2*)S.d_iq, S.n, S.dp.noise_sqrd, forced_guess ? 1 : 0,
+                   forced_guess ? strtof(forced_guess, nullptr) : 0.0f, tg, S.spec.redone, vals, ranges, ws.counter, ws.base,
+                   (uint4*)S.fine.gh, fine_words / 4);
         URH_CHECK(urh_arena(ctx, (size_t)S.ntiles, &S.spec.margin));
-        S.spec.tg = tg;
-        URH_LAUNCH(ctx, k_speculate_guess, 1, URH_GUESS_THREADS, 0, (const float2*)S.d_iq, S.n, S.dp.noise_sqrd, forced_guess ? 1 : 0,
-                   forced_guess ? strtof(forced_guess, nullptr) : 0.0f, tg, S.spec.redone);
-    }
+    } else if (certify) {
+        URH_CUDA(ctx, cudaMemsetAsync(S.fine.gh, 0, (size_t)fine_words * sizeof(unsigned int), ctx->stream));
+    }
+    S.cls.noise_value = urh_noise_value(S.mod_type);
+    S.cls.order = 2;
+    if (tables) URH_CHECK(S.dz.init(ctx, S.n, tol, S.mod_type == URH_MOD_ASK, sps, S.ntiles, false));
     return URH_OK;
 }
 
@@ -741,6 +781,25 @@
         o.spec = &S.spec;
     }
     return launch_dense_iq(ctx, S.dtype, S.mod_type, S.d_iq, S.n, S.dp, S.cls, o);
+}
+
+static int center_demod_resident(urh_ctx* ctx, CenterStep& S) {
+    if (S.ntiles < 2) return center_demod(ctx, S, 0, S.ntiles);
+    cudaStream_t main = ctx->stream, side = ctx->copy_stream[1];
+    URH_CUDA(ctx, cudaEventRecord(ctx->ev_comp[0], main));
+    URH_CUDA(ctx, cudaStreamWaitEvent(side, ctx->ev_comp[0], 0));
+    const int profiling = ctx->profiling;
+    ctx->profiling = 0;
+    ctx->stream = side;
+    const int rc = center_demod(ctx, S, 0, 1);
+    ctx->stream = main;
+    ctx->profiling = profiling;
+    URH_CHECK(rc);
+    URH_CUDA(ctx, cudaEventRecord(ctx->ev_comp[1], side));
+    URH_CHECK(center_demod(ctx, S, 1, S.ntiles));
+    URH_CUDA(ctx, cudaStreamWaitEvent(main, ctx->ev_comp[1], 0));
+    URH_PROF_END(ctx);
+    return URH_OK;
 }
 
 static int center_demod_host(urh_ctx* ctx, CenterStep& S, const void* h_iq, int64_t chunk_samples) {
@@ -780,13 +839,8 @@
                       place_after_pad, true);
 }
 
-static int center_copy_results(urh_ctx* ctx, const CenterPlan* plan, CenterMail* mail) {
-    const double* d_center;
-    const int* d_state;
-    urh_center_plan_result(ctx, plan, nullptr, &d_center, &d_state);
-    URH_CUDA(ctx, cudaMemcpyAsync(&mail->center, d_center, sizeof(double), cudaMemcpyDeviceToHost, ctx->stream));
-    URH_CUDA(ctx, cudaMemcpyAsync(&mail->state, d_state, sizeof(int), cudaMemcpyDeviceToHost, ctx->stream));
-    return urh_center_plan_certify_stats(ctx, plan, mail->cert);
+static int center_copy_results(urh_ctx* ctx, const CenterPlan* plan, CenterMail* mail, cudaStream_t st) {
+    return urh_center_plan_copy_results(ctx, plan, mail->plan, st);
 }
 
 static int center_digitize_resident(urh_ctx* ctx, CenterStep& S, const CenterPlan* plan, const FinishShard& sh, CenterMail* mail,
@@ -804,19 +858,28 @@
     }
     URH_LAUNCH(ctx, (k_dense_f32<SrcQad2, float>), (unsigned)grid, URH_WARPS_PER_BLOCK * 32, 0, (const float*)S.d_qad, S.n, vec_in, S.cls,
                S.dz.tol, S.dz.tiles, S.dz.staging, S.dz.cap, S.dz.d_init, 0, d_centerf, (const UrhTileStats*)S.ts, S.spec);
-    URH_CHECK(center_copy_results(ctx, plan, mail));
+    cudaStream_t cp = ctx->copy_stream[1];
+    URH_CUDA(ctx, cudaEventRecord(ctx->ev_comp[1], ctx->stream));
+    URH_CUDA(ctx, cudaStreamWaitEvent(cp, ctx->ev_comp[1], 0));
+    URH_CHECK(center_copy_results(ctx, plan, mail, cp));
     mail->redone = 0u;
-    if (S.speculate) URH_CUDA(ctx, cudaMemcpyAsync(&mail->redone, S.spec.redone, sizeof(unsigned int), cudaMemcpyDeviceToHost, ctx->stream));
-    return finish_tiles(ctx, S.dz, sh, rows);
+    if (S.speculate) URH_CUDA(ctx, cudaMemcpyAsync(&mail->redone, S.spec.redone, sizeof(unsigned int), cudaMemcpyDeviceToHost, cp));
+    const int rc = finish_tiles(ctx, S.dz, sh, rows);
+    URH_CUDA(ctx, cudaStreamSynchronize(cp));
+    return rc;
 }
 
 static int center_digitize_chunked(urh_ctx* ctx, CenterStep& S, const CenterPlan* plan, int64_t cs, int tol, uint32_t sps,
                                    CenterMail* mail, int64_t* rows) {
-    URH_CHECK(center_copy_results(ctx, plan, mail));
+    URH_CHECK(center_copy_results(ctx, plan, mail, ctx->stream));
     URH_CUDA(ctx, cudaMemcpyAsync(&mail->kept, (const int64_t*)ctx->center_prefix + S.ntiles, sizeof(int64_t), cudaMemcpyDeviceToHost,
                                   ctx->stream));
     URH_CUDA(ctx, cudaStreamSynchronize(ctx->stream));
-    if (mail->state != 1) return URH_OK;
+    double center;
+    int state;
+    int64_t cert[3];
+    urh_center_results_unpack(mail->plan, &center, &state, cert);
+    if (state != 1) return URH_OK;
     const float* d_centerf;
     urh_center_plan_result(ctx, plan, &d_centerf, nullptr, nullptr);
     StreamDigitizer sd;
@@ -858,7 +921,7 @@
     int64_t cs = 0;
     if (sc) URH_CHECK(center_demod_ring(ctx, S, *sc, tolerance, ring, &cs));
     else if (h_iq) URH_CHECK(center_demod_host(ctx, S, h_iq, chunk_samples));
-    else URH_CHECK(center_demod(ctx, S, 0, S.ntiles));
+    else URH_CHECK(center_demod_resident(ctx, S));
 
     CenterPlan* plan = nullptr;
     URH_CHECK(urh_center_chain(ctx, d_qad_out, n, S.ts, max_size, sharded ? ctx->nccl_rank : 0, sharded ? ctx->nccl_world : 1,
@@ -872,17 +935,17 @@
         URH_CHECK(center_digitize_resident(ctx, S, plan, sharded ? FinishShard::shard(ctx, S.dz, global_offset, n_total) : FinishShard::local(S.dz),
                                            mail, &rows));
 
-    *center = mail->center;
-    *center_state = mail->state;
+    int64_t cert[3];
+    urh_center_results_unpack(mail->plan, center, center_state, cert);
     if (sc) *sc->kept = mail->kept;
-    ctx->center_cert[0] = mail->cert[0];
+    ctx->center_cert[0] = cert[0];
     ctx->center_cert[1] = S.fine.gh ? URH_FINE_NB : 0;
-    ctx->center_cert[2] = mail->cert[2];
+    ctx->center_cert[2] = cert[2];
     const int64_t redone = (S.spec.hi > S.spec.lo) ? mail->redone : 0;
     ctx->spec_stats[0] = S.spec.hi - S.spec.lo;
     ctx->spec_stats[1] = S.spec.hi - S.spec.lo - redone;
     ctx->spec_stats[2] = redone;
-    if (mail->state != 1) {
+    if (*center_state != 1) {
         ctx->pulses_k = 0;
         rows = 0;
     }
diff --git a/urh_b200/csrc/finish.cu b/urh_b200/csrc/finish.cu
--- a/urh_b200/csrc/finish.cu
+++ b/urh_b200/csrc/finish.cu
@@ -4,6 +4,9 @@
 #include <limits.h>
 
 #define CLS_NONE INT_MIN
+
+constexpr int FIN_PREFETCH = 8;
+constexpr int FIN_MAIL = 32;
 
 struct __align__(16) CandAgg {
     int64_t cnt;
@@ -43,6 +46,45 @@
     int32_t fired;
     int32_t last_rel;
 };
+__device__ __forceinline__ TileFire walk_tile(const UrhTileSummary& s, const RunCarry& c, int tol, const uint32_t* st, int32_t* rel_out,
+                                              int* last) {
+    int64_t start_len = 0;
+    if (!(c.flags & 2) && c.cls == s.first_cls) start_len = c.len;
+    int32_t rel = -1;
+    if (start_len <= tol && (int64_t)tol < start_len + s.head_len) rel = (int32_t)(tol - start_len);
+    TileFire f;
+    f.first_cls = CLS_NONE; f.first_rel = -1; f.fired = 0; f.last_rel = -1;
+    int prev = CLS_NONE;
+    if (rel >= 0) {
+        prev = s.first_cls;
+        f.first_cls = prev;
+        f.first_rel = rel;
+    }
+    for (int j = 0; j < s.ncand; j += FIN_PREFETCH) {
+        uint32_t w[FIN_PREFETCH];
+#pragma unroll
+        for (int u = 0; u < FIN_PREFETCH; u++) w[u] = (j + u < s.ncand) ? st[j + u] : 0u;
+#pragma unroll
+        for (int u = 0; u < FIN_PREFETCH; u++) {
+            if (j + u < s.ncand) {
+                const int cl = (int)(w[u] & 0xffffu) - 1;
+                const int p = (int)(w[u] >> 16);
+                if (prev == CLS_NONE) {
+                    f.first_cls = cl;
+                    f.first_rel = p;
+                } else if (cl != prev) {
+                    f.fired++;
+                    f.last_rel = p;
+                }
+                prev = cl;
+            }
+        }
+    }
+    *rel_out = rel;
+    *last = prev;
+    return f;
+}
+
 struct ScanCandidates {
     const UrhTileSummary* tiles;
     const uint32_t* staging;
@@ -57,44 +99,13 @@
         const UrhTileSummary s = tiles[t];
         RunCarry c = carry[t];
         if (xcarry) c = RunCarryOp()(*xcarry, c);
-        int64_t start_len = 0;
-        if (!(c.flags & 2) && c.cls == s.first_cls) start_len = c.len;
-        int32_t rel = -1;
-        if (start_len <= tol && (int64_t)tol < start_len + s.head_len) rel = (int32_t)(tol - start_len);
+        int32_t rel;
+        int last;
+        fire[t] = walk_tile(s, c, tol, staging + t * (int64_t)stage_cap, &rel, &last);
         head_rel[t] = rel;
-        TileFire f;
-        f.first_cls = CLS_NONE; f.first_rel = -1; f.fired = 0; f.last_rel = -1;
-        int prev = CLS_NONE;
-        if (rel >= 0) {
-            prev = s.first_cls;
-            f.first_cls = prev;
-            f.first_rel = rel;
-        }
-        const uint32_t* st = staging + t * (int64_t)stage_cap;
-        for (int j = 0; j < s.ncand; j += 4) {
-            uint32_t w[4];
-#pragma unroll
-            for (int u = 0; u < 4; u++) w[u] = (j + u < s.ncand) ? st[j + u] : 0u;
-#pragma unroll
-            for (int u = 0; u < 4; u++) {
-                if (j + u < s.ncand) {
-                    const int cl = (int)(w[u] & 0xffffu) - 1;
-                    const int p = (int)(w[u] >> 16);
-                    if (prev == CLS_NONE) {
-                        f.first_cls = cl;
-                        f.first_rel = p;
-                    } else if (cl != prev) {
-                        f.fired++;
-                        f.last_rel = p;
-                    }
-                    prev = cl;
-                }
-            }
-        }
-        fire[t] = f;
         CandAgg r;
         r.cnt = (int64_t)s.ncand + (rel >= 0 ? 1 : 0);
-        r.last_cls = prev;
+        r.last_cls = last;
         r.pad = 0;
         return r;
     }
@@ -128,116 +139,142 @@
     }
 };
 
-constexpr int FIN_TILES = 32;
-constexpr int FIN_BATCH = 8;
+struct __align__(16) FireSpan {
+    int32_t first_cls;
+    int32_t last_cls;
+    int64_t fired;
+    int64_t first_pos;
+    int64_t last_pos;
+};
+struct FireSpanOp {
+    __device__ __forceinline__ FireSpan operator()(const FireSpan& a, const FireSpan& b) const {
+        if (b.first_cls == CLS_NONE) return a;
+        if (a.first_cls == CLS_NONE) return b;
+        const bool fires = b.first_cls != a.last_cls;
+        FireSpan r;
+        r.first_cls = a.first_cls;
+        r.last_cls = b.last_cls;
+        r.fired = a.fired + b.fired + (fires ? 1 : 0);
+        r.first_pos = a.first_pos;
+        r.last_pos = (b.last_pos >= 0) ? b.last_pos : (fires ? b.first_pos : a.last_pos);
+        return r;
+    }
+};
+struct ScanCandFirings {
+    const UrhTileSummary* tiles;
+    const uint32_t* staging;
+    int stage_cap;
+    const RunCarry* carry;
+    int tol;
+    const int16_t* d_prev0;
+    int32_t* head_rel;
+    int32_t* prev_cls;
+    int64_t* row_off;
+    int64_t* prev_fired;
+    __device__ __forceinline__ FireSpan load(int64_t t) const {
+        const UrhTileSummary s = tiles[t];
+        int32_t rel;
+        int last;
+        const TileFire f = walk_tile(s, carry[t], tol, staging + t * (int64_t)stage_cap, &rel, &last);
+        head_rel[t] = rel;
+        const int64_t base = t * URH_TILE;
+        FireSpan r;
+        r.first_cls = f.first_cls;
+        r.last_cls = last;
+        r.fired = f.fired;
+        r.first_pos = base + f.first_rel;
+        r.last_pos = (f.last_rel >= 0) ? base + f.last_rel : -1;
+        return r;
+    }
+    __device__ __forceinline__ void post(int64_t t, const FireSpan& excl, const FireSpan&) const {
+        if (excl.first_cls == CLS_NONE) {
+            prev_cls[t] = CLS_NONE;
+            row_off[t] = 0;
+            prev_fired[t] = -1;
+            return;
+        }
+        const bool first_fires = excl.first_cls != (int)*d_prev0;
+        prev_cls[t] = excl.last_cls;
+        row_off[t] = excl.fired + (first_fires ? 1 : 0);
+        prev_fired[t] = (excl.last_pos >= 0) ? excl.last_pos : (first_fires ? excl.first_pos : -1);
+    }
+};
+
+constexpr int FIN_THREADS = 128;
+constexpr int FIN_SMEM_ROWS = 2048;
 
 struct FinRows {
-    int64_t* out;
-    int64_t cap_rows;
     int tol;
     int is_ask;
     int64_t sps;
 };
 
-struct FinWalk {
-    int prev;
-    int64_t pp;
-    int64_t idx;
-};
-
-__device__ __forceinline__ void fin_row(const FinRows& R, int64_t idx, int64_t p, int64_t pp, int prev) {
+__device__ __forceinline__ longlong2 fin_row(const FinRows& R, int64_t p, int64_t pp, int prev) {
     const int64_t rec = (pp >= 0) ? (p - pp) : (p + 1 - R.tol);
     int64_t st = prev;
     if (R.is_ask && st == -1 && rec < R.sps) st = 0;
-    if (idx < R.cap_rows) *((longlong2*)R.out + idx) = make_longlong2(st, rec);
-}
-
-__device__ __forceinline__ void fin_chunk(FinWalk& W, uint32_t w, int cnt, int lane, int64_t base, const FinRows& R) {
-    const int c = (int)(w & 0xffffu) - 1;
-    const int rel = (int)(w >> 16);
-    int pc = __shfl_up_sync(URH_FULL_MASK, c, 1);
-    if (lane == 0) pc = W.prev;
-    const bool fire = lane < cnt && c != pc;
-    const unsigned fm = __ballot_sync(URH_FULL_MASK, fire);
-    const unsigned lower = fm & ((1u << lane) - 1u);
-    const int before = __shfl_sync(URH_FULL_MASK, rel, lower ? 31 - __clz(lower) : 0);
-    if (fire) fin_row(R, W.idx + __popc(lower), base + rel, lower ? base + before : W.pp, pc);
-    if (fm) W.pp = base + __shfl_sync(URH_FULL_MASK, rel, 31 - __clz(fm));
-    W.idx += __popc(fm);
-    if (cnt > 0) W.prev = __shfl_sync(URH_FULL_MASK, c, cnt - 1);
-}
-
-__global__ void __launch_bounds__(256) k_finish_rows(const UrhTileSummary* __restrict__ tiles, const uint32_t* __restrict__ staging,
-                                                    int stage_cap, const int32_t* __restrict__ head_rel, const int32_t* __restrict__ prev_cls,
-                                                    const int16_t* __restrict__ d_prev0, const int64_t* __restrict__ row_off,
-                                                    const int64_t* __restrict__ prev_fired, const int64_t* __restrict__ d_xprev_fired,
-                                                    int64_t ntiles, int64_t global_offset, int64_t n_total, int tol, int is_ask, int64_t sps,
-                                                    int emit_tail, int64_t row_base, int64_t* __restrict__ out, int64_t cap_rows,
-                                                    int64_t* __restrict__ d_out) {
-    const int64_t t0 = ((int64_t)blockIdx.x * blockDim.x + threadIdx.x) / 32 * FIN_TILES;
-    if (t0 >= ntiles) return;
-    const int lane = threadIdx.x & 31;
+    return make_longlong2(st, rec);
+}
+
+__global__ void __launch_bounds__(FIN_THREADS) k_finish_rows(const UrhTileSummary* __restrict__ tiles, const uint32_t* __restrict__ staging,
+                                                            int stage_cap, const int32_t* __restrict__ head_rel, const int32_t* __restrict__ prev_cls,
+                                                            const int16_t* __restrict__ d_prev0, const int64_t* __restrict__ row_off,
+                                                            const int64_t* __restrict__ prev_fired, const int64_t* __restrict__ d_xprev_fired,
+                                                            int64_t ntiles, int64_t global_offset, int64_t n_total, int tol, int is_ask, int64_t sps,
+                                                            int emit_tail, int64_t row_base, int64_t* __restrict__ out, int64_t cap_rows,
+                                                            int64_t* __restrict__ d_out) {
+    __shared__ longlong2 s_rows[FIN_SMEM_ROWS];
+    __shared__ int64_t s_end;
+    const int64_t t0 = (int64_t)blockIdx.x * FIN_THREADS;
+    const int64_t t = t0 + threadIdx.x;
+    const int64_t tlast = min(t0 + FIN_THREADS, ntiles) - 1;
+    const int64_t r0 = row_off[t0];
     FinRows R;
-    R.out = out; R.cap_rows = cap_rows; R.tol = tol; R.is_ask = is_ask; R.sps = sps;
-    const int64_t tl = t0 + lane;
-    int l_first = 0, l_ncand = 0, l_rel = -1, l_prev = 0;
-    int64_t l_idx = 0, l_pp = -1;
-    if (tl < ntiles) {
-        const UrhTileSummary s = tiles[tl];
-        l_first = s.first_cls;
-        l_ncand = s.ncand;
-        l_rel = head_rel[tl];
-        l_prev = prev_cls[tl];
-        if (l_prev == CLS_NONE) l_prev = *d_prev0;
-        l_idx = row_off[tl];
-        l_pp = prev_fired[tl];
-        if (l_pp < 0) l_pp = *d_xprev_fired;
-    }
-    for (int j0 = 0; j0 < FIN_TILES && t0 + j0 < ntiles; j0 += FIN_BATCH) {
-        uint32_t w0[FIN_BATCH];
+    R.tol = tol; R.is_ask = is_ask; R.sps = sps;
+    if (t <= tlast) {
+        const UrhTileSummary s = tiles[t];
+        int prev = prev_cls[t];
+        if (prev == CLS_NONE) prev = *d_prev0;
+        int64_t pp = prev_fired[t];
+        if (pp < 0) pp = d_xprev_fired ? *d_xprev_fired : -1;
+        int64_t idx = row_off[t];
+        const int64_t base = t * URH_TILE + global_offset;
+        auto fire = [&](int64_t p, int c) {
+            if (c != prev) {
+                const longlong2 row = fin_row(R, p, pp, prev);
+                if (idx - r0 < FIN_SMEM_ROWS) s_rows[idx - r0] = row;
+                else if (idx < cap_rows) *((longlong2*)out + idx) = row;
+                idx++;
+                pp = p;
+            }
+            prev = c;
+        };
+        const int32_t rel = head_rel[t];
+        if (rel >= 0) fire(base + rel, s.first_cls);
+        const uint32_t* st = staging + t * (int64_t)stage_cap;
+        for (int j = 0; j < s.ncand; j += FIN_PREFETCH) {
+            uint32_t w[FIN_PREFETCH];
 #pragma unroll
-        for (int u = 0; u < FIN_BATCH; u++) {
-            const int nc = __shfl_sync(URH_FULL_MASK, l_ncand, j0 + u);
-            w0[u] = (lane < nc) ? __ldg(staging + (t0 + j0 + u) * (int64_t)stage_cap + lane) : 0u;
-        }
+            for (int u = 0; u < FIN_PREFETCH; u++) w[u] = (j + u < s.ncand) ? __ldg(st + j + u) : 0u;
 #pragma unroll
-        for (int u = 0; u < FIN_BATCH; u++) {
-            const int j = j0 + u;
-            const int64_t t = t0 + j;
-            if (t >= ntiles) break;
-            const int64_t base = t * URH_TILE + global_offset;
-            const int ncand = __shfl_sync(URH_FULL_MASK, l_ncand, j);
-            const int rel = __shfl_sync(URH_FULL_MASK, l_rel, j);
-            FinWalk W;
-            W.prev = __shfl_sync(URH_FULL_MASK, l_prev, j);
-            W.pp = __shfl_sync(URH_FULL_MASK, l_pp, j);
-            W.idx = __shfl_sync(URH_FULL_MASK, l_idx, j);
-            if (rel >= 0) {
-                const int c = __shfl_sync(URH_FULL_MASK, l_first, j);
-                if (c != W.prev) {
-                    if (lane == 0) fin_row(R, W.idx, base + rel, W.pp, W.prev);
-                    W.idx++;
-                    W.pp = base + rel;
-                }
-                W.prev = c;
+            for (int u = 0; u < FIN_PREFETCH; u++)
+                if (j + u < s.ncand) fire(base + (int64_t)(w[u] >> 16), (int)(w[u] & 0xffffu) - 1);
+        }
+        if (t == tlast) s_end = idx;
+        if (t == ntiles - 1) {
+            const int64_t fired = idx;
+            if (emit_tail && (is_ask || row_base + fired < n_total)) {
+                if (idx < cap_rows) *((longlong2*)out + idx) = make_longlong2(prev, (pp >= 0) ? (n_total - 1 - pp) : (n_total - tol));
+                idx++;
             }
-            const uint32_t* st = staging + t * (int64_t)stage_cap;
-            for (int k = 0; k < ncand; k += 32) {
-                const uint32_t w = (k == 0) ? w0[u] : ((k + lane < ncand) ? __ldg(st + k + lane) : 0u);
-                fin_chunk(W, w, min(32, ncand - k), lane, base, R);
-            }
-            if (t == ntiles - 1 && lane == 0) {
-                int64_t idx = W.idx;
-                const int64_t fired = idx;
-                if (emit_tail && (is_ask || row_base + fired < n_total)) {
-                    if (idx < cap_rows) *((longlong2*)out + idx) = make_longlong2(W.prev, (W.pp >= 0) ? (n_total - 1 - W.pp) : (n_total - tol));
-                    idx++;
-                }
-                d_out[0] = idx;
-                d_out[1] = fired;
-            }
-        }
-    }
+            d_out[0] = idx;
+            d_out[1] = fired;
+        }
+    }
+    __syncthreads();
+    const int64_t cnt = min(s_end - r0, (int64_t)FIN_SMEM_ROWS);
+    for (int64_t i = threadIdx.x; i < cnt; i += FIN_THREADS)
+        if (r0 + i < cap_rows) *((longlong2*)out + r0 + i) = s_rows[i];
 }
 
 struct ScanMergeRows {
@@ -337,7 +374,6 @@
     TileFire* fire;
     URH_CHECK(urh_arena(ctx, (size_t)ntiles, &fire));
     URH_CHECK(urh_arena(ctx, (size_t)(32 + 8 * (sharded ? sh.world : 0)), &d_small));
-    URH_CUDA(ctx, cudaMemsetAsync(d_small, 0xff, 4 * sizeof(int64_t), ctx->stream));
     RunCarry* d_tot_run = (RunCarry*)(d_small + 4);
     CandAgg* d_tot_cand = (CandAgg*)(d_small + 6);
     FireAgg* d_tot_fire = (FireAgg*)(d_small + 8);
@@ -354,7 +390,7 @@
     rc_ident.len = 0; rc_ident.cls = 0; rc_ident.flags = 2 | 1;
     ScanRunCarry fa;
     fa.tiles = dz.tiles; fa.n = n; fa.carry = carry;
-    URH_CHECK((urhts::scan<RunCarry, RunCarryOp, ScanRunCarry>(ctx, ntiles, rc_ident, RunCarryOp(), fa, d_tot_run)));
+    URH_CHECK((urhts::scan<RunCarry, RunCarryOp, ScanRunCarry, 4>(ctx, ntiles, rc_ident, RunCarryOp(), fa, d_tot_run)));
     if (sharded) {
         URH_LAUNCH(ctx, k_pack_stage1, 1, 1, 0, dz.d_init, (const RunCarry*)d_tot_run, d_msg1);
         URH_TL_MARK(ctx, "x4 run carry: enter");
@@ -362,28 +398,37 @@
         URH_TL_MARK(ctx, "x4 run carry: done");
         URH_LAUNCH(ctx, k_fold_carry, 1, 1, 0, (const int64_t*)d_all1, sh.rank, d_xcarry);
     }
-    ScanCandidates fb;
-    fb.tiles = dz.tiles; fb.staging = dz.staging; fb.stage_cap = dz.cap; fb.carry = carry;
-    fb.xcarry = sharded ? d_xcarry : (chain ? &chain->run : nullptr);
-    fb.tol = dz.tol; fb.head_rel = head_rel; fb.prev_cls = prev_cls; fb.fire = fire;
-    CandAgg ca_ident;
-    ca_ident.cnt = 0; ca_ident.last_cls = CLS_NONE; ca_ident.pad = 0;
-    URH_CHECK((urhts::scan<CandAgg, CandOp, ScanCandidates, 4>(ctx, ntiles, ca_ident, CandOp(), fb, d_tot_cand)));
     const int16_t* prev0 = chain ? &chain->prev_cls : dz.d_init;
-    if (sharded) {
-        URH_TL_MARK(ctx, "x5 candidates: enter");
-        URH_CHECK(urh_nccl_allgather(ctx, d_tot_cand, d_all2, sizeof(CandAgg)));
-        URH_TL_MARK(ctx, "x5 candidates: done");
-        URH_LAUNCH(ctx, k_fold_prev_cls, 1, 1, 0, (const int64_t*)d_all2, sh.rank, (const int64_t*)d_all1, d_prev0);
-        prev0 = d_prev0;
-    }
-    ScanFirings fc;
-    fc.fire = fire; fc.prev_cls = prev_cls; fc.d_prev0 = prev0; fc.global_offset = sh.global_offset; fc.row_off = row_off;
-    fc.prev_fired = prev_fired;
-    FireAgg fi_ident;
-    fi_ident.fired = 0; fi_ident.last_pos = -1;
-    URH_CHECK((urhts::scan<FireAgg, FireOp, ScanFirings>(ctx, ntiles, fi_ident, FireOp(), fc, d_tot_fire)));
-    const int64_t* xprev = chain ? &chain->prev_fired : d_small + 2;
+    if (!sharded && !chain) {
+        ScanCandFirings fbc;
+        fbc.tiles = dz.tiles; fbc.staging = dz.staging; fbc.stage_cap = dz.cap; fbc.carry = carry; fbc.tol = dz.tol; fbc.d_prev0 = prev0;
+        fbc.head_rel = head_rel; fbc.prev_cls = prev_cls; fbc.row_off = row_off; fbc.prev_fired = prev_fired;
+        FireSpan fs_ident;
+        fs_ident.first_cls = CLS_NONE; fs_ident.last_cls = CLS_NONE; fs_ident.fired = 0; fs_ident.first_pos = -1; fs_ident.last_pos = -1;
+        URH_CHECK((urhts::scan<FireSpan, FireSpanOp, ScanCandFirings, 2>(ctx, ntiles, fs_ident, FireSpanOp(), fbc, (FireSpan*)nullptr)));
+    } else {
+        ScanCandidates fb;
+        fb.tiles = dz.tiles; fb.staging = dz.staging; fb.stage_cap = dz.cap; fb.carry = carry;
+        fb.xcarry = sharded ? d_xcarry : &chain->run;
+        fb.tol = dz.tol; fb.head_rel = head_rel; fb.prev_cls = prev_cls; fb.fire = fire;
+        CandAgg ca_ident;
+        ca_ident.cnt = 0; ca_ident.last_cls = CLS_NONE; ca_ident.pad = 0;
+        URH_CHECK((urhts::scan<CandAgg, CandOp, ScanCandidates, 2>(ctx, ntiles, ca_ident, CandOp(), fb, d_tot_cand)));
+        if (sharded) {
+            URH_TL_MARK(ctx, "x5 candidates: enter");
+            URH_CHECK(urh_nccl_allgather(ctx, d_tot_cand, d_all2, sizeof(CandAgg)));
+            URH_TL_MARK(ctx, "x5 candidates: done");
+            URH_LAUNCH(ctx, k_fold_prev_cls, 1, 1, 0, (const int64_t*)d_all2, sh.rank, (const int64_t*)d_all1, d_prev0);
+            prev0 = d_prev0;
+        }
+        ScanFirings fc;
+        fc.fire = fire; fc.prev_cls = prev_cls; fc.d_prev0 = prev0; fc.global_offset = sh.global_offset; fc.row_off = row_off;
+        fc.prev_fired = prev_fired;
+        FireAgg fi_ident;
+        fi_ident.fired = 0; fi_ident.last_pos = -1;
+        URH_CHECK((urhts::scan<FireAgg, FireOp, ScanFirings, 8>(ctx, ntiles, fi_ident, FireOp(), fc, d_tot_fire)));
+    }
+    const int64_t* xprev = chain ? &chain->prev_fired : nullptr;
     if (sharded) {
         URH_TL_MARK(ctx, "x6 firings: enter");
         URH_CHECK(urh_nccl_allgather(ctx, d_tot_fire, d_all3, sizeof(FireAgg)));
@@ -402,13 +447,18 @@
     int64_t* raw = ctx->pulses + 2 * row_base;
     int64_t raw_cap = chain ? sh.rows_cap : cap_rows;
     if (dz.is_ask) URH_CHECK(urh_arena(ctx, (size_t)raw_cap * 2, &raw));
+    int64_t* h_count = ctx->h_mail + FIN_MAIL;
+    int64_t* d_count;
+    URH_CUDA(ctx, cudaHostGetDevicePointer((void**)&d_count, h_count, 0));
     int64_t got[2] = {0, 0};
     for (int attempt = 0; attempt < 2; attempt++) {
-        URH_LAUNCH(ctx, k_finish_rows, (unsigned)urh_div_up(ntiles, 8 * FIN_TILES), 256, 0, dz.tiles, dz.staging, dz.cap, (const int32_t*)head_rel,
+        URH_LAUNCH(ctx, k_finish_rows, (unsigned)urh_div_up(ntiles, FIN_THREADS), FIN_THREADS, 0, dz.tiles, dz.staging, dz.cap, (const int32_t*)head_rel,
                    (const int32_t*)prev_cls, prev0, (const int64_t*)row_off, (const int64_t*)prev_fired, xprev, ntiles, sh.global_offset,
-                   sh.n_total, dz.tol, dz.is_ask ? 1 : 0, (int64_t)dz.sps, sh.emit_tail, row_base, raw, raw_cap, d_small);
+                   sh.n_total, dz.tol, dz.is_ask ? 1 : 0, (int64_t)dz.sps, sh.emit_tail, row_base, raw, raw_cap, d_count);
         if (sharded && attempt == 0) URH_TL_MARK(ctx, "rows written");
-        URH_CHECK(urh_read_i64(ctx, d_small, 2, got));
+        URH_CUDA(ctx, cudaStreamSynchronize(ctx->stream));
+        got[0] = h_count[0];
+        got[1] = h_count[1];
         if (got[0] <= raw_cap) break;
         if (attempt == 1 || chain) URH_FAIL(ctx, URH_ERR_CUDA, "finish_tiles: row buffer overflow after regrowth");
         if (dz.is_ask) {
```

After: 224,800 (median of 6 runs). 1.03x the previous value.
